# YuQiao0303/PointDreamer

Hardware: AMD Instinct MI355X
Metric: shapes/hour (30k-pt cloud, 8x256^2 views, DDNM) on MI355X (higher is better)
Workload: dtype f16 (f32 accumulate; f32 GroupNorm/softmax statistics, f32 geometry); 1 GPU; configs[2]: synthetic 30k-point sphere shape, 8x256^2 views, texture_gen_method='DDNM_inpaint' (100 DDNM steps, 552.8M-param guided-diffusion UNet, random-init weights), NBF [21], atlas 1024^2, complete_unseen_by='unproject', optimize_from=None, hidden-point removal on (device); 4 independent shapes per step, their views batched through the UNet together; parallelism=shapes-parallel x1, views_per_unet_batch=32

## Files before the change

include/pdhip.h:

```cpp
#ifndef PDHIP_H
#define PDHIP_H
#include <stdint.h>
#include <stddef.h>
#ifdef __cplusplus
extern "C" {
#endif

#define PDHIP_OK 0
#define PDHIP_E_ARG (-1)
#define PDHIP_E_HIP (-2)
#define PDHIP_E_STATE (-3)
#define PDHIP_E_NOMEM (-4)
#define PDHIP_E_UNKNOWN_NAME (-5)

int pdhip_version(void);
int pdhip_lab_build(void);
const char* pdhip_last_error(void);
int pdhip_debug_carve_log(int on);
int pdhip_debug_carve_log_read(uint64_t* triples, int capacity);

int pdhip_project_points(const float* cam_params, int V, const float* vertices, int Vn,
                         const float* points, int N, int rescale, double padding,
                         float* pos , float* vertice_uvs ,
                         float* uv_centers, float* uv_scales,
// ... 74 lines not shown
                              const uint8_t* hard_masks, int V, int S, int N, int res, int point_size, int edge_point_size,
                              double mask_ratio_thresh, float* sparse, float* mask0, float* mask2, float* scale_factors ,
                              float* mask_ratios, void* ws , void* stream);
int pdhip_texel_visibility_shapes(const float* cam_params, int V, int S, const float* gb_pos , const uint8_t* mask ,
                                  int A, const float* uv_centers, const float* uv_scales, double padding, const float* mesh_depths ,
                                  int R, float offset, uint8_t* visibility , void* stream);
int pdhip_nbf_shrink_shapes(const uint8_t* mask , const uint8_t* visibility , int V, int S, int A,
                            const int32_t* kernels, int K, uint8_t* out , uint8_t* ws , void* stream);
int pdhip_view_select_blend_shapes(const float* cam_params, int V, int S, const float* gb_pos, const uint8_t* mask, const int64_t* face_id,
                                   int A, const float* f_normals , int F, const float* base_dirs , const float* uv_centers,
                                   const float* uv_scales, double padding, const float* scale_factors, const uint8_t* shrinked ,
                                   int K, const uint8_t* visibility, int complete_unseen_by_projection, const float* inpainted ,
                                   int r, float* atlas , uint8_t* painted , int32_t* view_ids ,
                                   void* stream);

int pdhip_rescale_vertices(float* pos , int V, int Vn, const float* uv_centers, const float* uv_scales,
                           const float* factors , double padding, void* stream);
size_t pdhip_optimize_color_ws_bytes(int V, int res, int A);
int pdhip_optimize_color(float* atlas, int A, const float* uv_map, const int64_t* face_idxs, int V, int res,
                         const float* inpainted , int r, const uint8_t* shrinked, double lr, int iterations,
                         float* final_images, void* ws, void* stream);

int pdhip_resize_mask(const uint8_t* in , int B, int in_h, int in_w,
                      uint8_t* out , int out_h, int out_w, void* stream);

int pdhip_point_visibility(int cam_res, const float* point_uvs , const float* point_depths ,
                           const float* mesh_depths , int V, int N, float offset,
                           uint8_t* visibility , int64_t* point_pixels , void* stream);

size_t pdhip_hpr_ws_bytes(int V, int N);
int pdhip_hidden_point_removal(const float* points , int N, const double* eyes , int V, double radius,
                               const uint8_t* skip, uint8_t* visibility, void* ws, void* stream);
int pdhip_hpr_read_counters(const void* ws, int V, long long* out , void* stream);

int pdhip_point_pixels(const float* point_uvs , int V, int N, int res,
                       int64_t* point_pixels , void* stream);
int pdhip_point_visibility_pixels(int cam_res, const float* point_uvs, const float* point_depths, const float* mesh_depths,
                                  int V, int N, float offset, uint8_t* visibility , int res,
                                  int64_t* point_pixels , void* stream);

size_t pdhip_sparse_views_ws_bytes(int V, int N, int res);
int pdhip_sparse_views(const int64_t* point_pixels , const float* colors ,
                       const uint8_t* validation , const uint8_t* hard_masks ,
                       int V, int N, int res, int point_size, int edge_point_size, double mask_ratio_thresh,
                       float* sparse , float* mask0, float* mask2,
                       float* scale_factors , float* mask_ratios ,
                       void* ws, void* stream);

size_t pdhip_nearest_fill_ws_ints(int B, int H, int W);
int pdhip_nearest_fill(const float* img, float* out, int B, int C, int H, int W,
                       int64_t batch_stride, int64_t chan_stride, int64_t pix_stride,
                       const void* mask, int mask_is_f32, int64_t mask_batch_stride,
                       int32_t* ws, void* stream);

size_t pdhip_linear_fill_ws_bytes(int B, int H, int W);
int pdhip_linear_fill(const float* img, float* out, int B, int C, int H, int W, const void* mask, int mask_is_f32,
                      int64_t mask_batch_stride, void* ws, int32_t* tri, void* stream);
int pdhip_linear_fill_unresolved(const void* ws, int B, int H, int W, int* out, void* stream);
int pdhip_debug_set_linear_local(int on);

int pdhip_debug_set_unproject_generic(int on);

int pdhip_texel_visibility(const float* cam_params, int V, const float* gb_pos ,
                           const uint8_t* mask , int A, const float* uv_centers ,
                           const float* uv_scales , double padding,
                           const float* mesh_depths , int R, float offset,
                           uint8_t* visibility, void* stream);

int pdhip_nbf_shrink(const uint8_t* mask , const uint8_t* visibility , int V, int A,
                     const int32_t* kernels, int K, uint8_t* out, uint8_t* ws, void* stream);
int pdhip_pack_bits(const uint8_t* in , long long n, uint64_t* out , void* stream);
int pdhip_unpack_bits(const uint64_t* in , long long n, uint8_t* out , void* stream);
int pdhip_nbf_triptych(const uint8_t* mask, const uint8_t* visibility, int V, int A, int kernel, uint8_t* out, uint8_t* ws,
                       void* stream);

int pdhip_view_select_blend(const float* cam_params, int V, const float* gb_pos, const uint8_t* mask,
                            const int64_t* face_id , int A, const float* f_normals ,
                            const float* base_dirs , const float* uv_centers, const float* uv_scales,
                            double padding, const float* scale_factors ,
                            const uint8_t* shrinked, int K, const uint8_t* visibility,
                            int complete_unseen_by_projection,
                            const float* inpainted , int r,
                            float* atlas, uint8_t* painted, int32_t* view_ids, void* stream);

int pdhip_compact_texels(const float* gb_pos, const uint8_t* mask, int A, const int32_t* view_ids,
                         float* points, int64_t* coords, int64_t* point_view_ids, int32_t* count_dev,
                         int32_t* ws, void* stream);

typedef struct pdhip_unet pdhip_unet;

int pdhip_unet_create(int image_size, int model_channels, int num_res_blocks, const int* channel_mult, int n_mult,
                      const int* attention_ds, int n_att, int num_head_channels, int out_channels, int max_batch,
                      pdhip_unet** out);
void pdhip_unet_destroy(pdhip_unet* u);
long long pdhip_unet_arena_bytes(const pdhip_unet* u);
int pdhip_unet_route_table(int image_size, int model_channels, int num_res_blocks, const int* channel_mult, int n_mult, const int* attention_ds,
                           int n_att, int num_head_channels, int out_channels, int max_batch, int N, char* buf, int buf_len);
int pdhip_unet_num_tensors(const pdhip_unet* u);
int pdhip_unet_load_tensor(pdhip_unet* u, const char* name, const void* data, int is_f16, const int64_t* shape, int ndim,
                           void* stream);
int pdhip_unet_missing_tensors(const pdhip_unet* u, char* buf, int buf_len);
int pdhip_unet_forward(pdhip_unet* u, const float* x, const float* t, int N, float* out, void* stream);
int pdhip_unet_profile(pdhip_unet* u, int enable);
int pdhip_unet_profile_read(pdhip_unet* u, double* total_ms, double* total_flops, long long* launches);
int pdhip_unet_profile_read_attention(pdhip_unet* u, double* total_ms, double* total_flops, long long* launches);

int pdhip_ddnm_schedule(float* at, float* at_next, int* t, int* t_next, float* coefs);
int pdhip_ddnm_prepare(const float* masked_imgs , const float* masks , float* y, int N, int HW, void* stream);
int pdhip_ddnm_step(float* x, const float* et, int et_channels, const float* y, const float* mask, const float* eps,
                    uint64_t seed, int step, int N, int HW, void* stream);
int pdhip_ddnm_sample(pdhip_unet* u, const float* masked_imgs, const float* masks, int N, const float* x_T,
                      const float* eps_tape, uint64_t seed, int n_steps, float* out, void* stream);
int pdhip_ddnm_sample_keyed(pdhip_unet* u, const float* masked_imgs, const float* masks, int N, const float* x_T,
                            const float* eps_tape, uint64_t seed, uint64_t first_image_key, int n_steps, float* out, void* stream);

int pdhip_debug_set_conv_bk(int bk);
int pdhip_debug_set_conv_tile(int geometry);
int pdhip_debug_set_conv_stages(int stages);
int pdhip_debug_set_conv_splitk(void* ws, long long ws_floats, int splits);
int pdhip_debug_set_conv_halo_strips(int mode);
int pdhip_pack_conv_weight_f16(const float* w_oihw, int Cout, int Cin, int taps, void* w_packed , void* stream);
int pdhip_conv2d_nhwc_f16(const void* x, const void* w_packed , const float* bias, const void* residual,
                          void* y, int N, int H, int W, int Cin, int Cout, int Cout_pad, int taps, const void* zero_page,
                          void* stream);
int pdhip_groupnorm_nhwc_f16(const void* x, const float* gamma, const float* beta, const float* film , int N,
                             int H, int W, int C, int silu, int resample, void* y, float* stats_ws, float* ws,
                             long long ws_floats, void* stream);
int pdhip_gn_silu_conv3x3_nhwc_f16(const void* x, const float* gamma, const float* beta, const float* film ,
                                   long long film_stride, const void* w_packed, const float* bias, const void* residual, void* y,
                                   int N, int H, int W, int Cin, int Cout, int Cout_pad, const void* zero_page, float* ws,
                                   long long ws_floats, void* stream);
int pdhip_debug_conv3x3_apply(const void* x, const float* table , const void* w_packed, const float* bias, const void* residual,
                              void* y, int N, int H, int W, int Cin, int Cout, int Cout_pad, const void* zero_page, void* stream);
int pdhip_debug_set_fold_skip(int on);
int pdhip_debug_set_up_phase(int mode);
int pdhip_pack_conv_up2_phase_f16(const void* w_packed, int Cin, int Cout_pad, void* w_phase, void* stream);
int pdhip_conv3x3_up2_phase_nhwc_f16(const void* x, const void* w_phase, const float* bias, void* y, int N, int H, int W, int Cin, int Cout,
                                     int Cout_pad, const void* zero_page, float* gn_part, void* stream);
int pdhip_conv3x3_up2_halo_nhwc_f16(const void* x, const void* w_packed, const float* bias, void* y, int N, int H, int W, int Cin, int Cout,
                                    int Cout_pad, const void* zero_page, void* stream);
int pdhip_debug_set_fold_resample(int on);
int pdhip_debug_set_fold_finalize(int max_batch);
int pdhip_debug_set_fold_finalize_chunks(int chunks);
int pdhip_debug_set_conv_sk(int mode, int tile, int splits);
int pdhip_debug_set_conv_sk_stages(int stages);
int pdhip_debug_set_conv_sk_kgroups(int kg);
int pdhip_debug_set_attn(int nbuf, int vt_form, int qtiles);
int pdhip_debug_set_conv_sk_order(int order);
int pdhip_gn_silu_skip1x1_nhwc_f16(const void* xa, const void* xb, int Ca, int C, const float* stats, const float* gamma, const float* beta,
                                   const void* w_packed, const float* bias, void* h0, void* sk, int N, int H, int W, void* stream);
int pdhip_debug_set_gn_iters(int iters);
int pdhip_debug_set_gn_skip_variant(int v);
int pdhip_debug_set_fuse_skip(int mode, int min_tiles);
int pdhip_debug_set_fuse_gn(int on);
int pdhip_mark_unpainted_faces(const int64_t* face_id, const uint8_t* painted, int A, int F, uint8_t* flags , void* stream);
int pdhip_vertex_texel_fetch(const float* vert_uvs , int V, const float* atlas , const uint8_t* mask ,
                             int A, int32_t* texel , float* colors , float* count , void* stream);
int pdhip_neighbor_diffuse_round(const int32_t* rowptr , const int32_t* colidx, int V, const int32_t* invalid, int IV,
                                 float* colors, float* count, float* tmp , int* colored, void* stream);
int pdhip_scatter_vertex_colors(const int32_t* texel, const float* colors, int V, float* atlas, uint8_t* mask,
                                int32_t* owner_ws , int A, void* stream);
size_t pdhip_subdivide_with_uv_ws_bytes(int V, int U, int F, int K);
int pdhip_subdivide_with_uv(const float* vertices , int V, const int64_t* faces , int F, const float* uvs , int U,
                            const int64_t* face_uv_idx , const int64_t* face_index , int K,
                            float* out_vertices, int64_t* out_faces, float* out_uvs, int64_t* out_face_uv_idx,
                            int32_t* counts , int32_t* counts_host , void* ws, void* stream);
size_t pdhip_vertex_uv_table_ws_bytes(int V, int F);
int pdhip_vertex_uv_table(int V, const int64_t* faces , const int64_t* face_uv_idx , int F, const float* uvs ,
                          int U, float* vert_uvs , int32_t* counts , void* ws, void* stream);
size_t pdhip_neighbour_csr_ws_bytes(int V, int F);
int pdhip_neighbour_csr(int V, const int64_t* faces , int F, int32_t* rowptr , int32_t* colidx ,
                        int32_t* counts , int32_t* counts_host , void* ws, void* stream);
size_t pdhip_compact_zero_count_ws_bytes(int V);
int pdhip_compact_zero_count(const float* count , int V, int32_t* invalid , int32_t* counts ,
                             int32_t* counts_host , void* ws, void* stream);

long long pdhip_io_ply_count(const char* path);
int pdhip_io_read_ply_xyzrgb(const char* path, float* xyz , uint8_t* rgb , long long n);
int pdhip_io_write_obj_mtl(const char* obj_path, const char* mtl_path, const char* texture_stem, const double* points, long long P,
                           const double* tcoords, long long T, const int64_t* faces, const int64_t* facetex, long long F);
int pdhip_io_write_obj_plain(const char* obj_path, const float* points , long long P, const int64_t* faces , long long F);
int pdhip_io_write_png(const char* path, const uint8_t* hwc, int H, int W, int channels, int zlib_level);
int pdhip_chw_f32_to_hwc_u8(const float* img, int C, int H, int W, uint8_t* out, void* stream);

size_t pdhip_unet_head_ws_floats(int N, int H, int W, int C, int Cout);
int pdhip_unet_head_f32(const void* x, const float* gamma, const float* beta, const float* w_oihw, const float* bias,
                        int N, int H, int W, int C, int Cout, float* y_nchw, float* ws, long long ws_floats, void* stream);
int pdhip_conv_rr_f16(const void* x, const void* x2, int C, int Ca, int gn_mode, const float* gamma, const float* beta, const float* film,
                      long long film_stride, const float* partA, int chunksA, const float* partB, int chunksB, const void* xs, const void* xs2, int Cs,
                      int Cs1, int taps, const void* wf, const float* bias, const void* residual, int res_up, void* y, int N, int H, int W, int Cout,
                      float* ws, long long ws_floats, float* gn_part, int* gn_chunks, void* stream);
long long pdhip_conv_rr_weight_halfs(int Cin, int taps, int Cs, int Cout);
int pdhip_conv_rr_pack_f16(const void* w_packed, int Cin, int taps, int Cs, int Cout, void* wf, void* stream);
int pdhip_gn_octet_partials_f16(const void* x, int N, int HW, int C, int chunks, float* part, void* stream);
int pdhip_gn_apply_parts_f16(const void* x, const void* x2, int Ca, int C, const float* partA, int chunksA, const float* partB, int chunksB, const float* gamma,
                             const float* beta, const float* film, long long film_stride, int N, int H, int W, int silu, void* y, void* stream);
int pdhip_debug_conv_launch_nhwc_f16(const void* x, const void* x2, int Cin1, const void* w_packed, const float* bias, const void* residual, int res_up,
                                     const void* xs, const void* xs2, int Cs1, int Cs, void* y, int N, int H, int W, int Cin, int Cout, int Cout_pad, int taps,
                                     const void* zero_page, float* ws, long long ws_floats, float* gn_part, long long gn_part_floats, int* gn_chunks, int* kernel,
                                     void* stream);
int pdhip_gn_finalize_oct_f32(const float* partA, int Ca, int chunksA, const float* partB, int Cb, int chunksB, int N, int HW, float* stats, void* stream);
int pdhip_conv_ht_f16(const void* x, const void* w_packed, const float* bias, const void* residual, int res_up, void* y, int N, int H, int W, int Cin, int Cout,
                      int Cout_pad, const void* zero_page, float* splitk_ws, long long splitk_ws_floats, float* gn_part, int* gn_chunks, void* stream);
int pdhip_conv_ht_plan(int N, int H, int W, int Cin, int Cout, int Cout_pad, long long splitk_ws_floats, int* routed, int* slabs);
int pdhip_debug_set_conv_ht(int mode, int slabs);
int pdhip_debug_set_rr_gn(int max_width);
int pdhip_debug_set_conv_rr(int mode, int variant, int slabs);
int pdhip_attention_f16(const void* qkv , void* out , int N, int T, int C, int head_dim,
                        void* vt_ws , void* stream);
int pdhip_philox_normal(float* out, long long n, uint64_t seed, uint64_t stream_id, void* stream);
int pdhip_gemv_rows_f32(const float* W, const float* b, const float* x, float* y, int R, int K, int N, int silu_out, void* stream);
int pdhip_timestep_mlp_f32(const float* t, int N, int mc, const float* w0, const float* b0, const float* w2, const float* b2, float* emb_silu,
                           float* tmp, void* stream);
int pdhip_conv_in_f16(const float* x_nchw, const void* Wt, const float* bias, void* Y, int N, int H, int W, int Cout, int Cout_pad, void* im2col_ws,
                      const void* zero_page, void* stream);
int pdhip_gn_apply_f16(const void* x, const void* x2, int Ca, int C, const float* stats, const float* partA, int chunksA, const float* partB, int chunksB,
                       const float* gamma, const float* beta, const float* film, long long film_stride, int N, int H, int W, int silu, int resample, void* y,
                       void* y_raw, void* stream);
int pdhip_gn_table_f32(const float* stats, const float* gamma, const float* beta, const float* film, long long film_stride, int N, int C, float* table, void* stream);
int pdhip_resample2x_nhwc_f16(const void* x, int N, int H, int W, int C, int mode, void* y, void* stream);
int pdhip_concat_channels_f16(const void* a, int Ca, const void* b, int Cb, long long pixels, void* y, void* stream);
int pdhip_bench_copy16(const void* src, void* dst, long long bytes, int blocks, int unroll, void* stream);

size_t pdhip_nearest_points_workspace_bytes(int Q, int M);
int pdhip_nearest_points_stage_chunk(void);
int pdhip_nearest_points(const float* queries, int Q, const float* targets, int M, double* d2, int32_t* idx, int32_t* counts, void* ws, void* stream);
int pdhip_debug_set_nearest_path(int path);
size_t pdhip_cloud_metrics_workspace_bytes(int T);
int pdhip_cloud_metrics(const double* d2, const int32_t* idx, int Q, const float* normals_src, const float* normals_tgt, int M,
                        const double* thresholds, int T, double* sums, int64_t* within, void* ws, void* stream);

size_t pdhip_mesh_contains_workspace_bytes(int Vn, int F, int Q, int resolution);
int pdhip_mesh_contains(const float* vertices, int Vn, const int64_t* faces, int F, const float* points, int Q, int resolution, uint8_t* occ,
                        int32_t* counts, void* ws, void* stream);
int pdhip_debug_set_mesh_contains_slabs(int slabs);
int pdhip_occupancy_iou(const uint8_t* a, const uint8_t* b, int Q, int64_t* out, void* stream);

size_t pdhip_closest_on_mesh_workspace_bytes(int Vn, int F, int Q);
int pdhip_closest_on_mesh(const float* vertices, int Vn, const int64_t* faces, int F, const float* points, int Q, double* d2, int32_t* face,
                          double* closest, int32_t* counts, void* ws, void* stream);
int pdhip_debug_set_closest_on_mesh(int cells_per_axis, int path);

size_t pdhip_fps_workspace_bytes(int N, int M);
int pdhip_fps(const float* points, int N, int M, int start, int32_t* idx, double* min_d2, int32_t* counts, void* ws, void* stream);
int pdhip_debug_set_fps_cells(int cells_per_axis);
size_t pdhip_owner_mean_colors_workspace_bytes(int M);
int pdhip_owner_mean_colors(const int32_t* owner, const float* colors, int N, int M, const float* fallback, float* out, void* ws_or_null, void* stream);

size_t pdhip_knn_points_workspace_bytes(int Q, int M, int k);
int pdhip_knn_max_k(void);
size_t pdhip_knn_lds_bytes(int k);
int pdhip_knn_points(const float* queries, int Q, const float* targets, int M, int k, double* d2, int32_t* idx, int32_t* counts, void* ws, void* stream);
int pdhip_debug_set_knn(int cells_per_axis, int path);
size_t pdhip_sor_filter_workspace_bytes(int N);
int pdhip_sor_filter(const double* knn_d2, int N, int kk, double std_ratio, double* mean_d, double* stats, uint8_t* keep, int32_t* kept_idx,
                     int32_t* counts, void* ws, void* stream);

size_t pdhip_mesh_components_workspace_bytes(int Vn, int F);
int pdhip_mesh_components(const int64_t* faces, int F, const float* vertices_or_null, int Vn, int32_t* vertex_comp, int32_t* face_comp,
                          int32_t* comp_root, int32_t* comp_vertices, int32_t* comp_faces, float* comp_box_or_null, int comp_capacity,
                          int32_t* counts, void* ws, void* stream);
size_t pdhip_compact_mesh_workspace_bytes(int Vn, int F);
int pdhip_compact_mesh(const float* vertices, int Vn, const int64_t* faces, int F, const float* colors_or_null, const uint8_t* face_keep,
                       float* out_vertices, int64_t* out_faces, float* out_colors_or_null, int32_t* vertex_map_or_null, int32_t* counts, void* ws,
                       void* stream);

int pdhip_mesh_boundary_vertices(const int64_t* faces, int F, int Vn, const int32_t* rowptr, const int32_t* colidx, int32_t* pair_faces,
                                 uint8_t* boundary, int32_t* counts, void* stream);
int pdhip_smooth_mesh(const float* vertices, int Vn, const int32_t* rowptr, const int32_t* colidx, const uint8_t* held_or_null, int steps,
                      double lambda, double mu, double* state_a, double* state_b, float* out_vertices, int32_t* counts, void* stream);

int pdhip_weld_cells_axis(int Vn);
int pdhip_weld_vertices(const float* vertices, int Vn, double tol, int32_t* rep, int32_t* counts, uint64_t* keys_a, uint64_t* keys_b, int32_t* vals_a,
                        int32_t* vals_b, size_t sort_len, int32_t* hist, size_t hist_words, int32_t* cstart, size_t cstart_len, float* sorted_xyzi,
                        size_t sorted_len, int32_t* parent, size_t parent_len, int32_t* misc, size_t misc_len, void* stream);
int pdhip_clean_faces(const int64_t* faces, int F, const int32_t* rep, int Vn, int64_t* out_faces, uint8_t* keep, int32_t* counts, uint64_t* keys_a,
                      uint64_t* keys_b, int32_t* vals_a, int32_t* vals_b, size_t sort_len, int32_t* hist, size_t hist_words, int32_t* misc,
                      size_t misc_len, void* stream);

size_t pdhip_debug_prims_workspace_bytes(int n, int nc);
int pdhip_debug_radix_sort(const uint64_t* keys, const int32_t* vals, int n, int bits, uint64_t* keys_out, int32_t* vals_out, void* ws, void* stream);
int pdhip_debug_sort_by_cell(const uint64_t* keys, int n, int nc, uint64_t* keys_out, int32_t* idx_out, int32_t* cstart_out, void* ws, void* stream);
int pdhip_debug_scan(const void* in, void* out, int n, int elem_bytes, int mode, int inclusive, int nc, void* ws, void* stream);

#ifdef __cplusplus
}
#endif
#endif
```

pointdreamer_amd/csrc/nn_common.h:

```cpp
#pragma once
#include "common.h"
#include <hip/hip_fp16.h>

namespace pdnn {

typedef _Float16 half_t;
typedef __attribute__((ext_vector_type(8))) _Float16 half8;
typedef __attribute__((ext_vector_type(4))) _Float16 half4;
typedef __attribute__((ext_vector_type(4))) float float4_t;

struct Tuning {
    int force_bk = 0;
    int force_stages = 0;
    int force_wmw = 0;
    int force_splits = 0;
    int halo_strips = 0;
    int sk_mode = 1;
    int sk_tile = 0;
    int sk_splits = 0;
    int sk_stages = 0;
    int sk_kg = 0;
    int sk_order = 0;
    int rr_mode = 1;
    int rr_variant = 0;
    int rr_slabs = 0;
    int ht_mode = 1;
    int ht_slabs = 0;
    int fuse_gn = 0;
    int fold_resample = 1;
    int fold_skip = 1;
    int rr_gn = 0;
    int fold_finalize = 8, fold_finalize_chunks = 16;
    int fuse_skip = 1, fuse_skip_min_tiles = 1;
    int up_phase = 1;
    int attn_nbuf = 0;
    int attn_qtn = 0;
    int attn_vt = 0;
    int gn_iters = 0;
    int gs_variant = 1;
};
Tuning& tuning();

bool conv3x3_halo_eligible(int N, int H, int W, int Cin, int Cout_pad);
int conv3x3_halo_splits(int N, int H, int W, int Cin, int Cout, int Cout_pad, size_t splitk_ws_floats);
int conv3x3_halo_launch_splits(const Tuning& t, int N, int H, int W, int Cin, int Cout, int Cout_pad, size_t halo_ws_floats);
inline bool conv3x3_halo_rows(const Tuning& t, int H, int W) { return W == 256 && (t.halo_strips == 1 || H % 4 != 0); }
int conv3x3_halo(const half_t* X, const half_t* Wt, const float* bias, const half_t* residual, half_t* Y, int N, int H, int W,
                 int Cin, int Cout, int Cout_pad, const half_t* zero_page, hipStream_t s, float* gn_part, int splits, bool full_rows,
                 float* splitk_ws, size_t splitk_ws_floats, const float* apply_table = nullptr, int res_up = 0,
                 int in_up = 0);
int splitk_reduce(const float* partial, int splits, long long M, int Cout, const float* bias, const half_t* residual, half_t* Y,
                  float* gn_part, int hw, hipStream_t s);
int conv_igemm(const Tuning& t, const half_t* X, const half_t* Wt, const float* bias, const half_t* residual, half_t* Y, int N, int H,
               int W, int Cin, int Cout, int Cout_pad, int taps, const half_t* zero_page, hipStream_t s,
               float* splitk_ws = nullptr, size_t splitk_ws_floats = 0, float* gn_part = nullptr,
               const half_t* X2 = nullptr, int Cin1 = 0,
               const float* apply_table = nullptr,
               int res_up = 0,
               int in_up = 0);
bool conv_up2_phase_eligible(int N, int H, int W, int Cin, int Cout, int Cout_pad);
int conv_up2_phase_pack(const half_t* w9, int Cin, int Cout_pad, half_t* dst, hipStream_t s);
int conv_up2_phase(const half_t* X, const half_t* Wph, const float* bias, half_t* Y, int N, int H, int W, int Cin, int Cout, int Cout_pad,
                   const half_t* zero_page, hipStream_t s, float* gn_part, int geo);
struct SkPlan { int bm, bn, splits, tile_id;
                int kg, stages, m_fast; };
SkPlan conv_sk_plan(const Tuning& t, int N, int H, int W, int Cin, int Cout, int Cout_pad, int taps, bool two_source, size_t ws_floats, int k_extra = 0);
int conv_sk_skip(const SkPlan& pl, const half_t* X, const half_t* Wt, const float* bias, half_t* Y, int N, int H, int W, int Cin, int Cout,
                 int Cout_pad, const half_t* XS, const half_t* XS2, int Cs1, int Cs, const half_t* zero_page, hipStream_t s, float* ws,
                 size_t ws_floats, float* gn_part);
int fuse_skip_weights(const half_t* w3, int K9, const half_t* w1, int Cs, int Cout_pad, const float* b3, const float* b1, int Cout, half_t* dst,
                      float* bdst, hipStream_t s);
int conv_sk(const SkPlan& pl, const half_t* X, const half_t* Wt, const float* bias, const half_t* residual, half_t* Y, int N, int H, int W,
            int Cin, int Cout, int Cout_pad, int taps, const half_t* zero_page, hipStream_t s, float* ws, size_t ws_floats, float* gn_part,
            const half_t* X2, int Cin1, int res_up = 0);
#define PD_SK_TICKET_FLOATS 4096
int gn_finalize_oct(const float* partA, int Ca, int chunksA, const float* partB, int Cb, int chunksB, int N, int HW, float eps,
                    float* stats, hipStream_t s);

struct RrIn {
    const half_t* x; const half_t* x2; int C, Ca;
    int gn;
    const float* gamma; const float* beta; const float* film; long long film_stride;
    const float* partA; const float* partB; int chunksA, chunksB; float eps;
};
struct RrPlan { int variant, S0, U0, S1, U1, bands, ntiles; };
RrPlan conv_rr_plan(const Tuning& t, int N, int H, int W, int Cin, int Cout, int taps, int Cs , size_t ws_floats,
                    bool want_gn = false );
size_t conv_rr_weight_halfs(int Cin, int taps, int Cs, int Cout);
int conv_rr_pack(const half_t* w_packed, int Cin, int taps, int Cs, int Cout, half_t* dst, hipStream_t s);
int conv_rr(const RrPlan& pl, const RrIn& in, const RrIn* skip, int taps, const half_t* wf, const float* bias, const half_t* residual, int res_up,
            half_t* Y, int N, int H, int W, int Cout, float* ws, size_t ws_floats, float* gn_part , hipStream_t s);
#define PD_RR_MAX_PART_LOADS 8

bool conv_ht_routes(const Tuning& t, int N, int H, int W, int Cin, int Cout, int Cout_pad, size_t ws_floats);
int conv_ht_slabs(const Tuning& t, int N, int H, int W, int Cin, int Cout_pad, size_t ws_floats);
int conv_ht(const half_t* X, const half_t* Wt, const float* bias, const half_t* residual, half_t* Y, int N, int H, int W, int Cin, int Cout,
            int Cout_pad, const half_t* zero_page, hipStream_t s, float* gn_part , int res_up, int slabs, float* ws, size_t ws_floats);

enum ConvKernel { CONV_HALO, CONV_RR, CONV_HT, CONV_SK, CONV_IGEMM, CONV_UP_PHASE };
const char* conv_kernel_name(ConvKernel k);
struct ConvNeeds {
    bool two_source = false;
    bool in_up = false;
    bool apply = false;
    bool in_gn = false;
    bool want_gn = false;
    int skip_cs = 0;
    bool have_wf = false, have_wf_skip = false;
};
struct ConvPlan {
    int N = 0, H = 0, W = 0, Cin = 0, Cout = 0, Cout_pad = 0, taps = 0;
    ConvKernel kernel = CONV_IGEMM;
    SkPlan sk{0, 0, 0, 0}; RrPlan rr{0, 0, 0, 0, 0, 0, 0};
    int splits = 1;
    bool halo_rows = false;
    int slabs = 1;
    int bk = 0, geo = 0;
    int stages = 0;
    bool want_gn = false;
    int gn_chunks = 0;
    bool takes_res_up = false;
    bool takes_in_up = false, takes_apply = false, takes_in_gn = false, takes_skip = false;
    int skip_cs = 0;
};
ConvPlan conv_plan(const Tuning& t, int N, int H, int W, int Cin, int Cout, int Cout_pad, int taps, const ConvNeeds& needs, size_t ws_floats);
ConvPlan conv_up2_phase_plan(const Tuning& t, int N, int H, int W, int Cin, int Cout, int Cout_pad, bool want_gn);
struct ConvArgs {
    const half_t* X; const half_t* X2; int Cin1;
    const half_t* Wt;
    const float* bias; const half_t* residual; int res_up;
    const float* apply_table;
    const RrIn* rr_in;
    const half_t* XS; const half_t* XS2; int Cs1;
    half_t* Y; const half_t* zero_page; float* ws; size_t ws_floats;
    float* gn_part;
};
int conv_launch(const ConvPlan& p, const ConvArgs& a, hipStream_t s);

__device__ __forceinline__ float silu_f(float x) { return x * __builtin_amdgcn_rcpf(1.0f + __expf(-x)); }

__device__ __forceinline__ float gn_round_f16(float f) { asm("" : "+v"(f)); return (float)(half_t)f; }
template <bool OUT_F32, bool FILM>
__device__ __forceinline__ float gn_elem(float x, float ga, float gb, float t1, float sh, int silu) {
    float f = __builtin_fmaf(x, ga, gb);
    if (!OUT_F32) f = gn_round_f16(f);
    if (FILM) {
        f = gn_round_f16(f * t1);
        f = gn_round_f16(f + sh);
    }
    if (silu) { f = silu_f(f); if (!OUT_F32) f = gn_round_f16(f); }
    return f;
}


int gn_stats(const half_t* X, int N, int HW, int C, float eps, float* stats, float* ws, size_t ws_floats, hipStream_t s);
struct GnPartsArg { const float* partA; int Ca, chunksA; const float* partB; int Cb, chunksB; float eps; };
int gn_apply(const half_t* X, const float* stats, const float* gamma, const float* beta, const float* film,
             long long film_stride, int N, int H, int W, int C, int silu, int resample, void* Y, int out_f32, hipStream_t s,
             const half_t* XB = nullptr, int Ca = 0,
             half_t* Yraw = nullptr,
             const GnPartsArg* parts = nullptr,
             int iters_hook = 0);
int gn_table(const float* stats, const float* gamma, const float* beta, const float* film, long long film_stride, int N, int C,
             float* table, hipStream_t s);
bool gn_skip_eligible(int N, int HW, int Ca, int C, int Cout, int Cout_pad);
int gn_skip(const half_t* XA, const half_t* XB, int Ca, int C, const float* stats, const float* gamma, const float* beta, const half_t* Wt,
            const float* bias, half_t* H0, half_t* SK, int N, int HW, hipStream_t s, int variant );
int resample2x(const half_t* X, int N, int H, int W, int C, int mode, half_t* Y, hipStream_t s);
int concat_channels(const half_t* A, int Ca, const half_t* B, int Cb, long long pixels, half_t* Y, hipStream_t s);

int attention(const half_t* qkv, half_t* out, int N, int T, int C, int D, hipStream_t s, half_t* vt_ws, int nbuf, int qtn, int vt);

int conv_in_3x3(const ConvPlan& p, const float* x_nchw, const half_t* Wt , const float* bias, half_t* Y,
                int N, int H, int W, int Cout, int Cout_pad, half_t* im2col_ws , const half_t* zero_page, hipStream_t s, float* gn_part = nullptr);
int head_pack(const float* w, int NO, int C, half_t* wz, hipStream_t s);
int head_gn_silu_conv3x3(const half_t* X, const float* stats, const float* gamma, const float* beta, const half_t* wz,
                         const float* bias, float* y_nchw, int N, int H, int W, int C, int NO, hipStream_t s);
int timestep_mlp(const float* t, int N, int mc, const float* w0, const float* b0, const float* w2, const float* b2,
                 float* emb_silu , float* tmp, hipStream_t s);
int gemv_rows(const float* Wm , const float* b, const float* x , float* y , int R, int K, int N,
              hipStream_t s);

struct DdnmCoef { float sqrt_1m_at, sqrt_at, sqrt_at_next, sigma_t, c1, c2; };
int ddnm_update(float* x , const float* et , int Cet, const float* y,
                const float* mask , const float* eps , unsigned long long seed,
                unsigned long long step, DdnmCoef co, int N, int HW, hipStream_t s, unsigned long long quad0 = 0);
int ddnm_prepare(const float* masked_img, const float* mask, float* y, int N, int HW, hipStream_t s);
int ddnm_finish(const float* x, float* out, long long n, hipStream_t s);
int copy16(const void* src, void* dst, long long bytes, int blocks, int unroll, hipStream_t s);
int philox_normal(float* out, long long n, unsigned long long seed, unsigned long long stream_id, hipStream_t s,
                  unsigned long long quad0 = 0);

}
```

pointdreamer_amd/csrc/nn_head.hip:

```cpp
#include "nn_common.h"
using namespace pdhip;
namespace pdnn {

#define HD_TW 32
#define HD_TH 8
#define HD_TPW 4
#define HD_IW (HD_TW + 2)
#define HD_IH (HD_TH + 2)
#define HD_NPIX (HD_IW * HD_IH)
#define HD_NCH ((HD_NPIX + 15) / 16)
#define HD_ZS_OF(NO) ((NO) == 6 ? 60 : 28)

__device__ __host__ __forceinline__ int hd_swz(int n, int C) { return n & 15 & (C / 8 - 1); }

__global__ void k_head_pack(const float* __restrict__ w , int NO, int C, half_t* __restrict__ wz) {
    const int total = 64 * C;
    for (int i = blockIdx.x * blockDim.x + threadIdx.x; i < total; i += gridDim.x * blockDim.x) {
        const int n = i / C, c = i - n * C;
        float v = 0.f;
        if (n < 9 * NO) { const int tap = n / NO, o = n - tap * NO; v = w[(size_t)o * 9 * C + (size_t)tap * C + c]; }
        const half_t hi = (half_t)v;
        const half_t lo = (half_t)(v - (float)hi);
        const int dst = n * C + (((c >> 3) ^ hd_swz(n, C)) << 3) + (c & 7);
        wz[dst] = hi;
        wz[64 * C + dst] = lo;
    }
}

int head_pack(const float* w, int NO, int C, half_t* wz, hipStream_t s) {
    PD_REQUIRE((NO == 3 || NO == 6) && (C == 32 || C == 64 || C == 128 || C == 256), "head_pack: out channels 3|6, C in {32,64,128,256}");
    k_head_pack<<<cdiv(64 * C, 256), 256, 0, s>>>(w, NO, C, wz);
    PD_LAUNCH_CHECK();
    return PDHIP_OK;
}

__device__ __forceinline__ float hd_silu(float x) { return x * __builtin_amdgcn_rcpf(1.0f + __expf(-x)); }

template <int NO, int C>
__global__ __launch_bounds__(512) void k_head(const half_t* __restrict__ X, const float* __restrict__ stats,
                                              const float* __restrict__ gamma, const float* __restrict__ beta,
                                              const half_t* __restrict__ wz, const float* __restrict__ bias,
                                              float* __restrict__ y, int H, int W, int tpw) {
    constexpr int KK = C / 32;
    constexpr int NT = (9 * NO + 15) / 16;
    constexpr int NR = NT * 16;
    constexpr int HD_ZS = HD_ZS_OF(NO);
    extern __shared__ __attribute__((aligned(16))) char smem[];
    half_t* Bs = reinterpret_cast<half_t*>(smem);
    float* zs = reinterpret_cast<float*>(smem + (size_t)2 * NR * C * 2);
    float* gab = zs + HD_NCH * 16 * HD_ZS;
    const int tid = threadIdx.x, lane = tid & 63, wave = tid >> 6;
    const int n = blockIdx.z, x0 = blockIdx.x * HD_TW;

    for (int i = tid; i < 2 * NR * C / 8; i += 512) {
        const int pl = i / (NR * C / 8), r = i - pl * (NR * C / 8);
        reinterpret_cast<half8*>(Bs)[i] = reinterpret_cast<const half8*>(wz)[pl * (64 * C / 8) + r];
    }
    for (int c = tid; c < C; c += 512) {
        const int grp = c / (C / 32);
        const float mean = stats[((size_t)n * 32 + grp) * 2], rstd = stats[((size_t)n * 32 + grp) * 2 + 1];
        const float ga = rstd * gamma[c];
        gab[c] = ga;
        gab[C + c] = beta[c] - mean * ga;
    }
    __syncthreads();

    const int q4 = lane >> 4, r16 = lane & 15;
    for (int it = 0; it < tpw; ++it) {
    const int y0 = (blockIdx.y * tpw + it) * HD_TH;
    if (y0 >= H) break;
    auto src_of = [&](int chunk, bool* inimg) -> const half_t* {
        const int idx = chunk * 16 + r16;
        const int iy = idx / HD_IW, ix = idx - iy * HD_IW;
        const int gy = y0 - 1 + iy, gx = x0 - 1 + ix;
        *inimg = idx < HD_NPIX && gy >= 0 && gy < H && gx >= 0 && gx < W;
        return X + (((size_t)n * H + (*inimg ? gy : 0)) * W + (*inimg ? gx : 0)) * C + 8 * q4;
    };
    half8 vn[KK];
    bool in_n = false;
    if (wave < HD_NCH) {
        const half_t* sp = src_of(wave, &in_n);
#pragma unroll
        for (int kk = 0; kk < KK; ++kk) vn[kk] = *reinterpret_cast<const half8*>(sp + kk * 32);
    }
    for (int chunk = wave; chunk < HD_NCH; chunk += 8) {
        half8 v[KK];
        const bool inimg = in_n;
#pragma unroll
        for (int kk = 0; kk < KK; ++kk) v[kk] = vn[kk];
        if (chunk + 8 < HD_NCH) {
            const half_t* sp = src_of(chunk + 8, &in_n);
#pragma unroll
            for (int kk = 0; kk < KK; ++kk) vn[kk] = *reinterpret_cast<const half8*>(sp + kk * 32);
        }
        float4_t acc[NT];
#pragma unroll
        for (int t = 0; t < NT; ++t) acc[t] = (float4_t){0.f, 0.f, 0.f, 0.f};
#pragma unroll
        for (int kk = 0; kk < KK; ++kk) {
            const int c0 = kk * 32 + 8 * q4;
            const float4 g0 = *reinterpret_cast<const float4*>(gab + c0), g1 = *reinterpret_cast<const float4*>(gab + c0 + 4);
            const float4 b0 = *reinterpret_cast<const float4*>(gab + C + c0), b1 = *reinterpret_cast<const float4*>(gab + C + c0 + 4);
            const float ga[8] = {g0.x, g0.y, g0.z, g0.w, g1.x, g1.y, g1.z, g1.w};
            const float gb[8] = {b0.x, b0.y, b0.z, b0.w, b1.x, b1.y, b1.z, b1.w};
            half8 ah, al;
#pragma unroll
            for (int e = 0; e < 8; ++e) {
                float a = hd_silu((float)v[kk][e] * ga[e] + gb[e]);
                if (!inimg) a = 0.f;
                const half_t hi = (half_t)a;
                ah[e] = hi;
                al[e] = (half_t)(a - (float)hi);
            }
#pragma unroll
            for (int t = 0; t < NT; ++t) {
                const int nrow = t * 16 + r16;
                const int off = nrow * C + (((kk * 4 + q4) ^ hd_swz(nrow, C)) << 3);
                const half8 bh = *reinterpret_cast<const half8*>(Bs + off);
                const half8 bl = *reinterpret_cast<const half8*>(Bs + NR * C + off);
                acc[t] = __builtin_amdgcn_mfma_f32_16x16x32_f16(al, bh, acc[t], 0, 0, 0);
                acc[t] = __builtin_amdgcn_mfma_f32_16x16x32_f16(ah, bl, acc[t], 0, 0, 0);
                acc[t] = __builtin_amdgcn_mfma_f32_16x16x32_f16(ah, bh, acc[t], 0, 0, 0);
            }
        }
#pragma unroll
        for (int t = 0; t < NT; ++t) {
            const int col = t * 16 + r16;
            if (col < 9 * NO) {
#pragma unroll
                for (int r = 0; r < 4; ++r) zs[(chunk * 16 + q4 * 4 + r) * HD_ZS + col] = acc[t][r];
            }
        }
    }
    __syncthreads();

    for (int item = tid; item < HD_TW * HD_TH * NO; item += 512) {
        const int o = item / (HD_TW * HD_TH), q = item - o * (HD_TW * HD_TH);
        const int qy = q / HD_TW, qx = q - qy * HD_TW;
        const int gy = y0 + qy, gx = x0 + qx;
        if (gy >= H || gx >= W) continue;
        float a = bias[o];
#pragma unroll
        for (int tap = 0; tap < 9; ++tap) {
            const int iy = qy + tap / 3, ix = qx + tap % 3;
            a += zs[(iy * HD_IW + ix) * HD_ZS + tap * NO + o];
        }
        y[(((size_t)n * NO + o) * H + gy) * W + gx] = a;
    }
    __syncthreads();
    }
}

size_t head_smem_bytes(int C, int NO) {
    const int NR = ((9 * NO + 15) / 16) * 16;
    return (size_t)2 * NR * C * 2 + (size_t)HD_NCH * 16 * HD_ZS_OF(NO) * 4 + (size_t)2 * C * 4;
}

template <int NO, int C>
static int head_launch(const half_t* X, const float* stats, const float* gamma, const float* beta, const half_t* wz,
                       const float* bias, float* y, int N, int H, int W, hipStream_t s) {
    auto kern = k_head<NO, C>;
    const size_t smem = head_smem_bytes(C, NO);
    PD_HIP(hipFuncSetAttribute((const void*)kern, hipFuncAttributeMaxDynamicSharedMemorySize, (int)smem));
    int tpw = HD_TPW;
    while (tpw > 1 && (long long)cdiv(W, HD_TW) * cdiv(cdiv(H, HD_TH), tpw) * N < 512) tpw >>= 1;
    dim3 grid(cdiv(W, HD_TW), cdiv(cdiv(H, HD_TH), tpw), N);
    kern<<<grid, 512, smem, s>>>(X, stats, gamma, beta, wz, bias, y, H, W, tpw);
    PD_LAUNCH_CHECK();
    return PDHIP_OK;
}

int head_gn_silu_conv3x3(const half_t* X, const float* stats, const float* gamma, const float* beta, const half_t* wz,
                         const float* bias, float* y_nchw, int N, int H, int W, int C, int NO, hipStream_t s) {
    PD_REQUIRE(NO == 3 || NO == 6, "head: out channels must be 3 or 6");
#define HL(NO_, C_) head_launch<NO_, C_>(X, stats, gamma, beta, wz, bias, y_nchw, N, H, W, s)
    if (C == 256) return NO == 6 ? HL(6, 256) : HL(3, 256);
    if (C == 128) return NO == 6 ? HL(6, 128) : HL(3, 128);
    if (C == 64) return NO == 6 ? HL(6, 64) : HL(3, 64);
    if (C == 32) return NO == 6 ? HL(6, 32) : HL(3, 32);
#undef HL
    PD_REQUIRE(false, "head: final channel count must be 32, 64, 128 or 256 (got %d)", C);
    return PDHIP_OK;
}

}
```

pointdreamer_amd/csrc/nn_misc.hip:

```cpp
#include "nn_common.h"
using namespace pdhip;
namespace pdnn {

__global__ __launch_bounds__(256) void k_im2col_in(const float* __restrict__ x, half_t* __restrict__ A, int H, int W,
                                                   long long pixels) {
    for (long long p = blockIdx.x * (long long)blockDim.x + threadIdx.x; p < pixels; p += (long long)gridDim.x * blockDim.x) {
        const int xx = (int)(p % W), y = (int)((p / W) % H);
        const long long n = p / ((long long)W * H);
        half_t row[32];
#pragma unroll
        for (int k = 27; k < 32; ++k) row[k] = (half_t)0.f;
#pragma unroll
        for (int ky = 0; ky < 3; ++ky)
#pragma unroll
            for (int kx = 0; kx < 3; ++kx) {
                const int yy = y + ky - 1, xc = xx + kx - 1;
                const bool ok = yy >= 0 && yy < H && xc >= 0 && xc < W;
#pragma unroll
                for (int c = 0; c < 3; ++c)
                    row[(ky * 3 + kx) * 3 + c] = ok ? (half_t)x[(((size_t)n * 3 + c) * H + yy) * W + xc] : (half_t)0.f;
            }
        half8* dst = reinterpret_cast<half8*>(A + (size_t)p * 32);
#pragma unroll
        for (int q = 0; q < 4; ++q) {
            half8 v;
#pragma unroll
            for (int e = 0; e < 8; ++e) v[e] = row[q * 8 + e];
            dst[q] = v;
        }
    }
}

int conv_in_3x3(const ConvPlan& p, const float* x_nchw, const half_t* Wt, const float* bias, half_t* Y, int N, int H, int W, int Cout, int Cout_pad,
                half_t* im2col_ws, const half_t* zero_page, hipStream_t s, float* gn_part) {
    PD_REQUIRE(p.N == N && p.H == H && p.W == W && p.Cin == 32 && p.Cout == Cout && p.Cout_pad == Cout_pad && p.taps == 1, "conv_in_3x3: the plan is of another layer");
    const long long pixels = (long long)N * H * W;
    k_im2col_in<<<(int)std::min<long long>((pixels + 255) / 256, 8192), 256, 0, s>>>(x_nchw, im2col_ws, H, W, pixels);
    PD_LAUNCH_CHECK();
    const ConvArgs a{im2col_ws, nullptr, 32, Wt, bias, nullptr, 0, nullptr, nullptr, nullptr, nullptr, 0, Y, zero_page, nullptr, 0, gn_part};
    return conv_launch(p, a, s);
}

#define GEMV_ROWS 128
template <int KI>
__global__ __launch_bounds__(256) void k_gemv_rows(const float* __restrict__ Wm, const float* __restrict__ b,
                                                   const float* __restrict__ x, float* __restrict__ y, int R, int K, int N,
                                                   int silu_out) {
    extern __shared__ __attribute__((aligned(16))) float s_x[];
    const int lane = threadIdx.x & 63, wave = threadIdx.x >> 6;
    const int r0 = blockIdx.x * GEMV_ROWS + wave * (GEMV_ROWS / 4);
    for (int n0 = 0; n0 < N; n0 += 8) {
        const int nb = min(8, N - n0);
        __syncthreads();
        for (int j = 0; j < 8; ++j)
            for (int k = threadIdx.x; k < K; k += 256) s_x[j * K + k] = j < nb ? x[(size_t)(n0 + j) * K + k] : 0.f;
        __syncthreads();
        for (int rr = 0; rr < GEMV_ROWS / 4; rr += 4) {
            const int r = r0 + rr;
            if (r >= R) break;
            float acc[4][8];
#pragma unroll
            for (int q = 0; q < 4; ++q)
#pragma unroll
                for (int j = 0; j < 8; ++j) acc[q][j] = 0.f;
            if (KI > 0) {
                float4 w[4][KI > 0 ? KI : 1];
#pragma unroll
                for (int q = 0; q < 4; ++q)
#pragma unroll
                    for (int it = 0; it < KI; ++it)
                        w[q][it] = *reinterpret_cast<const float4*>(Wm + (size_t)min(r + q, R - 1) * K + it * 256 + lane * 4);
#pragma unroll
                for (int it = 0; it < KI; ++it)
#pragma unroll
                    for (int j = 0; j < 8; ++j) {
                        const float4 xv = *reinterpret_cast<const float4*>(s_x + j * K + it * 256 + lane * 4);
#pragma unroll
                        for (int q = 0; q < 4; ++q)
                            acc[q][j] += w[q][it].x * xv.x + w[q][it].y * xv.y + w[q][it].z * xv.z + w[q][it].w * xv.w;
                    }
            } else {
                for (int k = lane; k < K; k += 64) {
#pragma unroll
                    for (int q = 0; q < 4; ++q) {
                        const float w = Wm[(size_t)min(r + q, R - 1) * K + k];
#pragma unroll
                        for (int j = 0; j < 8; ++j) acc[q][j] += w * s_x[j * K + k];
                    }
                }
            }
#pragma unroll
            for (int q = 0; q < 4; ++q)
#pragma unroll
                for (int j = 0; j < 8; ++j) {
                    float a = acc[q][j];
#pragma unroll
                    for (int off = 32; off > 0; off >>= 1) a += __shfl_xor(a, off);
                    if (lane == 0 && j < nb && r + q < R) {
                        a += b[r + q];
                        if (silu_out) a = a / (1.0f + expf(-a));
                        y[(size_t)(n0 + j) * R + r + q] = a;
                    }
                }
        }
    }
}

static int gemv_launch(const float* Wm, const float* b, const float* x, float* y, int R, int K, int N, int silu_out, hipStream_t s) {
    PD_REQUIRE((size_t)8 * K * sizeof(float) <= 64 * 1024, "gemv_rows: K too large (%d)", K);
    const size_t smem = (size_t)8 * K * sizeof(float);
    const int grid = cdiv(R, GEMV_ROWS);
    if (K == 1024) k_gemv_rows<4><<<grid, 256, smem, s>>>(Wm, b, x, y, R, K, N, silu_out);
    else if (K == 512) k_gemv_rows<2><<<grid, 256, smem, s>>>(Wm, b, x, y, R, K, N, silu_out);
    else if (K == 256) k_gemv_rows<1><<<grid, 256, smem, s>>>(Wm, b, x, y, R, K, N, silu_out);
    else k_gemv_rows<0><<<grid, 256, smem, s>>>(Wm, b, x, y, R, K, N, silu_out);
    PD_LAUNCH_CHECK();
    return PDHIP_OK;
}

int gemv_rows(const float* Wm, const float* b, const float* x, float* y, int R, int K, int N, hipStream_t s) {
    return gemv_launch(Wm, b, x, y, R, K, N, 0, s);
}

__global__ void k_timestep_embedding(const float* __restrict__ t, int N, int mc, float* __restrict__ e) {
    const int half = mc / 2;
    for (int idx = blockIdx.x * blockDim.x + threadIdx.x; idx < N * half; idx += gridDim.x * blockDim.x) {
        const int n = idx / half, i = idx - n * half;
        const float freq = expf(-logf(10000.0f) * (float)i / (float)half);
        const float a = t[n] * freq;
        e[(size_t)n * mc + i] = cosf(a);
        e[(size_t)n * mc + half + i] = sinf(a);
    }
}

int timestep_mlp(const float* t, int N, int mc, const float* w0, const float* b0, const float* w2, const float* b2,
                 float* emb_silu, float* tmp, hipStream_t s) {
    float* temb = tmp;
    float* h1 = tmp + (size_t)N * mc;
    k_timestep_embedding<<<cdiv((long long)N * mc / 2, 256), 256, 0, s>>>(t, N, mc, temb);
    int rc = gemv_launch(w0, b0, temb, h1, 4 * mc, mc, N, 1, s);
    if (rc) return rc;
    return gemv_launch(w2, b2, h1, emb_silu, 4 * mc, 4 * mc, N, 1, s);
}

__device__ __forceinline__ void philox4x32_10(uint32_t c[4], uint32_t k0, uint32_t k1) {
#pragma unroll
    for (int r = 0; r < 10; ++r) {
        const uint64_t p0 = (uint64_t)0xD2511F53u * c[0], p1 = (uint64_t)0xCD9E8D57u * c[2];
        const uint32_t n0 = (uint32_t)(p1 >> 32) ^ c[1] ^ k0, n2 = (uint32_t)(p0 >> 32) ^ c[3] ^ k1;
        c[0] = n0; c[1] = (uint32_t)p1; c[2] = n2; c[3] = (uint32_t)p0;
        k0 += 0x9E3779B9u; k1 += 0xBB67AE85u;
    }
}
__device__ __forceinline__ void normal4(unsigned long long seed, unsigned long long stream_id, unsigned long long quad, float out[4]) {
    uint32_t c[4] = {(uint32_t)quad, (uint32_t)(quad >> 32), (uint32_t)stream_id, (uint32_t)(stream_id >> 32)};
    philox4x32_10(c, (uint32_t)seed, (uint32_t)(seed >> 32));
    const float u0 = ((float)c[0] + 0.5f) * 2.3283064365386963e-10f, u1 = ((float)c[1] + 0.5f) * 2.3283064365386963e-10f;
    const float u2 = ((float)c[2] + 0.5f) * 2.3283064365386963e-10f, u3 = ((float)c[3] + 0.5f) * 2.3283064365386963e-10f;
    const float r0 = sqrtf(-2.0f * logf(u0)), r1 = sqrtf(-2.0f * logf(u2));
    out[0] = r0 * cosf(6.283185307179586f * u1); out[1] = r0 * sinf(6.283185307179586f * u1);
    out[2] = r1 * cosf(6.283185307179586f * u3); out[3] = r1 * sinf(6.283185307179586f * u3);
}

__global__ void k_philox_normal(float* __restrict__ out, long long n, unsigned long long seed, unsigned long long stream_id,
                                unsigned long long quad0) {
    const long long quads = (n + 3) / 4;
    for (long long qd = blockIdx.x * (long long)blockDim.x + threadIdx.x; qd < quads; qd += (long long)gridDim.x * blockDim.x) {
        float z[4];
        normal4(seed, stream_id, quad0 + (unsigned long long)qd, z);
#pragma unroll
        for (int e = 0; e < 4; ++e)
            if (qd * 4 + e < n) out[qd * 4 + e] = z[e];
    }
}

int philox_normal(float* out, long long n, unsigned long long seed, unsigned long long stream_id, hipStream_t s,
                  unsigned long long quad0) {
    k_philox_normal<<<(int)std::min<long long>(((n + 3) / 4 + 255) / 256, 4096), 256, 0, s>>>(out, n, seed, stream_id, quad0);
    PD_LAUNCH_CHECK();
    return PDHIP_OK;
}

__global__ void k_ddnm_prepare(const float* __restrict__ img, const float* __restrict__ mask, float* __restrict__ y, int HW,
                               long long total) {
    for (long long i = blockIdx.x * (long long)blockDim.x + threadIdx.x; i < total; i += (long long)gridDim.x * blockDim.x) {
        const long long n = i / (3LL * HW);
        const int p = (int)(i % HW);
        y[i] = (2.0f * img[i] - 1.0f) * mask[n * HW + p];
    }
}
int ddnm_prepare(const float* masked_img, const float* mask, float* y, int N, int HW, hipStream_t s) {
    const long long total = (long long)N * 3 * HW;
    k_ddnm_prepare<<<(int)std::min<long long>((total + 255) / 256, 4096), 256, 0, s>>>(masked_img, mask, y, HW, total);
    PD_LAUNCH_CHECK();
    return PDHIP_OK;
}

__global__ void k_ddnm_update(float* __restrict__ x, const float* __restrict__ et, int Cet, const float* __restrict__ y,
                              const float* __restrict__ mask, const float* __restrict__ eps, unsigned long long seed,
                              unsigned long long step, DdnmCoef co, int HW, long long total, unsigned long long quad0) {
    for (long long q = blockIdx.x * (long long)blockDim.x + threadIdx.x; q * 4 < total; q += (long long)gridDim.x * blockDim.x) {
        const long long i = q * 4;
        const long long n = i / (3LL * HW);
        const int c = (int)((i / HW) % 3);
        const int p = (int)(i % HW);
        float z[4];
        if (eps) { const float4 e4 = *reinterpret_cast<const float4*>(eps + i); z[0] = e4.x; z[1] = e4.y; z[2] = e4.z; z[3] = e4.w; }
        else normal4(seed, step, quad0 + (unsigned long long)q, z);
        const float4 x4 = *reinterpret_cast<const float4*>(x + i);
        const float4 e4 = *reinterpret_cast<const float4*>(et + ((size_t)n * Cet + c) * HW + p);
        const float4 y4 = *reinterpret_cast<const float4*>(y + i);
        const float4 m4 = *reinterpret_cast<const float4*>(mask + n * HW + p);
        const float xv[4] = {x4.x, x4.y, x4.z, x4.w}, ev[4] = {e4.x, e4.y, e4.z, e4.w};
        const float yv[4] = {y4.x, y4.y, y4.z, y4.w}, mv[4] = {m4.x, m4.y, m4.z, m4.w};
        float o[4];
#pragma unroll
        for (int k = 0; k < 4; ++k) {
            const float x0 = (xv[k] - ev[k] * co.sqrt_1m_at) / co.sqrt_at;
            const float x0h = x0 - mv[k] * (mv[k] * x0 - yv[k]);
            o[k] = co.sqrt_at_next * x0h + co.sigma_t * (co.c1 * z[k] + co.c2 * ev[k]);
        }
        *reinterpret_cast<float4*>(x + i) = make_float4(o[0], o[1], o[2], o[3]);
    }
}
int ddnm_update(float* x, const float* et, int Cet, const float* y, const float* mask, const float* eps,
                unsigned long long seed, unsigned long long step, DdnmCoef co, int N, int HW, hipStream_t s,
                unsigned long long quad0) {
    PD_REQUIRE(HW % 4 == 0, "ddnm_update: H*W must be a multiple of 4");
    const long long total = (long long)N * 3 * HW;
    k_ddnm_update<<<(int)std::min<long long>((total / 4 + 255) / 256, 4096), 256, 0, s>>>(x, et, Cet, y, mask, eps, seed, step, co,
                                                                                       HW, total, quad0);
    PD_LAUNCH_CHECK();
    return PDHIP_OK;
}

__global__ void k_ddnm_finish(const float* __restrict__ x, float* __restrict__ out, long long n) {
    for (long long i = blockIdx.x * (long long)blockDim.x + threadIdx.x; i < n; i += (long long)gridDim.x * blockDim.x)
        out[i] = fminf(fmaxf((x[i] + 1.0f) / 2.0f, 0.0f), 1.0f);
}
int ddnm_finish(const float* x, float* out, long long n, hipStream_t s) {
    k_ddnm_finish<<<(int)std::min<long long>((n + 255) / 256, 4096), 256, 0, s>>>(x, out, n);
    PD_LAUNCH_CHECK();
    return PDHIP_OK;
}

typedef __attribute__((ext_vector_type(4))) float cp_f4;
template <int U, int MODE>
__global__ __launch_bounds__(256) void k_copy16(const cp_f4* __restrict__ src, cp_f4* __restrict__ dst, long long n16) {
    if (MODE == 2) {
        const long long per = (n16 + gridDim.x - 1) / gridDim.x, b0 = (long long)blockIdx.x * per, b1 = b0 + per < n16 ? b0 + per : n16;
        long long i = b0 + threadIdx.x;
        for (; i + (U - 1) * 256 < b1; i += U * 256) {
            cp_f4 v[U];
#pragma unroll
            for (int u = 0; u < U; ++u) v[u] = src[i + u * 256];
#pragma unroll
            for (int u = 0; u < U; ++u) dst[i + u * 256] = v[u];
        }
        for (; i < b1; i += 256) dst[i] = src[i];
        return;
    }
    const long long stride = (long long)gridDim.x * 256;
    long long i = (long long)blockIdx.x * 256 + threadIdx.x;
    for (; i + (U - 1) * stride < n16; i += U * stride) {
        cp_f4 v[U];
#pragma unroll
        for (int u = 0; u < U; ++u) v[u] = MODE == 1 ? __builtin_nontemporal_load(src + i + u * stride) : src[i + u * stride];
#pragma unroll
        for (int u = 0; u < U; ++u) { if (MODE == 1) __builtin_nontemporal_store(v[u], dst + i + u * stride); else dst[i + u * stride] = v[u]; }
    }
    for (; i < n16; i += stride) dst[i] = src[i];
}
int copy16(const void* src, void* dst, long long bytes, int blocks, int unroll, hipStream_t s) {
    PD_REQUIRE(src && dst && bytes > 0 && bytes % 16 == 0, "copy16: bytes must be a positive multiple of 16");
    const long long n16 = bytes / 16;
    if (blocks <= 0) blocks = 256 * 8;
    const int mode = unroll >> 4, u = unroll & 15;
#define PD_CP(U_, M_) k_copy16<U_, M_><<<blocks, 256, 0, s>>>((const cp_f4*)src, (cp_f4*)dst, n16)
#define PD_CPM(M_) (u == 8 ? PD_CP(8, M_) : u == 2 ? PD_CP(2, M_) : u == 1 ? PD_CP(1, M_) : PD_CP(4, M_))
    if (mode == 1) PD_CPM(1); else if (mode == 2) PD_CPM(2); else PD_CPM(0);
#undef PD_CPM
#undef PD_CP
    PD_LAUNCH_CHECK();
    return PDHIP_OK;
}

}

extern "C" int pdhip_gemv_rows_f32(const float* W, const float* b, const float* x, float* y, int R, int K, int N, int silu_out, void* stream) {
    PD_REQUIRE(W && b && x && y, "pdhip_gemv_rows_f32: null argument");
    PD_REQUIRE(R >= 1 && K >= 1 && N >= 1, "pdhip_gemv_rows_f32: R, K, N must be positive (R=%d K=%d N=%d)", R, K, N);
    return pdnn::gemv_launch(W, b, x, y, R, K, N, silu_out != 0, as_stream(stream));
}
extern "C" int pdhip_timestep_mlp_f32(const float* t, int N, int mc, const float* w0, const float* b0, const float* w2, const float* b2,
                                      float* emb_silu, float* tmp, void* stream) {
    PD_REQUIRE(t && w0 && b0 && w2 && b2 && emb_silu && tmp, "pdhip_timestep_mlp_f32: null argument");
    PD_REQUIRE(N >= 1 && mc >= 2 && mc % 2 == 0 && mc <= 512, "pdhip_timestep_mlp_f32: N must be positive and mc even, at most 512 (N=%d mc=%d)", N, mc);
    return pdnn::timestep_mlp(t, N, mc, w0, b0, w2, b2, emb_silu, tmp, as_stream(stream));
}
extern "C" int pdhip_conv_in_f16(const float* x_nchw, const void* Wt, const float* bias, void* Y, int N, int H, int W, int Cout, int Cout_pad,
                                 void* im2col_ws, const void* zero_page, void* stream) {
    PD_REQUIRE(x_nchw && Wt && bias && Y && im2col_ws && zero_page, "pdhip_conv_in_f16: null argument");
    PD_REQUIRE(N >= 1 && H >= 1 && W >= 1 && Cout >= 1, "pdhip_conv_in_f16: N, H, W, Cout must be positive");
    PD_REQUIRE(Cout % 8 == 0 && Cout_pad % 128 == 0 && Cout_pad >= Cout, "conv_igemm: need Cin %% 32 == 0, Cout %% 8 == 0, padded Cout %% 128 == 0 (Cin=%d Cout=%d pad=%d)", 32,
               Cout, Cout_pad);
    const pdnn::ConvPlan p = pdnn::conv_plan(pdnn::tuning(), N, H, W, 32, Cout, Cout_pad, 1, pdnn::ConvNeeds(), 0);
    return pdnn::conv_in_3x3(p, x_nchw, (const pdnn::half_t*)Wt, bias, (pdnn::half_t*)Y, N, H, W, Cout, Cout_pad, (pdnn::half_t*)im2col_ws, (const pdnn::half_t*)zero_page,
                             as_stream(stream));
}
```

pointdreamer_amd/csrc/nn_norm.hip:

```cpp
#include "nn_common.h"
using namespace pdhip;
namespace pdnn {

#define GN_PIX_PER_BLOCK 256

__global__ __launch_bounds__(256) void k_gn_partial(const half_t* __restrict__ X, int HW, int C, float* __restrict__ part) {
    extern __shared__ float s_acc[];
    const int n = blockIdx.y, chunk = blockIdx.x;
    const int opp = C >> 3;
    const int pps = max(1, 256 / opp);
    const int tid = threadIdx.x;
    const int sub = tid / opp, oct = tid - sub * opp;
    const int p0 = chunk * GN_PIX_PER_BLOCK;
    const int p1 = min(HW, p0 + GN_PIX_PER_BLOCK);
    float s[8], q[8];
#pragma unroll
    for (int e = 0; e < 8; ++e) { s[e] = 0.f; q[e] = 0.f; }
    if (sub < pps) {
        for (int oc = oct; oc < opp; oc += 256) {
            for (int p = p0 + sub; p < p1; p += pps) {
                const half8 v = *reinterpret_cast<const half8*>(X + ((size_t)n * HW + p) * C + oc * 8);
#pragma unroll
                for (int e = 0; e < 8; ++e) { const float f = (float)v[e]; s[e] += f; q[e] += f * f; }
            }
// ... 152 lines not shown
        __syncthreads();
        if (threadIdx.x < 32) {
            const int opg = cg >> 3, g = threadIdx.x;
            double ds = 0.0, dq = 0.0;
            for (int k = 0; k < opg; ++k)
                for (int sl = 0; sl < pps; ++sl) { ds += s_fin[(sl * opp + g * opg + k) * 2]; dq += s_fin[(sl * opp + g * opg + k) * 2 + 1]; }
            const double cnt = (double)H * W * cg;
            const double mean = ds / cnt;
            double var = dq / cnt - mean * mean;
            if (var < 0.0) var = 0.0;
            s_st[2 * g] = (float)mean; s_st[2 * g + 1] = (float)(1.0 / sqrt(var + (double)gp.eps));
        }
        __syncthreads();
    }
#ifdef PD_LAB_GN_REV
    const int n = gridDim.y - 1 - blockIdx.y, bx = gridDim.x - 1 - blockIdx.x;
#else
    const int n = blockIdx.y, bx = blockIdx.x;
#endif
    const int sub = threadIdx.x / opp;
    if (sub >= pps) return;
    const int p_begin = bx * (pps * iters), p_end = min(Ho * Wo, p_begin + pps * iters);
    for (int oc = threadIdx.x - sub * opp; oc < opp; oc += 256) {
        const int c0 = oc * 8;
        const bool second = XB != nullptr && c0 >= Ca;
        const half_t* const Xs = second ? XB + (c0 - Ca) : X + c0;
        const int cs = XB == nullptr ? C : (second ? C - Ca : Ca);
        float ga[8], gb[8], t1[8], sh[8];
#pragma unroll
        for (int e = 0; e < 8; ++e) {
            const int c = c0 + e, grp = c / cg;
            const float mean = FIN ? s_st[2 * grp] : stats[((size_t)n * 32 + grp) * 2], rstd = FIN ? s_st[2 * grp + 1] : stats[((size_t)n * 32 + grp) * 2 + 1];
            ga[e] = rstd * gamma[c];
            gb[e] = beta[c] - mean * ga[e];
            if (FILM) {
                t1[e] = (float)(half_t)(1.0f + (float)(half_t)film[(size_t)n * film_stride + c]);
                sh[e] = (float)(half_t)film[(size_t)n * film_stride + C + c];
            }
        }
        float raw[8];
#pragma unroll
        for (int e = 0; e < 8; ++e) raw[e] = 0.f;
        auto act = [&](int yi, int xi, float* o) {
            const half8 v = *reinterpret_cast<const half8*>(Xs + (((size_t)n * H + yi) * W + xi) * cs);
            if (RES == 1) {
#pragma unroll
                for (int e = 0; e < 8; ++e) raw[e] += (float)v[e];
            }
#pragma unroll
            for (int e = 0; e < 8; ++e) {
                o[e] = gn_elem<OUT_F32, FILM>((float)v[e], ga[e], gb[e], FILM ? t1[e] : 1.f, FILM ? sh[e] : 0.f, silu);
            }
        };
        auto finish = [&](const half8& v, float* r) {
#pragma unroll
            for (int e = 0; e < 8; ++e) {
                r[e] = gn_elem<OUT_F32, FILM>((float)v[e], ga[e], gb[e], FILM ? t1[e] : 1.f, FILM ? sh[e] : 0.f, silu);
            }
        };
        auto store = [&](int p, const float* r) {
            const size_t o = ((size_t)n * Ho * Wo + p) * C + c0;
            if (OUT_F32) {
                float* Y = reinterpret_cast<float*>(Yv);
                *reinterpret_cast<float4*>(Y + o) = make_float4(r[0], r[1], r[2], r[3]);
                *reinterpret_cast<float4*>(Y + o + 4) = make_float4(r[4], r[5], r[6], r[7]);
            } else {
                half8 hv;
#pragma unroll
                for (int e = 0; e < 8; ++e) hv[e] = (half_t)r[e];
#ifdef PD_LAB_GN_NT
                __builtin_nontemporal_store(hv, reinterpret_cast<half8*>(reinterpret_cast<half_t*>(Yv) + o));
#else
                *reinterpret_cast<half8*>(reinterpret_cast<half_t*>(Yv) + o) = hv;
#endif
            }
        };
        if (RES == 0) {
            int p = p_begin + sub;
#ifndef GNA_U
#define GNA_U 4
#endif
            for (; p + (GNA_U - 1) * pps < p_end; p += GNA_U * pps) {
                half8 v[GNA_U];
#pragma unroll
#ifdef PD_LAB_GN_NTL
                for (int u = 0; u < GNA_U; ++u) v[u] = __builtin_nontemporal_load(reinterpret_cast<const half8*>(Xs + ((size_t)n * H * W + p + u * pps) * cs));
#else
                for (int u = 0; u < GNA_U; ++u) v[u] = *reinterpret_cast<const half8*>(Xs + ((size_t)n * H * W + p + u * pps) * cs);
#endif
#pragma unroll
                for (int u = 0; u < GNA_U; ++u) { float r[8]; finish(v[u], r); store(p + u * pps, r); }
            }
            for (; p < p_end; p += pps) {
                const half8 v = *reinterpret_cast<const half8*>(Xs + ((size_t)n * H * W + p) * cs);
                float r[8]; finish(v, r); store(p, r);
            }
        } else {
            for (int p = p_begin + sub; p < p_end; p += pps) {
                float r[8];
                const int yo = p / Wo, xo = p - yo * Wo;
                if (RES == 1) {
                    float a[8], b[8], c[8], d[8];
                    act(2 * yo, 2 * xo, a); act(2 * yo, 2 * xo + 1, b); act(2 * yo + 1, 2 * xo, c); act(2 * yo + 1, 2 * xo + 1, d);
#pragma unroll
                    for (int e = 0; e < 8; ++e) r[e] = (a[e] + b[e] + c[e] + d[e]) * 0.25f;
                    if (Yraw != nullptr) {
                        half8 hv;
#pragma unroll
                        for (int e = 0; e < 8; ++e) { hv[e] = (half_t)(raw[e] * 0.25f); }
                        *reinterpret_cast<half8*>(Yraw + ((size_t)n * Ho * Wo + p) * C + c0) = hv;
                    }
#pragma unroll
                    for (int e = 0; e < 8; ++e) raw[e] = 0.f;
                } else {
                    act(yo >> 1, xo >> 1, r);
                }
                store(p, r);
            }
        }
    }
}

int gn_apply(const half_t* X, const float* stats, const float* gamma, const float* beta, const float* film,
             long long film_stride, int N, int H, int W, int C, int silu, int resample, void* Y, int out_f32, hipStream_t s,
             const half_t* XB, int Ca, half_t* Yraw, const GnPartsArg* parts, int iters_hook) {
    GnParts gp{nullptr, nullptr, 0, 0, 0, 0, 0.f};
    if (parts != nullptr) {
        PD_REQUIRE(stats == nullptr && parts->partA != nullptr && (C >> 3) <= 256 && ((C / 32) % 8) == 0 && parts->Ca + parts->Cb == C &&
                   parts->Ca % 8 == 0 && parts->Cb % 8 == 0 && (parts->Cb == 0 || parts->partB != nullptr),
                   "gn_apply: bad octet partials for the in-kernel statistics");
        gp = GnParts{parts->partA, parts->partB, parts->Ca, parts->Cb, parts->chunksA, parts->chunksB, parts->eps};
    }
    PD_REQUIRE(Yraw == nullptr || (resample == 1 && XB == nullptr), "gn_apply: the raw avg-pool output belongs to resample 1");
    PD_REQUIRE(XB == nullptr || (Ca > 0 && Ca < C && Ca % 8 == 0), "gn_apply: bad two-source split");
    PD_REQUIRE(C % 32 == 0 && resample >= 0 && resample <= 2, "gn_apply: bad arguments");
    PD_REQUIRE(resample != 1 || (H % 2 == 0 && W % 2 == 0), "gn_apply: avgpool needs even H, W");
    PD_REQUIRE(!out_f32 || (resample == 0 && film == nullptr), "gn_apply: f32 output only without resampling / FiLM");
    PD_REQUIRE(film == nullptr || resample == 0, "gn_apply: FiLM only without resampling");
    const int Ho = resample == 1 ? H / 2 : (resample == 2 ? H * 2 : H), Wo = resample == 1 ? W / 2 : (resample == 2 ? W * 2 : W);
    const int opp = C >> 3, pps = max(1, 256 / opp);
    int iters = iters_hook > 0 ? iters_hook : GNA_ITERS;
    const int tgt_blocks = parts != nullptr && N <= 8 ? 512 : 2048;
    while (iters > 1 && (long long)cdiv((long long)Ho * Wo, pps * iters) * N < tgt_blocks) iters >>= 1;
    dim3 grid(cdiv((long long)Ho * Wo, pps * iters), N);
#define GNA_ARGS X, stats, gamma, beta, film, film_stride, H, W, C, silu, Y, XB, Ca, iters, Yraw, gp
#define GNA_LAUNCH(R, O, F) do { if (parts) k_gn_apply<R, O, F, true><<<grid, 256, 0, s>>>(GNA_ARGS); else k_gn_apply<R, O, F, false><<<grid, 256, 0, s>>>(GNA_ARGS); } while (0)
    if (out_f32) GNA_LAUNCH(0, true, false);
    else if (film) GNA_LAUNCH(0, false, true);
    else if (resample == 0) GNA_LAUNCH(0, false, false);
    else if (resample == 1) GNA_LAUNCH(1, false, false);
    else GNA_LAUNCH(2, false, false);
#undef GNA_LAUNCH
#undef GNA_ARGS
    PD_LAUNCH_CHECK();
    return PDHIP_OK;
}

__global__ __launch_bounds__(256) void k_resample(const half_t* __restrict__ X, int H, int W, int C, int mode,
                                                  half_t* __restrict__ Y, long long total_oct) {
    const int opp = C >> 3;
    const int Ho = mode == 1 ? H / 2 : H * 2, Wo = mode == 1 ? W / 2 : W * 2;
    for (long long idx = blockIdx.x * (long long)blockDim.x + threadIdx.x; idx < total_oct; idx += (long long)gridDim.x * blockDim.x) {
        const int oc = (int)(idx % opp);
        const long long pix = idx / opp;
        const int xo = (int)(pix % Wo), yo = (int)((pix / Wo) % Ho), n = (int)(pix / ((long long)Wo * Ho));
        half8 out;
        if (mode == 1) {
            const half_t* p = X + (((size_t)n * H + 2 * yo) * W + 2 * xo) * C + oc * 8;
            const half8 a = *reinterpret_cast<const half8*>(p), b = *reinterpret_cast<const half8*>(p + C);
            const half8 c = *reinterpret_cast<const half8*>(p + (size_t)W * C), d = *reinterpret_cast<const half8*>(p + (size_t)W * C + C);
#pragma unroll
            for (int e = 0; e < 8; ++e) out[e] = (half_t)(((float)a[e] + (float)b[e] + (float)c[e] + (float)d[e]) * 0.25f);
        } else {
            out = *reinterpret_cast<const half8*>(X + (((size_t)n * H + (yo >> 1)) * W + (xo >> 1)) * C + oc * 8);
        }
        *reinterpret_cast<half8*>(Y + (((size_t)n * Ho + yo) * Wo + xo) * C + oc * 8) = out;
    }
}

int resample2x(const half_t* X, int N, int H, int W, int C, int mode, half_t* Y, hipStream_t s) {
    PD_REQUIRE((mode == 1 || mode == 2) && C % 8 == 0, "resample2x: bad arguments");
    const int Ho = mode == 1 ? H / 2 : H * 2, Wo = mode == 1 ? W / 2 : W * 2;
    const long long total = (long long)N * Ho * Wo * (C / 8);
    k_resample<<<(int)std::min<long long>((total + 255) / 256, 65536), 256, 0, s>>>(X, H, W, C, mode, Y, total);
    PD_LAUNCH_CHECK();
    return PDHIP_OK;
}

__global__ __launch_bounds__(256) void k_concat(const half_t* __restrict__ A, int Ca, const half_t* __restrict__ B, int Cb,
                                                long long pixels, half_t* __restrict__ Y) {
    const int oa = Ca >> 3, ob = Cb >> 3, ot = oa + ob;
    const long long total = pixels * ot;
    for (long long idx = blockIdx.x * (long long)blockDim.x + threadIdx.x; idx < total; idx += (long long)gridDim.x * blockDim.x) {
        const long long p = idx / ot;
        const int o = (int)(idx - p * ot);
        const half8 v = (o < oa) ? *reinterpret_cast<const half8*>(A + (size_t)p * Ca + o * 8)
                                 : *reinterpret_cast<const half8*>(B + (size_t)p * Cb + (o - oa) * 8);
        *reinterpret_cast<half8*>(Y + (size_t)p * (Ca + Cb) + o * 8) = v;
    }
}

int concat_channels(const half_t* A, int Ca, const half_t* B, int Cb, long long pixels, half_t* Y, hipStream_t s) {
    PD_REQUIRE(Ca % 8 == 0 && Cb % 8 == 0, "concat_channels: channels must be multiples of 8");
    const long long total = pixels * ((Ca + Cb) / 8);
    k_concat<<<(int)std::min<long long>((total + 255) / 256, 65536), 256, 0, s>>>(A, Ca, B, Cb, pixels, Y);
    PD_LAUNCH_CHECK();
    return PDHIP_OK;
}

constexpr int GS_BM = 128, GS_BN = 256, GS_CLD = GS_BN + 8;
constexpr int GS_SMEM = GS_BM * GS_CLD * 2;

template <int MI = 4>
__device__ __forceinline__ void gs_epilogue(const float4_t (&acc)[MI][8], char* smem, const float* __restrict__ bias, half_t* __restrict__ SK,
                                            long long m0, int tid) {
    const int lane = tid & 63, wave = tid >> 6, wm = wave & 1, wn = wave >> 1;
    half_t* const Cs = reinterpret_cast<half_t*>(smem);
#pragma unroll
    for (int j = 0; j < 8; ++j) {
        const int nl = wn * 128 + j * 16 + (lane >> 4) * 4;
        float4_t bv = (float4_t){0.f, 0.f, 0.f, 0.f};
        if (bias != nullptr) bv = *reinterpret_cast<const float4_t*>(bias + nl);
#pragma unroll
        for (int i = 0; i < MI; ++i) {
            const int ml = wm * (16 * MI) + i * 16 + (lane & 15);
            half4 h;
#pragma unroll
            for (int r = 0; r < 4; ++r) h[r] = (half_t)(acc[i][j][r] + bv[r]);
            *reinterpret_cast<half4*>(&Cs[ml * GS_CLD + nl]) = h;
        }
    }
    __syncthreads();
    const int col8 = (tid & 31) * 8;
#pragma unroll
    for (int p = 0; p < 4 * MI; ++p) {
        const int row = p * 8 + (tid >> 5);
        *reinterpret_cast<half8*>(SK + (size_t)(m0 + row) * GS_BN + col8) = *reinterpret_cast<const half8*>(&Cs[row * GS_CLD + col8]);
    }
}
template <int NB, int MI = 4>
__device__ __forceinline__ void gs_mfma_step(float4_t (&acc)[MI][8], const char* As, const char* Ws, int lane, int wm, int wn) {
#pragma unroll
    for (int kk = 0; kk < 2; ++kk) {
        const int fo = ((kk * 4 + (lane >> 4)) ^ (lane & 7)) << 4;
        half8 a[MI];
#pragma unroll
        for (int i = 0; i < MI; ++i) a[i] = *reinterpret_cast<const half8*>(As + (wm * (16 * MI) + i * 16 + (lane & 15)) * 128 + fo);
#pragma unroll
        for (int jh = 0; jh < 8 / NB; ++jh) {
            half8 b[NB];
#pragma unroll
            for (int j = 0; j < NB; ++j) b[j] = *reinterpret_cast<const half8*>(Ws + (wn * 128 + (jh * NB + j) * 16 + (lane & 15)) * 128 + fo);
#pragma unroll
            for (int i = 0; i < MI; ++i)
#pragma unroll
                for (int j = 0; j < NB; ++j) acc[i][jh * NB + j] = __builtin_amdgcn_mfma_f32_16x16x32_f16(b[j], a[i], acc[i][jh * NB + j], 0, 0, 0);
        }
    }
}

template <typename T> __device__ __forceinline__ T* gs_uniform(T* p) {
    const unsigned long long v = reinterpret_cast<unsigned long long>(p);
    const unsigned lo = __builtin_amdgcn_readfirstlane((unsigned)v), hi = __builtin_amdgcn_readfirstlane((unsigned)(v >> 32));
    return reinterpret_cast<T*>(((unsigned long long)hi << 32) | lo);
}

#ifndef GS1_NB
#define GS1_NB 2
#endif
constexpr int GS1_SMEM = GS_SMEM;
template <int BM>
__global__ __launch_bounds__(256, 2) void k_gn_skip_w1(const half_t* __restrict__ XA, const half_t* __restrict__ XB, int Ca, int C,
                                                       const float* __restrict__ stats, const float* __restrict__ gamma,
                                                       const float* __restrict__ beta, const half_t* __restrict__ Wt,
                                                       const float* __restrict__ bias, half_t* __restrict__ H0, half_t* __restrict__ SK,
                                                       int HW) {
    extern __shared__ __align__(16) char gs_smem[];
    char* const As = gs_smem;
    constexpr int MI = BM / 32, RJ = BM / 32;
    char* const Ws = gs_smem + BM * 128;
    float* const Gs = reinterpret_cast<float*>(gs_smem + BM * 128 + GS_BN * 128);
    const int tid = threadIdx.x, lane = tid & 63, wave = tid >> 6, wm = wave & 1, wn = wave >> 1;
    const long long m0 = (long long)blockIdx.x * BM;
    const int n = (int)(m0 / HW), cg = C / 32, Cb = C - Ca, KC = C / 64;
    const int slot = tid & 7, prow = tid >> 3;
    const int sw = (slot ^ (prow & 7)) << 4;
    half8 xa[2][RJ], wr[8];
    const unsigned offA = (unsigned)(prow * Ca + slot * 8) * 2u, offB = (unsigned)(prow * Cb + slot * 8) * 2u;
    const unsigned offC = (unsigned)(prow * C + slot * 8) * 2u;
    const char* const baseA = reinterpret_cast<const char*>(XA + (size_t)m0 * Ca);
    const char* const baseB = reinterpret_cast<const char*>(XB + (size_t)m0 * Cb);
    const char* const baseW = reinterpret_cast<const char*>(Wt);
    char* const baseH = reinterpret_cast<char*>(H0 + (size_t)m0 * C);
    auto issue_acts = [&](int kc, half8* dst) {
        const int cu = min(kc, KC - 1) * 64;
        const bool second = cu >= Ca;
        const char* const src = gs_uniform(second ? baseB + (size_t)(cu - Ca) * 2 : baseA + (size_t)cu * 2);
        const unsigned off = second ? offB : offA, rs = (unsigned)(second ? Cb : Ca) * 64u;
#pragma unroll
        for (int j = 0; j < RJ; ++j) dst[j] = *reinterpret_cast<const half8*>(src + (off + j * rs));
    };
    auto issue_w = [&](int kc) {
        const char* const src = gs_uniform(baseW + (size_t)(min(kc, KC - 1) * 64) * 2);
#pragma unroll
        for (int j = 0; j < 8; ++j) wr[j] = *reinterpret_cast<const half8*>(src + (offC + j * ((unsigned)C * 64u)));
    };
// ... 85 lines not shown
```

pointdreamer_amd/csrc/nn_unet.hip:

```cpp
#include "nn_common.h"
#include <map>
#include <string>
#include <vector>
#include <cmath>
#include <cstring>
using namespace pdhip;
using namespace pdnn;

namespace {

struct ConvW { half_t* w = nullptr; float* b = nullptr; int cin = 0, cout = 0, cout_pad = 0, taps = 0; bool have_w = false, have_b = false;
               half_t* wf = nullptr; half_t* wph = nullptr; bool has_wf = false, has_wph = false; };
struct NormW { float* g = nullptr; float* b = nullptr; int c = 0; bool have_g = false, have_b = false; };
struct ResB { std::string name; int cin, cout, mode; NormW n1, n2; ConvW c1, c2, skip; long long emb_off; bool has_skip; bool have_ew = false, have_eb = false;
              half_t* c2s_w = nullptr; float* c2s_b = nullptr; bool c2s_ready = false; half_t* c2s_wf = nullptr; int hw = 0; bool has_c2s = false, has_c2s_wf = false; };
struct AttB { std::string name; int c; NormW n; ConvW qkv, proj; };
struct Block { int kind; int idx; };

struct Act { half_t* p; int C, H, W; const float* gn_part = nullptr; int gn_chunks = 0; const float* gn_partB = nullptr; int Ca = 0; int gn_chunksB = 0;
             half_t* p2 = nullptr;
             int row = -1, rowB = -1; };

}
namespace pdnn {
Tuning& tuning() { static thread_local Tuning t; return t; }
}
static thread_local float* g_dbg_splitk_ws = nullptr;
static thread_local size_t g_dbg_splitk_floats = 0;
namespace {
struct Prof { std::vector<hipEvent_t> ev; std::vector<uint8_t> cls; size_t used = 0; double flops[2] = {0, 0}; bool on = false;
              int period = 1; long long forwards = 0; bool armed = false; };

}

struct pdhip_unet {
    int image_size, mc, nres, head, out_ch, max_batch, ted;
    std::vector<int> mult, att_ds;
    std::vector<ResB> res;
    std::vector<AttB> att;
    std::vector<std::vector<Block>> input, output;
    std::vector<Block> middle;
    int final_ch;
    half_t* w_in = nullptr; float* b_in = nullptr; bool have_win = false, have_bin = false;
    float *te_w0 = nullptr, *te_b0 = nullptr, *te_w2 = nullptr, *te_b2 = nullptr; bool have_te[4] = {false, false, false, false};
    float *emb_w = nullptr, *emb_b = nullptr; long long emb_rows = 0;
    NormW out_norm; float* out_w = nullptr; float* out_b = nullptr; bool have_ow = false, have_ob = false;
    half_t* zero_page = nullptr;
    char* arena = nullptr; size_t arena_bytes = 0, arena_off = 0; bool arena_overflow = false;
    float *stats = nullptr, *gn_ws = nullptr; size_t gn_ws_floats = 0;
    float* ap_table = nullptr;
    float *emb_silu = nullptr, *emb_tmp = nullptr, *emb_all = nullptr;
    float *steps_t = nullptr, *steps_silu = nullptr, *steps_tmp = nullptr, *steps_emb = nullptr; int steps_cached = 0;
    half_t* head_wz = nullptr;
    half_t* head_wz3 = nullptr;
    float *t_dev = nullptr;
    float* splitk_ws = nullptr; size_t splitk_floats = 0;
    float *sx = nullptr, *sy = nullptr, *set_ = nullptr, *smask = nullptr;
    Prof prof;
    std::vector<void*> owned;
};

namespace {

template <typename T>
int dalloc(pdhip_unet* u, T** p, size_t count) {
    void* q = nullptr;
    hipError_t e = hipMalloc(&q, std::max<size_t>(count * sizeof(T), 256));
    if (e != hipSuccess) { set_error("hipMalloc(%zu bytes) failed: %s", count * sizeof(T), hipGetErrorString(e)); return PDHIP_E_NOMEM; }
    u->owned.push_back(q);
    *p = reinterpret_cast<T*>(q);
    return PDHIP_OK;
}
#define PD_TRY(expr) do { int rc_ = (expr); if (rc_ != PDHIP_OK) return rc_; } while (0)

int alloc_conv(pdhip_unet* u, ConvW& c) {
    PD_TRY(dalloc(u, &c.w, (size_t)c.cout_pad * c.taps * c.cin));
    PD_HIP(hipMemset(c.w, 0, (size_t)c.cout_pad * c.taps * c.cin * sizeof(half_t)));
    PD_TRY(dalloc(u, &c.b, (size_t)c.cout));
    return PDHIP_OK;
}
int alloc_norm(pdhip_unet* u, NormW& n, int c) {
    n.c = c;
    PD_TRY(dalloc(u, &n.g, (size_t)c));
    PD_TRY(dalloc(u, &n.b, (size_t)c));
    return PDHIP_OK;
}

__global__ void k_pack_conv(const void* __restrict__ src, int src_f16, int Cout, int Cin, int taps, half_t* __restrict__ dst) {
    const long long total = (long long)Cout * Cin * taps;
    for (long long i = blockIdx.x * (long long)blockDim.x + threadIdx.x; i < total; i += (long long)gridDim.x * blockDim.x) {
        const int tap = (int)(i % taps);
        const int c = (int)((i / taps) % Cin);
        const int o = (int)(i / ((long long)taps * Cin));
        const float v = src_f16 ? (float)reinterpret_cast<const half_t*>(src)[i] : reinterpret_cast<const float*>(src)[i];
        dst[(size_t)o * taps * Cin + (size_t)tap * Cin + c] = (half_t)v;
    }
}
__global__ void k_pack_conv_in(const void* __restrict__ src, int src_f16, int Cout, half_t* __restrict__ dst) {
    const int total = Cout * 27;
    for (int i = blockIdx.x * blockDim.x + threadIdx.x; i < total; i += gridDim.x * blockDim.x) {
        const int tap = i % 9, c = (i / 9) % 3, o = i / 27;
        const float v = src_f16 ? (float)reinterpret_cast<const half_t*>(src)[i] : reinterpret_cast<const float*>(src)[i];
        dst[(size_t)o * 32 + tap * 3 + c] = (half_t)v;
    }
}
__global__ void k_pack_conv_f32(const void* __restrict__ src, int src_f16, int Cout, int Cin, int taps, float* __restrict__ dst) {
    const long long total = (long long)Cout * Cin * taps;
    for (long long i = blockIdx.x * (long long)blockDim.x + threadIdx.x; i < total; i += (long long)gridDim.x * blockDim.x) {
        const int tap = (int)(i % taps);
        const int c = (int)((i / taps) % Cin);
        const int o = (int)(i / ((long long)taps * Cin));
        const float v = src_f16 ? (float)reinterpret_cast<const half_t*>(src)[i] : reinterpret_cast<const float*>(src)[i];
        dst[(size_t)o * taps * Cin + (size_t)tap * Cin + c] = v;
    }
}
__global__ void k_copy_f32(const void* __restrict__ src, int src_f16, long long n, float* __restrict__ dst, int round_f16) {
    for (long long i = blockIdx.x * (long long)blockDim.x + threadIdx.x; i < n; i += (long long)gridDim.x * blockDim.x) {
        float v = src_f16 ? (float)reinterpret_cast<const half_t*>(src)[i] : reinterpret_cast<const float*>(src)[i];
        if (round_f16) v = (float)(half_t)v;
        dst[i] = v;
    }
}
int grid_for(long long n) { return (int)std::min<long long>((n + 255) / 256, 4096); }

half_t* arena_take(pdhip_unet* u, size_t halfs) {
    size_t bytes = (halfs * sizeof(half_t) + 255) & ~(size_t)255;
    if (u->arena == nullptr) { u->arena_off += bytes; return nullptr; }
    if (u->arena_off + bytes > u->arena_bytes) { u->arena_overflow = true; return reinterpret_cast<half_t*>(u->arena); }
    half_t* p = reinterpret_cast<half_t*>(u->arena + u->arena_off);
    u->arena_off += bytes;
    return p;
}

struct Act;
struct Table { std::vector<std::string> name, line; };
struct Ctx { pdhip_unet* u; int N; hipStream_t s; bool dry; const float* film_base; long long film_stride; Table* table;
             Tuning t;
             bool go() const { return !dry && table == nullptr; } };

int prof_begin(Ctx& c, double flops, int cls = 0) {
    Prof& p = c.u->prof;
    if (!p.on || !p.armed || !c.go()) return PDHIP_OK;
    if (p.used + 2 > p.ev.size()) {
        for (int i = 0; i < 256; ++i) { hipEvent_t e; PD_HIP(hipEventCreate(&e)); p.ev.push_back(e); p.cls.push_back(0); }
    }
    PD_HIP(hipEventRecord(p.ev[p.used], c.s));
    p.cls[p.used] = (uint8_t)cls;
    p.flops[cls] += flops;
    return PDHIP_OK;
}
int prof_end(Ctx& c) {
    Prof& p = c.u->prof;
    if (!p.on || !p.armed || !c.go()) return PDHIP_OK;
    PD_HIP(hipEventRecord(p.ev[p.used + 1], c.s));
    p.used += 2;
    return PDHIP_OK;
}

float* take_parts(Ctx& c, int H, int W, int cout) {
    return reinterpret_cast<float*>(arena_take(c.u, (size_t)c.N * ((H * W + 15) / 16) * (cout / 8) * 2 * 2));
}
void adopt_parts(Act* out, float* part, int chunks) {
    if (part != nullptr && chunks > 0) { out->gn_part = part; out->gn_chunks = chunks; out->Ca = out->C; }
}

struct ConvIn { const Act* x; const half_t* residual = nullptr; int res_up = 0; const float* apply_table = nullptr; const RrIn* rr_in = nullptr;
                const Act* skip_src = nullptr; const ResB* skip_w = nullptr;
                const Act* parts_of = nullptr; const char* note = nullptr; };

void table_row(Ctx& c, const std::string& name, const ConvPlan& p, const ConvIn& in, Act* out) {
    char detail[64];
    switch (p.kernel) {
    case CONV_HALO: case CONV_IGEMM: snprintf(detail, sizeof detail, "splits=%d", p.splits); break;
    case CONV_HT: snprintf(detail, sizeof detail, "slabs=%d", p.slabs); break;
    case CONV_RR: snprintf(detail, sizeof detail, "variant=%d,slabs=%d", p.rr.variant, p.rr.S0); break;
    case CONV_SK: snprintf(detail, sizeof detail, "tile=%dx%d,splits=%d", p.sk.bm, p.sk.bn, p.sk.splits); break;
    default: snprintf(detail, sizeof detail, "-"); break;
    }
    std::string folds;
    auto add = [&](const std::string& f) { folds += (folds.empty() ? "" : ",") + f; };
    if (in.note) add(in.note);
    if (in.x->p2) add("two_source");
    if (p.takes_apply) add("apply");
    if (p.takes_in_gn) add("in_gn");
    if (p.takes_in_up) add("in_up");
    if (in.res_up) add("res_up");
    if (p.takes_skip) add("skip");
    if (in.parts_of) {
        const Act& a = *in.parts_of;
        add("parts<-" + (a.gn_part && a.row >= 0 ? c.table->name[a.row] : std::string("?")) +
            (a.p2 ? "+" + (a.gn_partB && a.rowB >= 0 ? c.table->name[a.rowB] : std::string("?")) : std::string()));
    }
    char line[512];
    snprintf(line, sizeof line, "%s %dx%d %d->%d %s %s gn=%d %s", name.c_str(), p.H, p.W, p.Cin, p.Cout, conv_kernel_name(p.kernel), detail, p.gn_chunks,
             folds.empty() ? "-" : folds.c_str());
    out->row = (int)c.table->line.size();
    c.table->name.push_back(name);
    c.table->line.push_back(line);
}

int run_conv(Ctx& c, const std::string& name, const ConvPlan& p, const ConvW& w, const ConvIn& in, Act* out) {
    *out = Act{nullptr, p.Cout, p.H, p.W};
    out->p = arena_take(c.u, (size_t)c.N * p.H * p.W * p.Cout);
    float* part = p.want_gn ? take_parts(c, p.H, p.W, p.Cout) : nullptr;
    if (c.table) table_row(c, name, p, in, out);
    if (!c.dry) adopt_parts(out, part, p.gn_chunks);
    if (!c.go()) return PDHIP_OK;
    PD_REQUIRE(w.have_w && w.have_b, "unet: weights of %s not loaded", name.c_str());
    const ResB* fs = p.takes_skip ? in.skip_w : nullptr;
    PD_REQUIRE(fs == nullptr || (fs->skip.have_w && fs->skip.have_b && fs->c2s_ready), "unet: fused conv2 + skip weights of %s were not built at load time", name.c_str());
    const half_t* wt = fs ? (p.kernel == CONV_RR ? fs->c2s_wf : fs->c2s_w) : p.kernel == CONV_RR ? w.wf : p.kernel == CONV_UP_PHASE ? w.wph : w.w;
    const Act& x = *in.x;
    const Act* xs = p.takes_skip ? in.skip_src : nullptr;
    const ConvArgs a{x.p, x.p2, x.p2 ? x.Ca : 0, wt, fs ? fs->c2s_b : w.b, in.residual, in.res_up, in.apply_table, in.rr_in,
                     xs ? xs->p : nullptr, xs ? xs->p2 : nullptr, xs && xs->p2 ? xs->Ca : 0, out->p, c.u->zero_page, c.u->splitk_ws, c.u->splitk_floats, part};
    const bool booked = p.kernel == CONV_HALO && p.splits == 1;
    if (booked) PD_TRY(prof_begin(c, 2.0 * c.N * p.H * p.W * (double)p.Cout * 9.0 * p.Cin));
    PD_TRY(conv_launch(p, a, c.s));
    return booked ? prof_end(c) : PDHIP_OK;
}
ConvPlan plan_conv(const Ctx& c, const Act& x, const ConvW& w, bool want_gn) {
    ConvNeeds nd;
    nd.two_source = x.p2 != nullptr; nd.want_gn = want_gn; nd.have_wf = w.has_wf;
    return conv_plan(c.t, c.N, x.H, x.W, w.cin, w.cout, w.cout_pad, w.taps, nd, c.u->splitk_floats);
}

int run_gn_stats(Ctx& c, const Act& x) {
    if (x.gn_part != nullptr && ((x.C / 32) % 8) == 0)
        return gn_finalize_oct(x.gn_part, x.Ca, x.gn_chunks, x.gn_partB, x.C - x.Ca, x.gn_chunksB, c.N, x.H * x.W, 1e-5f, c.u->stats, c.s);
    PD_REQUIRE(x.p2 == nullptr, "unet: a virtual concat needs fused GroupNorm partials of both tensors");
    return gn_stats(x.p, c.N, x.H * x.W, x.C, 1e-5f, c.u->stats, c.u->gn_ws, c.u->gn_ws_floats, c.s);
}

int run_gn(Ctx& c, const Act& x, const NormW& n, const float* film, long long film_stride, int silu, int resample, Act* out,
           half_t* raw_pool = nullptr) {
    *out = Act{nullptr, x.C, 0, 0};
    out->H = resample == 1 ? x.H / 2 : (resample == 2 ? x.H * 2 : x.H);
    out->W = resample == 1 ? x.W / 2 : (resample == 2 ? x.W * 2 : x.W);
    out->p = arena_take(c.u, (size_t)c.N * out->H * out->W * x.C);
    if (!c.go()) return PDHIP_OK;
    PD_REQUIRE(n.have_g && n.have_b, "unet: norm weights not loaded");
#ifdef PD_LAB_SKIP_GN
    if (resample == 0 && x.p2 == nullptr && x.W <= 128 && silu) { out->p = x.p; return PDHIP_OK; }
#endif
    if (x.gn_part != nullptr && ((x.C / 32) % 8) == 0 && (x.C >> 3) <= 256 && c.t.fold_finalize > 0 &&
        (c.N <= c.t.fold_finalize || (x.gn_chunks <= c.t.fold_finalize_chunks && x.gn_chunksB <= c.t.fold_finalize_chunks))) {
        const GnPartsArg pa{x.gn_part, x.Ca, x.gn_chunks, x.gn_partB, x.C - x.Ca, x.gn_chunksB, 1e-5f};
        return gn_apply(x.p, nullptr, n.g, n.b, film, film_stride, c.N, x.H, x.W, x.C, silu, resample, out->p, 0, c.s, x.p2,
                        x.p2 ? x.Ca : 0, raw_pool, &pa, c.t.gn_iters);
    }
    PD_TRY(run_gn_stats(c, x));
    return gn_apply(x.p, c.u->stats, n.g, n.b, film, film_stride, c.N, x.H, x.W, x.C, silu, resample, out->p, 0, c.s, x.p2, x.p2 ? x.Ca : 0,
                    raw_pool, nullptr, c.t.gn_iters);
}

int run_gn_then_conv(Ctx& c, const std::string& name, const ConvPlan& p, const Act& x, const NormW& n, const float* film, long long film_stride,
                     int resample, half_t* raw_pool, const ConvW& w, ConvIn in, Act* out) {
    if (p.takes_apply) {
        if (c.go()) {
            PD_REQUIRE(n.have_g && n.have_b, "unet: norm weights not loaded");
            PD_TRY(run_gn_stats(c, x));
            PD_TRY(gn_table(c.u->stats, n.g, n.b, film, film_stride, c.N, x.C, c.u->ap_table, c.s));
            in.apply_table = c.u->ap_table;
        }
        in.x = &x;
        return run_conv(c, name, p, w, in, out);
    }
    if (p.takes_in_gn) {
        if (c.go()) PD_REQUIRE(n.have_g && n.have_b, "unet: norm weights not loaded");
        const RrIn rr_in{x.p, nullptr, x.C, x.C, 2, n.g, n.b, film, film_stride, x.gn_part, nullptr, x.gn_chunks, 0, 1e-5f};
        in.x = &x; in.rr_in = &rr_in; in.parts_of = &x;
        return run_conv(c, name, p, w, in, out);
    }
    Act h;
    PD_TRY(run_gn(c, x, n, film, film_stride, 1, resample, &h, raw_pool));
    in.x = &h;
    if (x.p2 != nullptr) in.parts_of = &x;
    return run_conv(c, name, p, w, in, out);
}

struct ResPlan {
    bool fuse_skip = false;
    bool fold_down = false;
    bool fold_up = false;
    bool skip_conv = false;
    ConvPlan c1, c2, skip;
};
bool wish_in_gn(const Tuning& t, const Act& x, const ConvW& w, int W) {
    if (t.rr_gn <= 0 || W > t.rr_gn || x.p2 != nullptr || x.gn_part == nullptr || x.gn_partB != nullptr || ((x.C / 32) % 8) != 0 || w.cin > 1024 ||
        x.C != w.cin) return false;
    const int pps = std::max(1, 256 / (x.C >> 3));
    return (x.gn_chunks + pps - 1) / pps <= PD_RR_MAX_PART_LOADS;
}
bool wish_up_phase(const Tuning& t, int N, const ResB& rb, int H, int W) {
    if (t.up_phase == 0 || rb.mode != 2 || !rb.c1.has_wph || (H * W) % 256 != 0 ||
        !conv_up2_phase_eligible(N, H, W, rb.c1.cin, rb.c1.cout, rb.c1.cout_pad)) return false;
    if (t.up_phase == 2) return true;
    const long long tiles = (long long)N * H * W / 256 * 4 * (rb.c1.cout_pad / (rb.c1.cout_pad % 256 == 0 ? 256 : 128));
    return tiles >= 128;
}
ResPlan plan_res(const Tuning& t, int N, size_t ws_floats, bool conservative, const Act& x, const ResB& rb) {
    ResPlan r;
    const int Ho = rb.mode == 1 ? x.H / 2 : (rb.mode == 2 ? x.H * 2 : x.H), Wo = rb.mode == 1 ? x.W / 2 : (rb.mode == 2 ? x.W * 2 : x.W);
    const bool lean = !conservative;
    const bool fold = t.fold_resample != 0 && lean && x.p2 == nullptr && !rb.has_skip;
    r.fold_down = fold && rb.mode == 1;
    r.fuse_skip = rb.has_skip && rb.mode == 0 && t.fuse_skip != 0 && rb.skip.taps == 1 && x.C == rb.skip.cin &&
                  gn_skip_eligible(N, x.H * x.W, x.p2 ? x.Ca : x.C, x.C, rb.skip.cout, rb.skip.cout_pad) &&
                  (t.fuse_skip == 2 || (long long)N * x.H * x.W / 128 >= t.fuse_skip_min_tiles) &&
                  (conservative || (x.gn_part != nullptr && ((x.C / 32) % 8) == 0));
    ConvNeeds n1;
    n1.want_gn = true; n1.have_wf = rb.c1.has_wf;
    if (lean && !r.fuse_skip && rb.mode == 0 && x.p2 == nullptr) { n1.apply = t.fuse_gn != 0; n1.in_gn = wish_in_gn(t, x, rb.c1, x.W); }
    n1.in_up = fold && rb.mode == 2;
    if (lean && x.p2 == nullptr && !rb.has_skip && wish_up_phase(t, N, rb, x.H, x.W))
        r.c1 = conv_up2_phase_plan(t, N, Ho, Wo, rb.c1.cin, rb.c1.cout, rb.c1.cout_pad, true);
    else
        r.c1 = conv_plan(t, N, Ho, Wo, rb.c1.cin, rb.c1.cout, rb.c1.cout_pad, 9, n1, ws_floats);
    Act h1{nullptr, rb.cout, Ho, Wo};
    if (r.c1.gn_chunks > 0) { h1.gn_part = x.gn_part ? x.gn_part : reinterpret_cast<const float*>(&r); h1.gn_chunks = r.c1.gn_chunks; h1.Ca = rb.cout; }
    ConvNeeds n2;
    n2.want_gn = true; n2.have_wf = rb.c2.has_wf;
    if (lean) { n2.apply = t.fuse_gn != 0; n2.in_gn = wish_in_gn(t, h1, rb.c2, Wo); }
    if (lean && rb.has_skip && !r.fuse_skip && t.fold_skip != 0 && rb.mode == 0 && rb.has_c2s && rb.skip.taps == 1 &&
        (x.p2 == nullptr || (x.Ca % 64 == 0 && (x.C - x.Ca) % 64 == 0))) {
        n2.skip_cs = rb.skip.cin;
        n2.have_wf_skip = rb.has_c2s_wf && (x.p2 == nullptr || (x.Ca % 128 == 0 && (x.C - x.Ca) % 128 == 0));
    }
    r.c2 = conv_plan(t, N, Ho, Wo, rb.c2.cin, rb.c2.cout, rb.c2.cout_pad, 9, n2, ws_floats);
    r.fold_up = fold && rb.mode == 2 && r.c2.takes_res_up;
    r.skip_conv = rb.has_skip && !r.fuse_skip && !r.c2.takes_skip;
    if (r.skip_conv) {
        ConvNeeds ns;
        ns.two_source = x.p2 != nullptr;
        r.skip = conv_plan(t, N, Ho, Wo, rb.skip.cin, rb.skip.cout, rb.skip.cout_pad, rb.skip.taps, ns, ws_floats);
    }
    return r;
}

int run_res(Ctx& c, const Act& x, ResB& rb, Act* out) {
    const ResPlan r = plan_res(c.t, c.N, c.u->splitk_floats, c.dry, x, rb);
    Act h1, xr = x, sk;
    const float* film = c.go() ? c.film_base + rb.emb_off : nullptr;
    if (c.go()) PD_REQUIRE(rb.have_ew && rb.have_eb, "unet: emb_layers of %s not loaded", rb.name.c_str());
    if (rb.mode != 0) {
        xr.H = r.c2.H; xr.W = r.c2.W;
        xr.p = arena_take(c.u, (size_t)c.N * xr.H * xr.W * x.C);
    }
    const std::string n1 = rb.name + ".in_layers.2";
    if (r.fuse_skip) {
        Act h0{nullptr, x.C, x.H, x.W};
        h0.p = arena_take(c.u, (size_t)c.N * x.H * x.W * x.C);
        sk = Act{nullptr, rb.skip.cout, x.H, x.W};
        sk.p = arena_take(c.u, (size_t)c.N * x.H * x.W * rb.skip.cout);
        if (c.go()) {
            PD_REQUIRE(rb.n1.have_g && rb.n1.have_b && rb.skip.have_w && rb.skip.have_b, "unet: norm / skip weights of %s not loaded", rb.name.c_str());
            PD_TRY(run_gn_stats(c, x));
            PD_TRY(gn_skip(x.p, x.p2, x.p2 ? x.Ca : x.C, x.C, c.u->stats, rb.n1.g, rb.n1.b, rb.skip.w, rb.skip.b, h0.p, sk.p, c.N, x.H * x.W, c.s, c.t.gs_variant));
        }
        ConvIn in{&h0};
        in.parts_of = &x; in.note = "gn_skip";
        PD_TRY(run_conv(c, n1, r.c1, rb.c1, in, &h1));
    } else {
        const bool half_res = r.c1.kernel == CONV_UP_PHASE || r.c1.takes_in_up;
        PD_TRY(run_gn_then_conv(c, n1, r.c1, x, rb.n1, nullptr, 0, half_res ? 0 : rb.mode, r.fold_down ? xr.p : nullptr, rb.c1, ConvIn{nullptr}, &h1));
    }
    if (rb.mode != 0 && c.go() && !r.fold_down && !r.fold_up) PD_TRY(resample2x(x.p, c.N, x.H, x.W, x.C, rb.mode, xr.p, c.s));
    if (!r.fuse_skip) sk = r.fold_up ? x : xr;
    if (r.skip_conv) PD_TRY(run_conv(c, rb.name + ".skip_connection", r.skip, rb.skip, ConvIn{&xr}, &sk));
    ConvIn in2{nullptr, r.c2.takes_skip ? nullptr : sk.p, r.fold_up ? 1 : 0};
    in2.skip_src = &x; in2.skip_w = &rb;
    return run_gn_then_conv(c, rb.name + ".out_layers.3", r.c2, h1, rb.n2, film, c.film_stride, 0, nullptr, rb.c2, in2, out);
}

int run_att(Ctx& c, const Act& x, AttB& ab, Act* out) {
    Act xn, qkv, a;
    PD_TRY(run_gn(c, x, ab.n, nullptr, 0, 0, 0, &xn));
    PD_TRY(run_conv(c, ab.name + ".qkv", plan_conv(c, xn, ab.qkv, false), ab.qkv, ConvIn{&xn}, &qkv));
    a = x;
    a.p = arena_take(c.u, (size_t)c.N * x.H * x.W * x.C);
    half_t* vt = arena_take(c.u, (size_t)c.N * x.H * x.W * x.C);
    if (c.go()) {
        const double T = (double)x.H * x.W;
        PD_TRY(prof_begin(c, 4.0 * c.N * T * T * x.C, 1));
        PD_TRY(attention(qkv.p, a.p, c.N, x.H * x.W, x.C, c.u->head, c.s, vt, c.t.attn_nbuf, c.t.attn_qtn, c.t.attn_vt));
        PD_TRY(prof_end(c));
    }
    return run_conv(c, ab.name + ".proj_out", plan_conv(c, a, ab.proj, true), ab.proj, ConvIn{&a, x.p}, out);
}

int run_blocks(Ctx& c, std::vector<Block>& blocks, Act* h, const float* x_nchw) {
    for (Block& b : blocks) {
        Act o;
        if (b.kind == 0) {
            o.C = c.u->mult[0] * c.u->mc; o.H = o.W = c.u->image_size;
            const int cpad = ((o.C + 127) / 128) * 128;
            ConvNeeds nd;
            nd.want_gn = true;
            const ConvPlan p = conv_plan(c.t, c.N, o.H, o.W, 32, o.C, cpad, 1, nd, 0);
            o.p = arena_take(c.u, (size_t)c.N * o.H * o.W * o.C);
            half_t* col = arena_take(c.u, (size_t)c.N * o.H * o.W * 32);
            float* part = reinterpret_cast<float*>(arena_take(c.u, (size_t)c.N * ((o.H * o.W + 127) / 128) * (o.C / 8) * 2 * 2));
            if (c.table) { Act in{nullptr, 32, o.H, o.W}; table_row(c, "input_blocks.0.0", p, ConvIn{&in}, &o); }
            if (!c.dry) adopt_parts(&o, part, p.gn_chunks);
            if (c.go()) {
                PD_REQUIRE(c.u->have_win && c.u->have_bin, "unet: input conv not loaded");
                PD_TRY(conv_in_3x3(p, x_nchw, c.u->w_in, c.u->b_in, o.p, c.N, o.H, o.W, o.C, cpad, col, c.u->zero_page, c.s, part));
            }
        } else if (b.kind == 1) {
            PD_TRY(run_res(c, *h, c.u->res[b.idx], &o));
        } else {
            PD_TRY(run_att(c, *h, c.u->att[b.idx], &o));
        }
        *h = o;
    }
    return PDHIP_OK;
}

int forward_impl(const Tuning& tun, pdhip_unet* u, const float* x, const float* t, int N, float* out, hipStream_t s, bool dry,
                 const float* shared_emb = nullptr, int head_ch = 0, Table* table = nullptr) {
    Ctx c{u, N, s, dry, shared_emb ? shared_emb : u->emb_all, shared_emb ? 0 : u->emb_rows, table, tun};
    u->arena_off = 0;
    u->arena_overflow = false;
    if (c.go() && u->prof.on) u->prof.armed = (u->prof.forwards++ % u->prof.period) == 0;
    if (c.go() && shared_emb == nullptr) {
        PD_REQUIRE(u->have_te[0] && u->have_te[1] && u->have_te[2] && u->have_te[3], "unet: time_embed not loaded");
        PD_TRY(timestep_mlp(t, N, u->mc, u->te_w0, u->te_b0, u->te_w2, u->te_b2, u->emb_silu, u->emb_tmp, s));
        PD_TRY(gemv_rows(u->emb_w, u->emb_b, u->emb_silu, u->emb_all, (int)u->emb_rows, u->ted, N, s));
    }
    std::vector<Act> hs;
    Act h{nullptr, 0, 0, 0};
    for (auto& blk : u->input) {
        PD_TRY(run_blocks(c, blk, &h, x));
        hs.push_back(h);
    }
    PD_TRY(run_blocks(c, u->middle, &h, x));
    for (auto& blk : u->output) {
        Act sk = hs.back(); hs.pop_back();
        Act cat{nullptr, h.C + sk.C, h.H, h.W};
        const bool part_ok = h.gn_part && sk.gn_part && !h.gn_partB && !sk.gn_partB && !h.p2 && !sk.p2;
        if (part_ok) {
            cat.gn_part = h.gn_part; cat.gn_partB = sk.gn_part; cat.Ca = h.C; cat.gn_chunks = h.gn_chunks; cat.gn_chunksB = sk.gn_chunks;
            cat.row = h.row; cat.rowB = sk.row;
        }
        const Block& first = blk.front();
        const bool virt = part_ok && h.C % 64 == 0 && sk.C % 64 == 0 && ((cat.C / 32) % 8) == 0 && first.kind == 1 &&
                          u->res[first.idx].mode == 0 && u->res[first.idx].has_skip;
        if (virt) {
            cat.p = h.p; cat.p2 = sk.p;
        } else {
            cat.p = arena_take(u, (size_t)N * h.H * h.W * (h.C + sk.C));
            if (c.go()) PD_TRY(concat_channels(h.p, h.C, sk.p, sk.C, (long long)N * h.H * h.W, cat.p, s));
        }
        h = cat;
        PD_TRY(run_blocks(c, blk, &h, x));
    }
    if (c.go()) {
        PD_REQUIRE(!u->arena_overflow, "unet: activation arena too small for this routing (sized at create())");
        PD_REQUIRE(u->out_norm.have_g && u->out_norm.have_b && u->have_ow && u->have_ob, "unet: output head not loaded");
        PD_TRY(run_gn_stats(c, h));
        const bool eps_only = head_ch == 3 && u->out_ch == 6;
        PD_TRY(head_gn_silu_conv3x3(h.p, u->stats, u->out_norm.g, u->out_norm.b, eps_only ? u->head_wz3 : u->head_wz, u->out_b, out, N,
                                    h.H, h.W, h.C, eps_only ? 3 : u->out_ch, s));
    }
    return PDHIP_OK;
}

const size_t kSplitkFloats = (size_t)16 * 384 * 128 * 128;
void shape_conv(ConvW& c, int cin, int cout, int taps) { c.cin = cin; c.cout = cout; c.taps = taps; c.cout_pad = ((cout + 127) / 128) * 128; }
int build_graph(pdhip_unet* u, int image_size, int model_channels, int num_res_blocks, const int* channel_mult, int n_mult,
                const int* attention_ds, int n_att, int num_head_channels, int out_channels, int max_batch) {
    PD_REQUIRE(channel_mult && n_mult > 0 && (n_att == 0 || attention_ds), "pdhip_unet_create: null argument");
    PD_REQUIRE(model_channels % 32 == 0 && image_size % (1 << (n_mult - 1)) == 0 && max_batch >= 1 && max_batch <= 64,
               "pdhip_unet_create: model_channels %% 32, image_size %% 2^(levels-1), 1 <= max_batch <= 64 required");
    PD_REQUIRE(num_head_channels == 32 || num_head_channels == 64, "pdhip_unet_create: num_head_channels must be 32 or 64");
    PD_REQUIRE(out_channels == 3 || out_channels == 6, "pdhip_unet_create: out_channels must be 3 or 6");
    u->image_size = image_size; u->mc = model_channels; u->nres = num_res_blocks; u->head = num_head_channels;
    u->out_ch = out_channels; u->max_batch = max_batch; u->ted = model_channels * 4;
    u->splitk_floats = kSplitkFloats;
    u->mult.assign(channel_mult, channel_mult + n_mult);
    u->att_ds.assign(attention_ds, attention_ds + n_att);
    auto is_att = [&](int ds) { for (int a : u->att_ds) if (a == ds) return true; return false; };
    long long emb_rows = 0;
    auto add_res = [&](const std::string& name, int cin, int cout, int mode, int hw) -> int {
        ResB rb; rb.name = name; rb.cin = cin; rb.cout = cout; rb.mode = mode; rb.has_skip = cin != cout; rb.hw = hw;
        rb.emb_off = emb_rows; emb_rows += 2 * cout;
        shape_conv(rb.c1, cin, cout, 9); shape_conv(rb.c2, cout, cout, 9);
        if (rb.has_skip) shape_conv(rb.skip, cin, cout, 1);
        rb.has_c2s = rb.has_skip && mode == 0 && cin % 64 == 0 && cout % 64 == 0;
        rb.c1.has_wph = mode == 2 && ((hw / 2) * (hw / 2)) % 256 == 0 && conv_up2_phase_eligible(1, hw / 2, hw / 2, cin, cout, rb.c1.cout_pad);
        rb.c1.has_wf = rb.c2.has_wf = hw <= 64 && cin % 128 == 0 && cout % 128 == 0;
        rb.has_c2s_wf = rb.c2.has_wf && rb.has_c2s;
        u->res.push_back(rb);
        return (int)u->res.size() - 1;
    };
    auto add_att = [&](const std::string& name, int c) -> int {
        AttB ab; ab.name = name; ab.c = c;
        shape_conv(ab.qkv, c, 3 * c, 1); shape_conv(ab.proj, c, c, 1);
        u->att.push_back(ab);
        return (int)u->att.size() - 1;
    };
    int ch = u->mult[0] * u->mc;
    std::vector<int> chans{ch};
    u->input.push_back({Block{0, 0}});
    int ds = 1, n = 1;
    for (int level = 0; level < n_mult; ++level) {
        for (int r = 0; r < num_res_blocks; ++r) {
            std::vector<Block> layers;
            const int o = u->mult[level] * u->mc;
            layers.push_back(Block{1, add_res("input_blocks." + std::to_string(n) + ".0", ch, o, 0, image_size / ds)});
            ch = o;
            if (is_att(ds)) layers.push_back(Block{2, add_att("input_blocks." + std::to_string(n) + ".1", ch)});
            u->input.push_back(layers);
            chans.push_back(ch);
            ++n;
        }
        if (level != n_mult - 1) {
            u->input.push_back({Block{1, add_res("input_blocks." + std::to_string(n) + ".0", ch, ch, 1, image_size / (ds * 2))}});
            chans.push_back(ch);
            ds *= 2;
            ++n;
        }
    }
    u->middle.push_back(Block{1, add_res("middle_block.0", ch, ch, 0, image_size / ds)});
    u->middle.push_back(Block{2, add_att("middle_block.1", ch)});
    u->middle.push_back(Block{1, add_res("middle_block.2", ch, ch, 0, image_size / ds)});
    n = 0;
    for (int level = n_mult - 1; level >= 0; --level) {
        for (int i = 0; i < num_res_blocks + 1; ++i) {
            const int ich = chans.back(); chans.pop_back();
            const int o = u->mc * u->mult[level];
            std::vector<Block> layers;
            const std::string base = "output_blocks." + std::to_string(n) + ".";
            layers.push_back(Block{1, add_res(base + "0", ch + ich, o, 0, image_size / ds)});
            ch = o;
            int k = 1;
            if (is_att(ds)) { layers.push_back(Block{2, add_att(base + std::to_string(k), ch)}); ++k; }
            if (level && i == num_res_blocks) {
                layers.push_back(Block{1, add_res(base + std::to_string(k), ch, ch, 2, image_size / (ds / 2))});
                ds /= 2;
            }
            u->output.push_back(layers);
            ++n;
        }
    }
    u->final_ch = ch;
    u->emb_rows = emb_rows;
    return PDHIP_OK;
}

}

extern "C" int pdhip_unet_create(int image_size, int model_channels, int num_res_blocks, const int* channel_mult, int n_mult,
                                 const int* attention_ds, int n_att, int num_head_channels, int out_channels, int max_batch,
                                 pdhip_unet** out) {
    PD_REQUIRE(out, "pdhip_unet_create: null argument");
    pdhip_unet* u = new pdhip_unet();
    *out = nullptr;
    auto fail = [&](int rc) { for (void* p : u->owned) (void)hipFree(p); delete u; return rc; };
    int rc = build_graph(u, image_size, model_channels, num_res_blocks, channel_mult, n_mult, attention_ds, n_att, num_head_channels, out_channels, max_batch);
    if (rc) return fail(rc);
    const long long emb_rows = u->emb_rows;
    auto chk = [&](int r) { if (rc == PDHIP_OK) rc = r; };
    for (ResB& rb : u->res) {
        chk(alloc_norm(u, rb.n1, rb.cin)); chk(alloc_norm(u, rb.n2, rb.cout));
        chk(alloc_conv(u, rb.c1)); chk(alloc_conv(u, rb.c2));
        if (rb.has_skip) chk(alloc_conv(u, rb.skip));
        if (rb.has_c2s) {
            chk(dalloc(u, &rb.c2s_w, (size_t)rb.c2.cout_pad * (9 * (size_t)rb.cout + rb.cin)));
            chk(dalloc(u, &rb.c2s_b, (size_t)rb.cout));
        }
        if (rb.c1.has_wph) chk(dalloc(u, &rb.c1.wph, (size_t)16 * rb.c1.cout_pad * rb.cin));
        if (rb.c1.has_wf) chk(dalloc(u, &rb.c1.wf, conv_rr_weight_halfs(rb.cin, 9, 0, rb.cout)));
        if (rb.c2.has_wf) chk(dalloc(u, &rb.c2.wf, conv_rr_weight_halfs(rb.cout, 9, 0, rb.cout)));
        if (rb.has_c2s_wf) chk(dalloc(u, &rb.c2s_wf, conv_rr_weight_halfs(rb.cout, 9, rb.cin, rb.cout)));
        if (rc) return fail(rc);
    }
    for (AttB& ab : u->att) {
        chk(alloc_norm(u, ab.n, ab.c)); chk(alloc_conv(u, ab.qkv)); chk(alloc_conv(u, ab.proj));
        if (rc) return fail(rc);
    }
    const int c0 = u->mult[0] * u->mc;
    chk(dalloc(u, &u->w_in, (size_t)(((c0 + 127) / 128) * 128) * 32)); chk(dalloc(u, &u->b_in, (size_t)c0));
    if (rc == PDHIP_OK && hipMemset(u->w_in, 0, (size_t)(((c0 + 127) / 128) * 128) * 32 * sizeof(half_t)) != hipSuccess) rc = PDHIP_E_HIP;
    chk(dalloc(u, &u->te_w0, (size_t)u->ted * u->mc)); chk(dalloc(u, &u->te_b0, (size_t)u->ted));
    chk(dalloc(u, &u->te_w2, (size_t)u->ted * u->ted)); chk(dalloc(u, &u->te_b2, (size_t)u->ted));
    chk(dalloc(u, &u->emb_w, (size_t)emb_rows * u->ted)); chk(dalloc(u, &u->emb_b, (size_t)emb_rows));
    chk(alloc_norm(u, u->out_norm, u->final_ch));
    chk(dalloc(u, &u->out_w, (size_t)out_channels * 9 * u->final_ch)); chk(dalloc(u, &u->out_b, (size_t)out_channels));
    chk(dalloc(u, &u->zero_page, (size_t)128));
    if (rc) return fail(rc);
    if (hipMemset(u->zero_page, 0, 256) != hipSuccess) { set_error("hipMemset failed"); return fail(PDHIP_E_HIP); }
    const size_t S2 = (size_t)image_size * image_size;
    chk(forward_impl(tuning(), u, nullptr, nullptr, max_batch, nullptr, nullptr, true));
    u->arena_bytes = u->arena_off + 4096;
    {
        void* q = nullptr;
        hipError_t e = hipMalloc(&q, u->arena_bytes);
        if (e != hipSuccess) { set_error("pdhip_unet_create: activation arena of %zu bytes: %s", u->arena_bytes, hipGetErrorString(e)); return fail(PDHIP_E_NOMEM); }
        u->owned.push_back(q);
        u->arena = reinterpret_cast<char*>(q);
    }
    u->gn_ws_floats = (size_t)max_batch * ((S2 + 255) / 256) * 64;
    chk(dalloc(u, &u->stats, (size_t)max_batch * 64)); chk(dalloc(u, &u->gn_ws, u->gn_ws_floats));
    { int cmax = 0; for (const ResB& rb : u->res) cmax = std::max(cmax, std::max(rb.cin, rb.cout)); chk(dalloc(u, &u->ap_table, (size_t)max_batch * cmax * 2)); }
    chk(dalloc(u, &u->emb_silu, (size_t)max_batch * u->ted)); chk(dalloc(u, &u->emb_tmp, (size_t)max_batch * (u->mc + u->ted)));
    chk(dalloc(u, &u->emb_all, (size_t)max_batch * emb_rows));
    chk(dalloc(u, &u->steps_t, 128)); chk(dalloc(u, &u->steps_silu, (size_t)100 * u->ted));
    chk(dalloc(u, &u->steps_tmp, (size_t)100 * (u->mc + u->ted))); chk(dalloc(u, &u->steps_emb, (size_t)100 * emb_rows));
    { float* wz = nullptr; chk(dalloc(u, &wz, (size_t)64 * u->final_ch)); u->head_wz = reinterpret_cast<half_t*>(wz); }
    { float* wz = nullptr; chk(dalloc(u, &wz, (size_t)64 * u->final_ch)); u->head_wz3 = reinterpret_cast<half_t*>(wz); }
    chk(dalloc(u, &u->t_dev, (size_t)max_batch));
    chk(dalloc(u, &u->splitk_ws, u->splitk_floats));
    if (rc == PDHIP_OK && hipMemset(u->splitk_ws, 0, PD_SK_TICKET_FLOATS * sizeof(float)) != hipSuccess) rc = PDHIP_E_HIP;
    chk(dalloc(u, &u->sx, (size_t)max_batch * 3 * S2)); chk(dalloc(u, &u->sy, (size_t)max_batch * 3 * S2));
    chk(dalloc(u, &u->set_, (size_t)max_batch * out_channels * S2)); chk(dalloc(u, &u->smask, (size_t)max_batch * S2));
// ... 128 lines not shown
        if (rest == "in_layers.0.bias") return load_vec(rb.n1.b, rb.cin, &rb.n1.have_b, 0);
        if (rest == "in_layers.2.weight") return load_conv_w(rb.c1);
        if (rest == "in_layers.2.bias") return load_vec(rb.c1.b, rb.cout, &rb.c1.have_b, 1);
        if (rest == "emb_layers.1.weight") return load_vec(u->emb_w + rb.emb_off * u->ted, (long long)2 * rb.cout * u->ted, &rb.have_ew, 0);
        if (rest == "emb_layers.1.bias") return load_vec(u->emb_b + rb.emb_off, 2 * rb.cout, &rb.have_eb, 0);
        if (rest == "out_layers.0.weight") return load_vec(rb.n2.g, rb.cout, &rb.n2.have_g, 0);
        if (rest == "out_layers.0.bias") return load_vec(rb.n2.b, rb.cout, &rb.n2.have_b, 0);
        auto refuse = [&](int rc) -> int {
            if (rc != PDHIP_OK || !rb.has_c2s) return rc;
            rb.c2s_ready = false;
            if (rb.c2.have_w && rb.c2.have_b && rb.skip.have_w && rb.skip.have_b && rb.skip.taps == 1) {
                PD_TRY(fuse_skip_weights(rb.c2.w, 9 * rb.c2.cin, rb.skip.w, rb.skip.cin, rb.c2.cout_pad, rb.c2.b, rb.skip.b, rb.cout, rb.c2s_w, rb.c2s_b, s));
                if (rb.has_c2s_wf) PD_TRY(conv_rr_pack(rb.c2s_w, rb.c2.cin, 9, rb.skip.cin, rb.cout, rb.c2s_wf, s));
                rb.c2s_ready = true;
            }
            return PDHIP_OK;
        };
        if (rest == "out_layers.3.weight") return refuse(load_conv_w(rb.c2));
        if (rest == "out_layers.3.bias") return refuse(load_vec(rb.c2.b, rb.cout, &rb.c2.have_b, 1));
        if (rb.has_skip && rest == "skip_connection.weight") return refuse(load_conv_w(rb.skip));
        if (rb.has_skip && rest == "skip_connection.bias") return refuse(load_vec(rb.skip.b, rb.cout, &rb.skip.have_b, 1));
    }
    for (AttB& ab : u->att) {
        if (!starts(ab.name + ".")) continue;
        const std::string rest = name.substr(ab.name.size() + 1);
        if (rest == "norm.weight") return load_vec(ab.n.g, ab.c, &ab.n.have_g, 0);
        if (rest == "norm.bias") return load_vec(ab.n.b, ab.c, &ab.n.have_b, 0);
        if (rest == "qkv.weight") return load_conv_w(ab.qkv);
        if (rest == "qkv.bias") return load_vec(ab.qkv.b, 3 * ab.c, &ab.qkv.have_b, 1);
        if (rest == "proj_out.weight") return load_conv_w(ab.proj);
        if (rest == "proj_out.bias") return load_vec(ab.proj.b, ab.c, &ab.proj.have_b, 1);
    }
    (void)ends;
    set_error("pdhip_unet_load_tensor: unknown tensor name '%s'", name_c);
    return PDHIP_E_UNKNOWN_NAME;
}

extern "C" int pdhip_unet_forward(pdhip_unet* u, const float* x, const float* t, int N, float* out, void* stream) {
    PD_REQUIRE(u && x && t && out, "pdhip_unet_forward: null argument");
    PD_REQUIRE(N >= 1 && N <= u->max_batch, "pdhip_unet_forward: batch %d outside [1, %d]", N, u->max_batch);
    return forward_impl(tuning(), u, x, t, N, out, as_stream(stream), false);
}

extern "C" int pdhip_unet_profile(pdhip_unet* u, int enable) {
    PD_REQUIRE(u, "pdhip_unet_profile: null handle");
    u->prof.on = enable != 0;
    u->prof.period = enable > 1 ? enable : 1;
    u->prof.forwards = 0;
    u->prof.armed = false;
    u->prof.used = 0;
    u->prof.flops[0] = u->prof.flops[1] = 0;
    return PDHIP_OK;
}
static int prof_read(pdhip_unet* u, int cls, double* total_ms, double* total_flops, long long* launches) {
    double ms = 0;
    long long n = 0;
    for (size_t i = 0; i + 1 < u->prof.used; i += 2) {
        if (u->prof.cls[i] != cls) continue;
        PD_HIP(hipEventSynchronize(u->prof.ev[i + 1]));
        float e = 0;
        PD_HIP(hipEventElapsedTime(&e, u->prof.ev[i], u->prof.ev[i + 1]));
        ms += e; ++n;
    }
    *total_ms = ms; *total_flops = u->prof.flops[cls]; *launches = n;
    return PDHIP_OK;
}
extern "C" int pdhip_unet_profile_read(pdhip_unet* u, double* total_ms, double* total_flops, long long* launches) {
    PD_REQUIRE(u && total_ms && total_flops && launches, "pdhip_unet_profile_read: null argument");
    return prof_read(u, 0, total_ms, total_flops, launches);
}
extern "C" int pdhip_unet_profile_read_attention(pdhip_unet* u, double* total_ms, double* total_flops, long long* launches) {
    PD_REQUIRE(u && total_ms && total_flops && launches, "pdhip_unet_profile_read_attention: null argument");
    return prof_read(u, 1, total_ms, total_flops, launches);
}

namespace {
struct Sched { std::vector<int> t; std::vector<DdnmCoef> co; std::vector<float> ab; };
Sched make_schedule() {
    Sched s;
    s.ab.resize(1001);
    double acc = 1.0;
    s.ab[0] = 1.0f;
    const double b0 = 1e-4, b1 = 0.02, step = (b1 - b0) / 999.0;
    for (int i = 0; i < 1000; ++i) {
        const double beta = (i == 999) ? b1 : b0 + (double)i * step;
        acc = acc * (double)(1.0f - (float)beta);
        s.ab[i + 1] = (float)acc;
    }
    const double eta = 0.85;
    for (int k = 99; k >= 0; --k) {
        const int t = k * 10, tn = (k - 1) * 10 < 0 ? -1 : (k - 1) * 10;
        const float at = s.ab[t + 1], an = s.ab[tn + 1];
        DdnmCoef c;
        c.sqrt_1m_at = sqrtf(1.0f - at); c.sqrt_at = sqrtf(at); c.sqrt_at_next = sqrtf(an);
        c.sigma_t = sqrtf(1.0f - an * an);
        c.c1 = sqrtf(1.0f - an) * (float)eta;
        c.c2 = sqrtf(1.0f - an) * (float)std::sqrt(1.0 - eta * eta);
        s.t.push_back(t); s.co.push_back(c);
    }
    return s;
}
__global__ void k_fill(float* p, float v, int n) { int i = blockIdx.x * blockDim.x + threadIdx.x; if (i < n) p[i] = v; }
}

extern "C" int pdhip_ddnm_schedule(float* at, float* at_next, int* t, int* t_next, float* coefs ) {
    Sched s = make_schedule();
    for (int k = 0; k < 100; ++k) {
        const int tt = s.t[k], tn = tt - 10 < 0 ? -1 : tt - 10;
        if (at) at[k] = s.ab[tt + 1];
        if (at_next) at_next[k] = s.ab[tn + 1];
        if (t) t[k] = tt;
        if (t_next) t_next[k] = tn;
        if (coefs) memcpy(coefs + 6 * k, &s.co[k], sizeof(DdnmCoef));
    }
    return PDHIP_OK;
}

extern "C" int pdhip_ddnm_step(float* x, const float* et, int et_channels, const float* y, const float* mask, const float* eps,
                               uint64_t seed, int step, int N, int HW, void* stream) {
    PD_REQUIRE(x && et && y && mask && step >= 0 && step < 100 && (et_channels == 3 || et_channels == 6), "pdhip_ddnm_step: bad arguments");
    static const Sched sched = make_schedule();
    return ddnm_update(x, et, et_channels, y, mask, eps, seed, (unsigned long long)step + 1, sched.co[step], N, HW, as_stream(stream));
}

extern "C" int pdhip_ddnm_prepare(const float* masked_imgs, const float* masks, float* y, int N, int HW, void* stream) {
    PD_REQUIRE(masked_imgs && masks && y, "pdhip_ddnm_prepare: null argument");
    return ddnm_prepare(masked_imgs, masks, y, N, HW, as_stream(stream));
}

extern "C" int pdhip_ddnm_sample_keyed(pdhip_unet* u, const float* masked_imgs, const float* masks, int N, const float* x_T,
                                       const float* eps_tape, uint64_t seed, uint64_t first_image_key, int n_steps, float* out,
                                       void* stream) {
    PD_REQUIRE(u && masked_imgs && masks && out, "pdhip_ddnm_sample: null argument");
    PD_REQUIRE(N >= 1 && N <= u->max_batch && n_steps >= 1 && n_steps <= 100, "pdhip_ddnm_sample: bad N / n_steps");
    static const Sched sched = make_schedule();
    hipStream_t s = as_stream(stream);
    const int HW = u->image_size * u->image_size;
    const long long n3 = (long long)N * 3 * HW;
    PD_TRY(ddnm_prepare(masked_imgs, masks, u->sy, N, HW, s));
    const unsigned long long quad0 = (unsigned long long)first_image_key * (unsigned long long)(3LL * HW / 4);
    if (x_T) PD_HIP(hipMemcpyAsync(u->sx, x_T, n3 * sizeof(float), hipMemcpyDeviceToDevice, s));
    else PD_TRY(philox_normal(u->sx, n3, seed, 0, s, quad0));
    if (u->steps_cached != n_steps) {
        PD_REQUIRE(u->have_te[0] && u->have_te[1] && u->have_te[2] && u->have_te[3], "unet: time_embed not loaded");
        float th[100];
        for (int k = 0; k < n_steps; ++k) th[k] = (float)sched.t[k];
        PD_HIP(hipMemcpyAsync(u->steps_t, th, n_steps * sizeof(float), hipMemcpyHostToDevice, s));
        PD_HIP(hipStreamSynchronize(s));
        PD_TRY(timestep_mlp(u->steps_t, n_steps, u->mc, u->te_w0, u->te_b0, u->te_w2, u->te_b2, u->steps_silu, u->steps_tmp, s));
        PD_TRY(gemv_rows(u->emb_w, u->emb_b, u->steps_silu, u->steps_emb, (int)u->emb_rows, u->ted, n_steps, s));
        u->steps_cached = n_steps;
    }
    const Tuning tun = tuning();
    for (int k = 0; k < n_steps; ++k) {
        PD_TRY(forward_impl(tun, u, u->sx, nullptr, N, u->set_, s, false, u->steps_emb + (size_t)k * u->emb_rows, 3));
        PD_TRY(ddnm_update(u->sx, u->set_, 3, u->sy, masks, eps_tape ? eps_tape + (size_t)k * n3 : nullptr, seed,
                           (unsigned long long)k + 1, sched.co[k], N, HW, s, quad0));
    }
    return ddnm_finish(u->sx, out, n3, s);
}
extern "C" int pdhip_ddnm_sample(pdhip_unet* u, const float* masked_imgs, const float* masks, int N, const float* x_T,
                                 const float* eps_tape, uint64_t seed, int n_steps, float* out, void* stream) {
    return pdhip_ddnm_sample_keyed(u, masked_imgs, masks, N, x_T, eps_tape, seed, 0, n_steps, out, stream);
}

static int swap_hook(int& field, int v) { const int old = field; field = v; return old; }
extern "C" int pdhip_debug_set_conv_tile(int wmw) { return swap_hook(tuning().force_wmw, wmw); }
extern "C" int pdhip_debug_set_conv_stages(int st) { return swap_hook(tuning().force_stages, st); }
extern "C" int pdhip_debug_set_conv_bk(int bk) { return swap_hook(tuning().force_bk, bk); }
extern "C" int pdhip_debug_set_conv_halo_strips(int mode) { return swap_hook(tuning().halo_strips, mode); }
extern "C" int pdhip_debug_set_conv_splitk(void* ws, long long ws_floats, int splits) {
    g_dbg_splitk_ws = (float*)ws; g_dbg_splitk_floats = ws ? (size_t)ws_floats : 0;
    if (ws != nullptr && ws_floats >= PD_SK_TICKET_FLOATS) (void)hipMemset(ws, 0, PD_SK_TICKET_FLOATS * sizeof(float));
    return swap_hook(tuning().force_splits, splits);
}
extern "C" int pdhip_debug_set_conv_sk(int mode, int tile, int splits) { tuning().sk_tile = tile; tuning().sk_splits = splits; return swap_hook(tuning().sk_mode, mode); }
extern "C" int pdhip_debug_set_conv_sk_stages(int stages) { return swap_hook(tuning().sk_stages, stages); }
extern "C" int pdhip_debug_set_conv_sk_kgroups(int kg) { return swap_hook(tuning().sk_kg, kg); }
extern "C" int pdhip_debug_set_conv_sk_order(int order) { return swap_hook(tuning().sk_order, order); }
extern "C" int pdhip_debug_set_conv_rr(int mode, int variant, int slabs) { tuning().rr_variant = variant; tuning().rr_slabs = slabs; return swap_hook(tuning().rr_mode, mode); }
extern "C" int pdhip_debug_set_conv_ht(int mode, int slabs) { tuning().ht_slabs = slabs; return swap_hook(tuning().ht_mode, mode); }
extern "C" int pdhip_debug_set_fuse_gn(int on) { return swap_hook(tuning().fuse_gn, on); }
extern "C" int pdhip_debug_set_fold_resample(int on) { return swap_hook(tuning().fold_resample, on); }
extern "C" int pdhip_debug_set_fold_skip(int on) { return swap_hook(tuning().fold_skip, on); }
extern "C" int pdhip_debug_set_rr_gn(int max_width) { return swap_hook(tuning().rr_gn, max_width); }
extern "C" int pdhip_debug_set_fold_finalize(int max_batch) { return swap_hook(tuning().fold_finalize, max_batch); }
extern "C" int pdhip_debug_set_fold_finalize_chunks(int chunks) { return swap_hook(tuning().fold_finalize_chunks, chunks); }
extern "C" int pdhip_debug_set_fuse_skip(int mode, int min_tiles) { if (min_tiles > 0) tuning().fuse_skip_min_tiles = min_tiles; return swap_hook(tuning().fuse_skip, mode); }
extern "C" int pdhip_debug_set_up_phase(int mode) { return swap_hook(tuning().up_phase, mode); }
extern "C" int pdhip_debug_set_attn(int nbuf, int vt_form, int qtiles) {
    Tuning& t = tuning();
    const int old = t.attn_nbuf | (t.attn_vt << 8) | (t.attn_qtn << 16);
    t.attn_nbuf = nbuf; t.attn_vt = vt_form; t.attn_qtn = qtiles;
    return old;
}
extern "C" int pdhip_debug_set_gn_iters(int iters) { return swap_hook(tuning().gn_iters, iters); }
extern "C" int pdhip_debug_set_gn_skip_variant(int v) { return swap_hook(tuning().gs_variant, v); }

extern "C" int pdhip_conv2d_nhwc_f16(const void* x, const void* w_packed, const float* bias, const void* residual, void* y,
                                     int N, int H, int W, int Cin, int Cout, int Cout_pad, int taps, const void* zero_page,
                                     void* stream) {
    PD_REQUIRE(x && w_packed && y && zero_page, "pdhip_conv2d_nhwc_f16: null argument");
    return conv_igemm(tuning(), (const half_t*)x, (const half_t*)w_packed, bias, (const half_t*)residual, (half_t*)y, N, H, W, Cin, Cout,
                      Cout_pad, taps, (const half_t*)zero_page, as_stream(stream), g_dbg_splitk_ws, g_dbg_splitk_floats);
}
extern "C" int pdhip_debug_conv_launch_nhwc_f16(const void* x, const void* x2, int Cin1, const void* w_packed, const float* bias, const void* residual,
                                                int res_up, const void* xs, const void* xs2, int Cs1, int Cs, void* y, int N, int H, int W, int Cin, int Cout,
                                                int Cout_pad, int taps, const void* zero_page, float* ws, long long ws_floats, float* gn_part,
                                                long long gn_part_floats, int* gn_chunks, int* kernel, void* stream) {
    const char* const fn = "pdhip_debug_conv_launch_nhwc_f16";
    PD_REQUIRE(x && w_packed && y && zero_page, "%s: null argument", fn);
    PD_REQUIRE(N > 0 && H > 0 && W > 0 && (taps == 1 || taps == 9), "%s: bad shape (N=%d H=%d W=%d taps=%d)", fn, N, H, W, taps);
    PD_REQUIRE(Cin % 32 == 0 && Cout % 8 == 0 && Cout_pad % 128 == 0 && Cout_pad >= Cout && Cin > 0 && Cout > 0,
               "%s: need Cin %% 32 == 0, Cout %% 8 == 0, padded Cout %% 128 == 0 (Cin=%d Cout=%d pad=%d)", fn, Cin, Cout, Cout_pad);
    PD_REQUIRE(x2 == nullptr || (taps == 1 && Cin1 > 0 && Cin1 < Cin && Cin1 % 64 == 0 && (Cin - Cin1) % 64 == 0),
               "%s: a two-source input needs a 1x1 conv and channel counts that are multiples of 64", fn);
    if (xs == nullptr) Cs = 0;
    PD_REQUIRE(xs == nullptr || (taps == 9 && Cs > 0 && Cs % 64 == 0 && (xs2 == nullptr || (Cs1 > 0 && Cs1 < Cs && Cs1 % 64 == 0))),
               "%s: a skip source needs a 3x3 conv and channel counts that are multiples of 64", fn);
    PD_REQUIRE(xs != nullptr || xs2 == nullptr, "%s: xs2 without xs", fn);
    PD_REQUIRE(xs == nullptr || residual == nullptr, "%s: the appended skip 1x1 takes the residual's place", fn);
    PD_REQUIRE(res_up == 0 || residual != nullptr, "%s: res_up without a residual", fn);
    const size_t wsf = ws != nullptr && ws_floats > 0 ? (size_t)ws_floats : 0;
    pdnn::ConvNeeds nd;
    nd.two_source = x2 != nullptr; nd.want_gn = gn_part != nullptr; nd.skip_cs = Cs;
    const pdnn::ConvPlan p = conv_plan(tuning(), N, H, W, Cin, Cout, Cout_pad, taps, nd, wsf);
    if (kernel) *kernel = (int)p.kernel;
    if (gn_chunks) *gn_chunks = p.gn_chunks;
    PD_REQUIRE(res_up == 0 || p.takes_res_up, "%s: the planned kernel (%s) does not read its residual at half resolution", fn, conv_kernel_name(p.kernel));
    PD_REQUIRE(Cs == 0 || p.takes_skip, "%s: the planned kernel (%s) does not append the skip 1x1", fn, conv_kernel_name(p.kernel));
    PD_REQUIRE(x2 == nullptr || p.kernel == pdnn::CONV_SK || p.kernel == pdnn::CONV_IGEMM, "%s: the planned kernel (%s) reads one source", fn,
               conv_kernel_name(p.kernel));
    PD_REQUIRE(gn_part == nullptr || gn_part_floats >= (long long)N * p.gn_chunks * (Cout / 8) * 2,
               "%s: gn_part holds %lld floats, the launch writes %lld", fn, gn_part_floats, (long long)N * p.gn_chunks * (Cout / 8) * 2);
    const pdnn::ConvArgs a{(const half_t*)x, (const half_t*)x2, x2 ? Cin1 : 0, (const half_t*)w_packed, bias, (const half_t*)residual, res_up, nullptr, nullptr,
                           (const half_t*)xs, (const half_t*)xs2, Cs1, (half_t*)y, (const half_t*)zero_page, wsf ? ws : nullptr, wsf, gn_part};
    return conv_launch(p, a, as_stream(stream));
}
extern "C" int pdhip_gn_finalize_oct_f32(const float* partA, int Ca, int chunksA, const float* partB, int Cb, int chunksB, int N, int HW, float* stats,
                                         void* stream) {
    PD_REQUIRE(partA && stats && N > 0 && HW > 0 && Ca > 0 && chunksA > 0, "pdhip_gn_finalize_oct_f32: bad arguments");
    PD_REQUIRE(partB ? (Cb > 0 && chunksB > 0) : Cb == 0, "pdhip_gn_finalize_oct_f32: partB and Cb / chunksB disagree");
    return gn_finalize_oct(partA, Ca, chunksA, partB, Cb, partB ? chunksB : 0, N, HW, 1e-5f, stats, as_stream(stream));
}
extern "C" int pdhip_pack_conv_up2_phase_f16(const void* w_packed, int Cin, int Cout_pad, void* w_phase, void* stream) {
    PD_REQUIRE(w_packed && w_phase && Cin > 0 && Cout_pad > 0, "pdhip_pack_conv_up2_phase_f16: bad arguments");
    return conv_up2_phase_pack((const half_t*)w_packed, Cin, Cout_pad, (half_t*)w_phase, as_stream(stream));
}
extern "C" int pdhip_conv3x3_up2_phase_nhwc_f16(const void* x, const void* w_phase, const float* bias, void* y, int N, int H, int W, int Cin, int Cout,
                                                int Cout_pad, const void* zero_page, float* gn_part, void* stream) {
    PD_REQUIRE(x && w_phase && y && zero_page, "pdhip_conv3x3_up2_phase_nhwc_f16: null argument");
    const pdnn::ConvPlan p = conv_up2_phase_plan(tuning(), N, 2 * H, 2 * W, Cin, Cout, Cout_pad, gn_part != nullptr);
    return conv_up2_phase((const half_t*)x, (const half_t*)w_phase, bias, (half_t*)y, N, H, W, Cin, Cout, Cout_pad, (const half_t*)zero_page,
                          as_stream(stream), p.gn_chunks > 0 ? gn_part : nullptr, p.geo);
}
extern "C" int pdhip_conv3x3_up2_halo_nhwc_f16(const void* x, const void* w_packed, const float* bias, void* y, int N, int H, int W, int Cin, int Cout,
                                               int Cout_pad, const void* zero_page, void* stream) {
    PD_REQUIRE(x && w_packed && y && zero_page, "pdhip_conv3x3_up2_halo_nhwc_f16: null argument");
    pdnn::ConvNeeds nd;
    nd.in_up = true;
    PD_REQUIRE(conv_plan(tuning(), N, 2 * H, 2 * W, Cin, Cout, Cout_pad, 9, nd, 0).takes_in_up,
               "pdhip_conv3x3_up2_halo_nhwc_f16: not a layer the halo-resident kernel takes unsplit");
    return conv_igemm(tuning(), (const half_t*)x, (const half_t*)w_packed, bias, nullptr, (half_t*)y, N, 2 * H, 2 * W, Cin, Cout, Cout_pad, 9,
                      (const half_t*)zero_page, as_stream(stream), nullptr, 0, nullptr, nullptr, 0, nullptr, 0, 1);
}
extern "C" int pdhip_gn_silu_skip1x1_nhwc_f16(const void* xa, const void* xb, int Ca, int C, const float* stats, const float* gamma,
                                              const float* beta, const void* w_packed, const float* bias, void* h0, void* sk, int N, int H,
                                              int W, void* stream) {
    PD_REQUIRE(xa && stats && gamma && beta && w_packed && h0 && sk, "pdhip_gn_silu_skip1x1_nhwc_f16: null argument");
    return gn_skip((const half_t*)xa, (const half_t*)xb, Ca, C, stats, gamma, beta, (const half_t*)w_packed, bias, (half_t*)h0, (half_t*)sk,
                   N, H * W, as_stream(stream), tuning().gs_variant);
}
extern "C" int pdhip_gn_silu_conv3x3_nhwc_f16(const void* x, const float* gamma, const float* beta, const float* film,
                                              long long film_stride, const void* w_packed, const float* bias, const void* residual,
                                              void* y, int N, int H, int W, int Cin, int Cout, int Cout_pad, const void* zero_page,
                                              float* ws, long long ws_floats, void* stream) {
    PD_REQUIRE(x && gamma && beta && w_packed && y && zero_page && ws, "pdhip_gn_silu_conv3x3_nhwc_f16: null argument");
    const size_t gws = (size_t)N * 64 * ((H * W + 255) / 256);
    PD_REQUIRE((size_t)ws_floats >= (size_t)N * 64 + gws + (size_t)N * Cin * 2, "pdhip_gn_silu_conv3x3_nhwc_f16: workspace too small");
    hipStream_t s = as_stream(stream);
    float* stats = ws;
    float* table = ws + (size_t)N * 64 + gws;
    PD_TRY(gn_stats((const half_t*)x, N, H * W, Cin, 1e-5f, stats, ws + (size_t)N * 64, gws, s));
    PD_TRY(gn_table(stats, gamma, beta, film, film_stride, N, Cin, table, s));
    float* hws = g_dbg_splitk_ws != nullptr && g_dbg_splitk_floats > PD_SK_TICKET_FLOATS ? g_dbg_splitk_ws + PD_SK_TICKET_FLOATS : nullptr;
    const size_t hws_floats = hws ? g_dbg_splitk_floats - PD_SK_TICKET_FLOATS : 0;
    PD_REQUIRE(conv3x3_halo_eligible(N, H, W, Cin, Cout_pad) && N > 0 && Cout > 0 && Cout_pad > 0, "conv3x3_halo: unsupported geometry (N=%d H=%d W=%d Cin=%d)", N, H, W, Cin);
    return conv3x3_halo((const half_t*)x, (const half_t*)w_packed, bias, (const half_t*)residual, (half_t*)y, N, H, W, Cin, Cout,
                        Cout_pad, (const half_t*)zero_page, s, nullptr, conv3x3_halo_launch_splits(tuning(), N, H, W, Cin, Cout, Cout_pad, hws_floats),
                        conv3x3_halo_rows(tuning(), H, W), hws, hws_floats, table);
}
extern "C" int pdhip_debug_conv3x3_apply(const void* x, const float* table, const void* w_packed, const float* bias, const void* residual,
                                         void* y, int N, int H, int W, int Cin, int Cout, int Cout_pad, const void* zero_page, void* stream) {
    PD_REQUIRE(x && table && w_packed && y && zero_page, "pdhip_debug_conv3x3_apply: null argument");
    return conv3x3_halo((const half_t*)x, (const half_t*)w_packed, bias, (const half_t*)residual, (half_t*)y, N, H, W, Cin, Cout,
                        Cout_pad, (const half_t*)zero_page, as_stream(stream), nullptr, 1, conv3x3_halo_rows(tuning(), H, W), nullptr, 0, table);
}
extern "C" int pdhip_pack_conv_weight_f16(const float* w_oihw, int Cout, int Cin, int taps, void* w_packed, void* stream) {
    PD_REQUIRE(w_oihw && w_packed, "pdhip_pack_conv_weight_f16: null argument");
    k_pack_conv<<<grid_for((long long)Cout * Cin * taps), 256, 0, as_stream(stream)>>>(w_oihw, 0, Cout, Cin, taps, (half_t*)w_packed);
    PD_LAUNCH_CHECK();
    return PDHIP_OK;
}
extern "C" int pdhip_groupnorm_nhwc_f16(const void* x, const float* gamma, const float* beta, const float* film, int N, int H,
                                        int W, int C, int silu, int resample, void* y, float* stats_ws ,
                                        float* ws, long long ws_floats, void* stream) {
    PD_REQUIRE(x && gamma && beta && y && stats_ws && ws, "pdhip_groupnorm_nhwc_f16: null argument");
    PD_TRY(gn_stats((const half_t*)x, N, H * W, C, 1e-5f, stats_ws, ws, (size_t)ws_floats, as_stream(stream)));
    return gn_apply((const half_t*)x, stats_ws, gamma, beta, film, 2LL * C, N, H, W, C, silu, resample, y, 0, as_stream(stream), nullptr, 0, nullptr, nullptr,
                    tuning().gn_iters);
}
extern "C" size_t pdhip_unet_head_ws_floats(int N, int H, int W, int C, int Cout) {
    return (size_t)N * 64 + (size_t)N * 64 * ((H * W + 255) / 256) + (size_t)Cout * 9 * C + (size_t)64 * C;
}
extern "C" int pdhip_unet_head_f32(const void* x, const float* gamma, const float* beta, const float* w_oihw, const float* bias,
                                   int N, int H, int W, int C, int Cout, float* y_nchw, float* ws, long long ws_floats, void* stream) {
    PD_REQUIRE(x && gamma && beta && w_oihw && bias && y_nchw && ws, "pdhip_unet_head_f32: null argument");
    PD_REQUIRE((size_t)ws_floats >= pdhip_unet_head_ws_floats(N, H, W, C, Cout), "pdhip_unet_head_f32: workspace too small");
    hipStream_t s = as_stream(stream);
    float* stats = ws;
    float* gws = stats + (size_t)N * 64;
    const size_t gws_floats = (size_t)N * 64 * ((H * W + 255) / 256);
    float* wp = gws + gws_floats;
    half_t* wz = reinterpret_cast<half_t*>(wp + (size_t)Cout * 9 * C);
    PD_TRY(gn_stats((const half_t*)x, N, H * W, C, 1e-5f, stats, gws, gws_floats, s));
    k_pack_conv_f32<<<grid_for((long long)Cout * 9 * C), 256, 0, s>>>(w_oihw, 0, Cout, C, 9, wp);
    PD_LAUNCH_CHECK();
    PD_TRY(head_pack(wp, Cout, C, wz, s));
    return head_gn_silu_conv3x3((const half_t*)x, stats, gamma, beta, wz, bias, y_nchw, N, H, W, C, Cout, s);
}
extern "C" int pdhip_attention_f16(const void* qkv, void* out, int N, int T, int C, int head_dim, void* vt_ws, void* stream) {
    PD_REQUIRE(qkv && out, "pdhip_attention_f16: null argument");
    const Tuning& t = tuning();
    return attention((const half_t*)qkv, (half_t*)out, N, T, C, head_dim, as_stream(stream), (half_t*)vt_ws, t.attn_nbuf, t.attn_qtn, t.attn_vt);
}
extern "C" int pdhip_philox_normal(float* out, long long n, uint64_t seed, uint64_t stream_id, void* stream) {
    PD_REQUIRE(out && n > 0, "pdhip_philox_normal: bad arguments");
    return philox_normal(out, n, seed, stream_id, as_stream(stream));
}
extern "C" int pdhip_bench_copy16(const void* src, void* dst, long long bytes, int blocks, int unroll, void* stream) {
    return copy16(src, dst, bytes, blocks, unroll, as_stream(stream));
}
extern "C" int pdhip_gn_apply_f16(const void* x, const void* x2, int Ca, int C, const float* stats, const float* partA, int chunksA,
                                  const float* partB, int chunksB, const float* gamma, const float* beta, const float* film,
                                  long long film_stride, int N, int H, int W, int silu, int resample, void* y, void* y_raw, void* stream) {
    PD_REQUIRE(x && gamma && beta && y, "pdhip_gn_apply_f16: null argument");
    PD_REQUIRE(N > 0 && H > 0 && W > 0 && C > 0, "pdhip_gn_apply_f16: empty tensor");
    PD_REQUIRE((stats != nullptr) != (partA != nullptr), "pdhip_gn_apply_f16: the statistics come finished (stats) or as octet partials (partA), not both");
    PD_REQUIRE(stats == nullptr || (partB == nullptr && chunksA == 0 && chunksB == 0), "pdhip_gn_apply_f16: partials next to finished statistics");
    PD_REQUIRE(partA == nullptr || (chunksA >= 1 && (x2 == nullptr ? (partB == nullptr && chunksB == 0) : (partB != nullptr && chunksB >= 1))),
               "pdhip_gn_apply_f16: one set of octet partials (and a chunk count >= 1) per source tensor");
    PD_REQUIRE(film == nullptr || film_stride >= 2LL * C, "pdhip_gn_apply_f16: film rows hold scale[C] | shift[C]");
    if (partA != nullptr) {
        const GnPartsArg pa{partA, x2 ? Ca : C, chunksA, partB, x2 ? C - Ca : 0, chunksB, 1e-5f};
        return gn_apply((const half_t*)x, nullptr, gamma, beta, film, film_stride, N, H, W, C, silu, resample, y, 0, as_stream(stream),
                        (const half_t*)x2, x2 ? Ca : 0, (half_t*)y_raw, &pa, tuning().gn_iters);
    }
    return gn_apply((const half_t*)x, stats, gamma, beta, film, film_stride, N, H, W, C, silu, resample, y, 0, as_stream(stream),
                    (const half_t*)x2, x2 ? Ca : 0, (half_t*)y_raw, nullptr, tuning().gn_iters);
}
extern "C" int pdhip_gn_table_f32(const float* stats, const float* gamma, const float* beta, const float* film, long long film_stride, int N, int C,
                                  float* table, void* stream) {
    PD_REQUIRE(stats && gamma && beta && table && N > 0 && C > 0, "pdhip_gn_table_f32: bad arguments");
    PD_REQUIRE(film == nullptr || film_stride >= 2LL * C, "pdhip_gn_table_f32: film rows hold scale[C] | shift[C]");
    return gn_table(stats, gamma, beta, film, film_stride, N, C, table, as_stream(stream));
}
extern "C" int pdhip_resample2x_nhwc_f16(const void* x, int N, int H, int W, int C, int mode, void* y, void* stream) {
    PD_REQUIRE(x && y && N > 0 && H > 0 && W > 0 && C > 0, "pdhip_resample2x_nhwc_f16: bad arguments");
    PD_REQUIRE(mode != 1 || (H % 2 == 0 && W % 2 == 0), "pdhip_resample2x_nhwc_f16: avgpool needs even H, W");
    return resample2x((const half_t*)x, N, H, W, C, mode, (half_t*)y, as_stream(stream));
}
extern "C" int pdhip_concat_channels_f16(const void* a, int Ca, const void* b, int Cb, long long pixels, void* y, void* stream) {
    PD_REQUIRE(a && b && y && Ca > 0 && Cb > 0 && pixels > 0, "pdhip_concat_channels_f16: bad arguments");
    return concat_channels((const half_t*)a, Ca, (const half_t*)b, Cb, pixels, (half_t*)y, as_stream(stream));
}
```

pointdreamer_amd/ddnm_inpainting.py:

```python
import ctypes as C
import math
import os

import torch

from . import _lib
from ._lib import ptr, stream, check

_reg = _lib.register
vp, i32, i64, f32, f64, u64 = C.c_void_p, C.c_int, C.c_int64, C.c_float, C.c_double, C.c_uint64
_reg('pdhip_unet_create', C.c_int, [i32, i32, i32, C.POINTER(C.c_int), i32, C.POINTER(C.c_int), i32, i32, i32, i32,
                                    C.POINTER(vp)])
_reg('pdhip_unet_destroy', None, [vp])
_reg('pdhip_unet_arena_bytes', C.c_longlong, [vp])
_reg('pdhip_unet_num_tensors', C.c_int, [vp])
_reg('pdhip_unet_load_tensor', C.c_int, [vp, C.c_char_p, vp, i32, C.POINTER(C.c_int64), i32, vp])
_reg('pdhip_unet_missing_tensors', C.c_int, [vp, C.c_char_p, i32])
_reg('pdhip_unet_forward', C.c_int, [vp, vp, vp, i32, vp, vp])
_reg('pdhip_unet_profile', C.c_int, [vp, i32])
_reg('pdhip_unet_profile_read', C.c_int, [vp, C.POINTER(C.c_double), C.POINTER(C.c_double), C.POINTER(C.c_longlong)])
_reg('pdhip_unet_profile_read_attention', C.c_int, [vp, C.POINTER(C.c_double), C.POINTER(C.c_double), C.POINTER(C.c_longlong)])
_reg('pdhip_ddnm_schedule', C.c_int, [vp, vp, vp, vp, vp])
_reg('pdhip_ddnm_prepare', C.c_int, [vp, vp, vp, i32, i32, vp])
_reg('pdhip_ddnm_step', C.c_int, [vp, vp, i32, vp, vp, vp, u64, i32, i32, i32, vp])
_reg('pdhip_ddnm_sample', C.c_int, [vp, vp, vp, i32, vp, vp, u64, i32, vp, vp])
_reg('pdhip_ddnm_sample_keyed', C.c_int, [vp, vp, vp, i32, vp, vp, u64, u64, i32, vp, vp])
_reg('pdhip_debug_set_conv_bk', C.c_int, [i32])
_reg('pdhip_debug_set_conv_stages', C.c_int, [i32])
_reg('pdhip_debug_set_conv_tile', C.c_int, [i32])
_reg('pdhip_debug_set_conv_halo_strips', C.c_int, [i32])
_reg('pdhip_debug_set_conv_splitk', C.c_int, [vp, C.c_longlong, i32])
_reg('pdhip_pack_conv_weight_f16', C.c_int, [vp, i32, i32, i32, vp, vp])
_reg('pdhip_unet_head_ws_floats', C.c_size_t, [i32, i32, i32, i32, i32])
_reg('pdhip_unet_head_f32', C.c_int, [vp, vp, vp, vp, vp, i32, i32, i32, i32, i32, vp, vp, C.c_longlong, vp])
_reg('pdhip_conv2d_nhwc_f16', C.c_int, [vp, vp, vp, vp, vp, i32, i32, i32, i32, i32, i32, i32, vp, vp])
_reg('pdhip_groupnorm_nhwc_f16', C.c_int, [vp, vp, vp, vp, i32, i32, i32, i32, i32, i32, vp, vp, vp, C.c_longlong, vp])
_reg('pdhip_gn_silu_conv3x3_nhwc_f16', C.c_int, [vp, vp, vp, vp, C.c_longlong, vp, vp, vp, vp, i32, i32, i32, i32, i32, i32, vp, vp, C.c_longlong, vp])
_reg('pdhip_debug_set_fuse_gn', C.c_int, [i32])
_reg('pdhip_gn_silu_skip1x1_nhwc_f16', C.c_int, [vp, vp, i32, i32, vp, vp, vp, vp, vp, vp, vp, i32, i32, i32, vp])
_reg('pdhip_debug_set_fuse_skip', C.c_int, [i32, i32])
_reg('pdhip_debug_set_gn_skip_variant', C.c_int, [i32])
_reg('pdhip_debug_set_fold_resample', C.c_int, [i32])
_reg('pdhip_debug_set_fold_finalize', C.c_int, [i32])
_reg('pdhip_debug_set_fold_finalize_chunks', C.c_int, [i32])
_reg('pdhip_debug_set_fold_skip', C.c_int, [i32])
_reg('pdhip_debug_set_up_phase', C.c_int, [i32])
_reg('pdhip_pack_conv_up2_phase_f16', C.c_int, [vp, i32, i32, vp, vp])
_reg('pdhip_conv3x3_up2_phase_nhwc_f16', C.c_int, [vp, vp, vp, vp, i32, i32, i32, i32, i32, i32, vp, vp, vp])
_reg('pdhip_conv3x3_up2_halo_nhwc_f16', C.c_int, [vp, vp, vp, vp, i32, i32, i32, i32, i32, i32, vp, vp])
_reg('pdhip_debug_set_conv_sk', C.c_int, [i32, i32, i32])
_reg('pdhip_debug_set_conv_sk_stages', C.c_int, [i32])
_reg('pdhip_debug_set_conv_sk_kgroups', C.c_int, [i32])
_reg('pdhip_debug_set_conv_sk_order', C.c_int, [i32])
_reg('pdhip_debug_set_attn', C.c_int, [i32, i32, i32])
_reg('pdhip_debug_set_conv_rr', C.c_int, [i32, i32, i32])
_reg('pdhip_debug_set_rr_gn', C.c_int, [i32])
_reg('pdhip_debug_set_conv_ht', C.c_int, [i32, i32])
_reg('pdhip_conv_ht_plan', C.c_int, [i32, i32, i32, i32, i32, i32, C.c_longlong, C.POINTER(C.c_int), C.POINTER(C.c_int)])
_reg('pdhip_unet_route_table', C.c_int, [i32, i32, i32, C.POINTER(C.c_int), i32, C.POINTER(C.c_int), i32, i32, i32, i32, i32, C.c_char_p, i32])
_reg('pdhip_conv_ht_f16', C.c_int, [vp, vp, vp, vp, i32, vp, i32, i32, i32, i32, i32, i32, vp, vp, C.c_longlong, vp, C.POINTER(C.c_int), vp])
_reg('pdhip_conv_rr_weight_halfs', C.c_longlong, [i32, i32, i32, i32])
_reg('pdhip_conv_rr_pack_f16', C.c_int, [vp, i32, i32, i32, i32, vp, vp])
_reg('pdhip_gn_octet_partials_f16', C.c_int, [vp, i32, i32, i32, i32, vp, vp])
_reg('pdhip_gn_apply_parts_f16', C.c_int, [vp, vp, i32, i32, vp, i32, vp, i32, vp, vp, vp, C.c_longlong, i32, i32, i32, i32, vp, vp])
_reg('pdhip_conv_rr_f16', C.c_int, [vp, vp, i32, i32, i32, vp, vp, vp, C.c_longlong, vp, i32, vp, i32, vp, vp, i32, i32, i32, vp, vp, vp, i32, vp,
                                   i32, i32, i32, i32, vp, C.c_longlong, vp, C.POINTER(C.c_int), vp])
_reg('pdhip_debug_conv_launch_nhwc_f16', C.c_int, [vp, vp, i32, vp, vp, vp, i32, vp, vp, i32, i32, vp, i32, i32, i32, i32, i32, i32, i32, vp, vp, C.c_longlong,
                                                  vp, C.c_longlong, C.POINTER(C.c_int), C.POINTER(C.c_int), vp])
_reg('pdhip_gn_finalize_oct_f32', C.c_int, [vp, i32, i32, vp, i32, i32, i32, i32, vp, vp])
_reg('pdhip_debug_conv3x3_apply', C.c_int, [vp, vp, vp, vp, vp, vp, i32, i32, i32, i32, i32, i32, vp, vp])
_reg('pdhip_attention_f16', C.c_int, [vp, vp, i32, i32, i32, i32, vp, vp])
_reg('pdhip_philox_normal', C.c_int, [vp, C.c_longlong, u64, u64, vp])
_reg('pdhip_gemv_rows_f32', C.c_int, [vp, vp, vp, vp, i32, i32, i32, i32, vp])
_reg('pdhip_timestep_mlp_f32', C.c_int, [vp, i32, i32, vp, vp, vp, vp, vp, vp, vp])
_reg('pdhip_conv_in_f16', C.c_int, [vp, vp, vp, vp, i32, i32, i32, i32, i32, vp, vp, vp])
_reg('pdhip_debug_set_gn_iters', C.c_int, [i32])
_reg('pdhip_gn_apply_f16', C.c_int, [vp, vp, i32, i32, vp, vp, i32, vp, i32, vp, vp, vp, C.c_longlong, i32, i32, i32, i32, i32, vp, vp, vp])
_reg('pdhip_gn_table_f32', C.c_int, [vp, vp, vp, vp, C.c_longlong, i32, i32, vp, vp])
_reg('pdhip_resample2x_nhwc_f16', C.c_int, [vp, i32, i32, i32, i32, i32, vp, vp])
_reg('pdhip_concat_channels_f16', C.c_int, [vp, i32, vp, i32, C.c_longlong, vp, vp])
_reg('pdhip_bench_copy16', C.c_int, [vp, vp, C.c_longlong, i32, i32, vp])

IMAGENET_256 = dict(image_size=256, num_channels=256, num_res_blocks=2, attention_resolutions="32,16,8",
                    num_head_channels=64, learn_sigma=True, use_scale_shift_norm=True, resblock_updown=True,
                    use_fp16=True, channel_mult="")
DEFAULT_CKPT = 'models/DDNM/256x256_diffusion_uncond.pt'


def default_channel_mult(image_size):
    return {512: (0.5, 1, 1, 2, 2, 4, 4), 256: (1, 1, 2, 2, 4, 4), 128: (1, 1, 2, 3, 4), 64: (1, 2, 3, 4)}[image_size]


def unet_route_table(N, image_size=256, num_channels=256, num_res_blocks=2, attention_resolutions="32,16,8", num_head_channels=64,
                     learn_sigma=True, channel_mult="", max_batch=64, **unused):
    L = _lib.lib()
    cm = tuple(int(c) for c in channel_mult.split(",")) if channel_mult else default_channel_mult(image_size)
    ads = tuple(image_size // int(r) for r in attention_resolutions.split(","))
    args = (image_size, num_channels, num_res_blocks, (C.c_int * len(cm))(*cm), len(cm), (C.c_int * len(ads))(*ads), len(ads), num_head_channels,
            6 if learn_sigma else 3, max_batch, N)
    n = L.pdhip_unet_route_table(*args, None, 0)
    check(min(n, 0), 'pdhip_unet_route_table')
    buf = C.create_string_buffer(n + 1)
    check(min(L.pdhip_unet_route_table(*args, buf, n + 1), 0), 'pdhip_unet_route_table')
    return buf.value.decode().splitlines()


class UNetModel:

    def __init__(self, image_size=256, num_channels=256, num_res_blocks=2, attention_resolutions="32,16,8",
                 num_head_channels=64, learn_sigma=True, channel_mult="", max_batch=8, device='cuda', **unused):
        if not unused.get('use_scale_shift_norm', True) or not unused.get('resblock_updown', True):
            raise NotImplementedError("only the scale-shift-norm / resblock-updown variant (imagenet_256.yml) is built")
        L = _lib.lib()
        cm = tuple(int(c) for c in channel_mult.split(",")) if channel_mult else default_channel_mult(image_size)
        if any(int(c) != c for c in cm):
            raise NotImplementedError("fractional channel multipliers (image_size 512) are not built")
        ads = tuple(image_size // int(r) for r in attention_resolutions.split(","))
        self.image_size, self.out_channels, self.max_batch = image_size, 6 if learn_sigma else 3, max_batch
        self.device = _lib.resolve_device(device)
        cm_arr = (C.c_int * len(cm))(*[int(c) for c in cm])
        ad_arr = (C.c_int * len(ads))(*ads)
        h = vp()
        with torch.cuda.device(self.device):
            check(L.pdhip_unet_create(image_size, num_channels, num_res_blocks, cm_arr, len(cm), ad_arr, len(ads),
                                      num_head_channels, self.out_channels, max_batch, C.byref(h)), 'pdhip_unet_create')
        self._h = h
        self._L = L

    def __del__(self):
        h, self._h = getattr(self, '_h', None), None
        if h:
            self._L.pdhip_unet_destroy(h)

    @property
    def arena_bytes(self):
        return int(self._L.pdhip_unet_arena_bytes(self._h))

    def load_state_dict(self, state_dict, strict=True):
        L = self._L
        n = 0
        with torch.cuda.device(self.device):
            for name, t in state_dict.items():
                if t.dtype not in (torch.float32, torch.float16):
                    t = t.float()
                t = t.to(self.device).contiguous()
                shape = (C.c_int64 * t.dim())(*t.shape)
                rc = L.pdhip_unet_load_tensor(self._h, name.encode(), ptr(t), 1 if t.dtype == torch.float16 else 0, shape,
                                              t.dim(), stream())
                if rc == -5 and not strict:
                    continue
                check(rc, f'pdhip_unet_load_tensor({name})')
                n += 1
            torch.cuda.synchronize(self.device)
        buf = C.create_string_buffer(4096)
        missing = L.pdhip_unet_missing_tensors(self._h, buf, 4096)
        if strict and missing:
            raise _lib.PdhipError(f"load_state_dict: {missing} tensors missing, e.g. {buf.value.decode().split()[:4]}")
        return n

    def forward(self, x, timesteps):
        x = x.float().contiguous()
        t = timesteps.float().to(x.device).contiguous()
        N = x.shape[0]
        if x.device != self.device:
            raise _lib.PdhipError(f"UNetModel lives on {self.device}, input is on {x.device}")
        out = torch.empty((N, self.out_channels, self.image_size, self.image_size), device=x.device)
        with torch.cuda.device(self.device):
            check(self._L.pdhip_unet_forward(self._h, ptr(x), ptr(t), N, ptr(out), stream()), 'pdhip_unet_forward')
        return out

    __call__ = forward

    def profile(self, enable):
        check(self._L.pdhip_unet_profile(self._h, int(enable)), 'pdhip_unet_profile')

    def profile_read(self, attention=False):
        ms, fl, n = C.c_double(), C.c_double(), C.c_longlong()
        fn = self._L.pdhip_unet_profile_read_attention if attention else self._L.pdhip_unet_profile_read
        check(fn(self._h, C.byref(ms), C.byref(fl), C.byref(n)), 'pdhip_unet_profile_read')
        return ms.value, fl.value, n.value


def ddnm_schedule():
    import numpy as np
    L = _lib.lib()
    at = np.zeros(100, np.float32)
    an = np.zeros(100, np.float32)
    t = np.zeros(100, np.int32)
    tn = np.zeros(100, np.int32)
    co = np.zeros((100, 6), np.float32)
    check(L.pdhip_ddnm_schedule(at.ctypes.data, an.ctypes.data, t.ctypes.data, tn.ctypes.data, co.ctypes.data),
          'pdhip_ddnm_schedule')
    return at, an, t, tn, co


def random_state_dict(model_kwargs, seed=0, device='cpu'):
    image_size = model_kwargs.get('image_size', 256)
    mc = model_kwargs.get('num_channels', 256)
    nres = model_kwargs.get('num_res_blocks', 2)
    cm = model_kwargs.get('channel_mult') or ""
    cm = tuple(int(c) for c in cm.split(",")) if cm else default_channel_mult(image_size)
    ads = tuple(image_size // int(r) for r in model_kwargs.get('attention_resolutions', "32,16,8").split(","))
    out_ch = 6 if model_kwargs.get('learn_sigma', True) else 3
    ted = mc * 4
    g = torch.Generator(device='cpu').manual_seed(seed)
    sd = {}

    def lin(name, o, i):
        sd[name + '.weight'] = torch.randn((o, i), generator=g) / math.sqrt(i)
        sd[name + '.bias'] = torch.randn((o,), generator=g) * 0.05

    def conv(name, o, i, k, one_d=False):
        shape = (o, i, k) if one_d else (o, i, k, k)
        sd[name + '.weight'] = torch.randn(shape, generator=g) / math.sqrt(i * k * (1 if one_d else k))
        sd[name + '.bias'] = torch.randn((o,), generator=g) * 0.05

    def norm(name, c):
        sd[name + '.weight'] = 1.0 + torch.randn((c,), generator=g) * 0.05
        sd[name + '.bias'] = torch.randn((c,), generator=g) * 0.05

    def res(name, cin, cout):
        norm(name + '.in_layers.0', cin); conv(name + '.in_layers.2', cout, cin, 3)
        lin(name + '.emb_layers.1', 2 * cout, ted)
        norm(name + '.out_layers.0', cout); conv(name + '.out_layers.3', cout, cout, 3)
        if cin != cout:
            conv(name + '.skip_connection', cout, cin, 1)

    def att(name, c):
        norm(name + '.norm', c); conv(name + '.qkv', 3 * c, c, 1, True); conv(name + '.proj_out', c, c, 1, True)
    lin('time_embed.0', ted, mc); lin('time_embed.2', ted, ted)
    ch = int(cm[0] * mc)
    conv('input_blocks.0.0', ch, 3, 3)
    chans = [ch]
    ds, n = 1, 1
# ... 69 lines not shown
```

Baseline: 2204 shapes/hour.

## Carry head conv halo rows across tiles and add fused DDNM update and conv_in GN paths

Measured after the change: 2207 shapes/hour, median of 6. Within noise of the previous version (+0.1%).

```diff
diff --git a/include/pdhip.h b/include/pdhip.h
--- a/include/pdhip.h
+++ b/include/pdhip.h
@@ -250,6 +250,12 @@
 int pdhip_debug_set_gn_iters(int iters);
 int pdhip_debug_set_gn_skip_variant(int v);
 int pdhip_debug_set_fuse_skip(int mode, int min_tiles);
+int pdhip_debug_set_ends(int bits);
+int pdhip_gn_apply_conv_in_f16(const void* col, const void* Wt, const float* bias, const float* stats, const float* gamma, const float* beta,
+                               int N, int H, int W, int C, int silu, void* y, void* stream);
+int pdhip_unet_head_ddnm_f32(const void* x, const float* gamma, const float* beta, const float* w_oihw, const float* bias, int N, int H, int W, int C,
+                             float* ws, long long ws_floats, float* xs, const float* y, const float* mask, const float* eps, uint64_t seed, int step,
+                             void* stream);
 int pdhip_debug_set_fuse_gn(int on);
 int pdhip_mark_unpainted_faces(const int64_t* face_id, const uint8_t* painted, int A, int F, uint8_t* flags , void* stream);
 int pdhip_vertex_texel_fetch(const float* vert_uvs , int V, const float* atlas , const uint8_t* mask ,
diff --git a/pointdreamer_amd/csrc/nn_common.h b/pointdreamer_amd/csrc/nn_common.h
--- a/pointdreamer_amd/csrc/nn_common.h
+++ b/pointdreamer_amd/csrc/nn_common.h
@@ -38,7 +38,9 @@
     int attn_vt = 0;
     int gn_iters = 0;
     int gs_variant = 1;
-};
+    int ends = 4;
+};
+enum { ENDS_CONV_IN_GN = 1, ENDS_CONV_IN_SKIP = 2, ENDS_HEAD_CARRY = 4, ENDS_HEAD_UPDATE = 8 };
 Tuning& tuning();
 
 bool conv3x3_halo_eligible(int N, int H, int W, int Cin, int Cout_pad);
@@ -161,6 +163,8 @@
              half_t* Yraw = nullptr,
              const GnPartsArg* parts = nullptr,
              int iters_hook = 0);
+int gn_apply_conv_in(const half_t* col, const half_t* Wt, const float* bias, const float* stats, const float* gamma, const float* beta, int N,
+                     int H, int W, int C, int silu, half_t* Y, hipStream_t s);
 int gn_table(const float* stats, const float* gamma, const float* beta, const float* film, long long film_stride, int N, int C,
              float* table, hipStream_t s);
 bool gn_skip_eligible(int N, int HW, int Ca, int C, int Cout, int Cout_pad);
@@ -174,14 +178,16 @@
 int conv_in_3x3(const ConvPlan& p, const float* x_nchw, const half_t* Wt , const float* bias, half_t* Y,
                 int N, int H, int W, int Cout, int Cout_pad, half_t* im2col_ws , const half_t* zero_page, hipStream_t s, float* gn_part = nullptr);
 int head_pack(const float* w, int NO, int C, half_t* wz, hipStream_t s);
+struct DdnmCoef { float sqrt_1m_at, sqrt_at, sqrt_at_next, sigma_t, c1, c2; };
+struct HeadUpdate { float* x; const float* y; const float* mask; const float* eps; unsigned long long seed, step, quad0; DdnmCoef co; };
 int head_gn_silu_conv3x3(const half_t* X, const float* stats, const float* gamma, const float* beta, const half_t* wz,
-                         const float* bias, float* y_nchw, int N, int H, int W, int C, int NO, hipStream_t s);
+                         const float* bias, float* y_nchw, int N, int H, int W, int C, int NO, hipStream_t s, int ends = 0,
+                         const HeadUpdate* upd = nullptr);
 int timestep_mlp(const float* t, int N, int mc, const float* w0, const float* b0, const float* w2, const float* b2,
                  float* emb_silu , float* tmp, hipStream_t s);
 int gemv_rows(const float* Wm , const float* b, const float* x , float* y , int R, int K, int N,
               hipStream_t s);
 
-struct DdnmCoef { float sqrt_1m_at, sqrt_at, sqrt_at_next, sigma_t, c1, c2; };
 int ddnm_update(float* x , const float* et , int Cet, const float* y,
                 const float* mask , const float* eps , unsigned long long seed,
                 unsigned long long step, DdnmCoef co, int N, int HW, hipStream_t s, unsigned long long quad0 = 0);
@@ -191,4 +197,44 @@
 int philox_normal(float* out, long long n, unsigned long long seed, unsigned long long stream_id, hipStream_t s,
                   unsigned long long quad0 = 0);
 
-}
+__device__ __forceinline__ void philox4x32_10(uint32_t c[4], uint32_t k0, uint32_t k1) {
+#pragma unroll
+    for (int r = 0; r < 10; ++r) {
+        const uint64_t p0 = (uint64_t)0xD2511F53u * c[0], p1 = (uint64_t)0xCD9E8D57u * c[2];
+        const uint32_t n0 = (uint32_t)(p1 >> 32) ^ c[1] ^ k0, n2 = (uint32_t)(p0 >> 32) ^ c[3] ^ k1;
+        c[0] = n0; c[1] = (uint32_t)p1; c[2] = n2; c[3] = (uint32_t)p0;
+        k0 += 0x9E3779B9u; k1 += 0xBB67AE85u;
+    }
+}
+__device__ __forceinline__ void normal4(unsigned long long seed, unsigned long long stream_id, unsigned long long quad, float out[4]) {
+    uint32_t c[4] = {(uint32_t)quad, (uint32_t)(quad >> 32), (uint32_t)stream_id, (uint32_t)(stream_id >> 32)};
+    philox4x32_10(c, (uint32_t)seed, (uint32_t)(seed >> 32));
+    const float u0 = ((float)c[0] + 0.5f) * 2.3283064365386963e-10f, u1 = ((float)c[1] + 0.5f) * 2.3283064365386963e-10f;
+    const float u2 = ((float)c[2] + 0.5f) * 2.3283064365386963e-10f, u3 = ((float)c[3] + 0.5f) * 2.3283064365386963e-10f;
+    const float r0 = sqrtf(-2.0f * logf(u0)), r1 = sqrtf(-2.0f * logf(u2));
+    out[0] = r0 * cosf(6.283185307179586f * u1); out[1] = r0 * sinf(6.283185307179586f * u1);
+    out[2] = r1 * cosf(6.283185307179586f * u3); out[3] = r1 * sinf(6.283185307179586f * u3);
+}
+
+__device__ __forceinline__ void ddnm_update_quad(float* __restrict__ x, const float ev[4], const float* __restrict__ y, const float* __restrict__ mask,
+                                                 const float* __restrict__ eps, unsigned long long seed, unsigned long long step,
+                                                 unsigned long long quad, const DdnmCoef& co) {
+    float z[4];
+    if (eps) { const float4 e4 = *reinterpret_cast<const float4*>(eps); z[0] = e4.x; z[1] = e4.y; z[2] = e4.z; z[3] = e4.w; }
+    else normal4(seed, step, quad, z);
+    const float4 x4 = *reinterpret_cast<const float4*>(x);
+    const float4 y4 = *reinterpret_cast<const float4*>(y);
+    const float4 m4 = *reinterpret_cast<const float4*>(mask);
+    const float xv[4] = {x4.x, x4.y, x4.z, x4.w};
+    const float yv[4] = {y4.x, y4.y, y4.z, y4.w}, mv[4] = {m4.x, m4.y, m4.z, m4.w};
+    float o[4];
+#pragma unroll
+    for (int k = 0; k < 4; ++k) {
+        const float x0 = (xv[k] - ev[k] * co.sqrt_1m_at) / co.sqrt_at;
+        const float x0h = x0 - mv[k] * (mv[k] * x0 - yv[k]);
+        o[k] = co.sqrt_at_next * x0h + co.sigma_t * (co.c1 * z[k] + co.c2 * ev[k]);
+    }
+    *reinterpret_cast<float4*>(x) = make_float4(o[0], o[1], o[2], o[3]);
+}
+
+}
diff --git a/pointdreamer_amd/csrc/nn_head.hip b/pointdreamer_amd/csrc/nn_head.hip
--- a/pointdreamer_amd/csrc/nn_head.hip
+++ b/pointdreamer_amd/csrc/nn_head.hip
@@ -9,6 +9,7 @@
 #define HD_IH (HD_TH + 2)
 #define HD_NPIX (HD_IW * HD_IH)
 #define HD_NCH ((HD_NPIX + 15) / 16)
+#define HD_CARRY_PIX 64
 #define HD_ZS_OF(NO) ((NO) == 6 ? 60 : 28)
 
 __device__ __host__ __forceinline__ int hd_swz(int n, int C) { return n & 15 & (C / 8 - 1); }
@@ -36,11 +37,11 @@
 
 __device__ __forceinline__ float hd_silu(float x) { return x * __builtin_amdgcn_rcpf(1.0f + __expf(-x)); }
 
-template <int NO, int C>
+template <int NO, int C, bool UPD>
 __global__ __launch_bounds__(512) void k_head(const half_t* __restrict__ X, const float* __restrict__ stats,
                                               const float* __restrict__ gamma, const float* __restrict__ beta,
                                               const half_t* __restrict__ wz, const float* __restrict__ bias,
-                                              float* __restrict__ y, int H, int W, int tpw) {
+                                              float* __restrict__ y, int H, int W, int tpw, int carry, HeadUpdate u) {
     constexpr int KK = C / 32;
     constexpr int NT = (9 * NO + 15) / 16;
     constexpr int NR = NT * 16;
@@ -66,6 +67,8 @@
     __syncthreads();
 
     const int q4 = lane >> 4, r16 = lane & 15;
+    constexpr int HD_CJ = (HD_CARRY_PIX * 9 * NO + 511) / 512;
+    bool carried = false;
     for (int it = 0; it < tpw; ++it) {
     const int y0 = (blockIdx.y * tpw + it) * HD_TH;
     if (y0 >= H) break;
@@ -78,12 +81,13 @@
     };
     half8 vn[KK];
     bool in_n = false;
-    if (wave < HD_NCH) {
-        const half_t* sp = src_of(wave, &in_n);
+    const int chunk0 = wave + (carried ? HD_CARRY_PIX / 16 : 0);
+    if (chunk0 < HD_NCH) {
+        const half_t* sp = src_of(chunk0, &in_n);
 #pragma unroll
         for (int kk = 0; kk < KK; ++kk) vn[kk] = *reinterpret_cast<const half8*>(sp + kk * 32);
     }
-    for (int chunk = wave; chunk < HD_NCH; chunk += 8) {
+    for (int chunk = chunk0; chunk < HD_NCH; chunk += 8) {
         half8 v[KK];
         const bool inimg = in_n;
 #pragma unroll
@@ -134,6 +138,27 @@
     }
     __syncthreads();
 
+    if (UPD) {
+        for (int item = tid; item < HD_TW / 4 * HD_TH * NO; item += 512) {
+            const int o = item / (HD_TW / 4 * HD_TH), q = item - o * (HD_TW / 4 * HD_TH);
+            const int qy = q / (HD_TW / 4), qx = (q - qy * (HD_TW / 4)) * 4;
+            const int gy = y0 + qy, gx = x0 + qx;
+            if (gy >= H || gx >= W) continue;
+            float a[4];
+#pragma unroll
+            for (int k = 0; k < 4; ++k) {
+                a[k] = bias[o];
+#pragma unroll
+                for (int tap = 0; tap < 9; ++tap) {
+                    const int iy = qy + tap / 3, ix = qx + k + tap % 3;
+                    a[k] += zs[(iy * HD_IW + ix) * HD_ZS + tap * NO + o];
+                }
+            }
+            const size_t i = (((size_t)n * NO + o) * H + gy) * W + gx;
+            ddnm_update_quad(u.x + i, a, u.y + i, u.mask + ((size_t)n * H + gy) * W + gx, u.eps ? u.eps + i : nullptr, u.seed, u.step,
+                             u.quad0 + (unsigned long long)(i >> 2), u.co);
+        }
+    } else {
     for (int item = tid; item < HD_TW * HD_TH * NO; item += 512) {
         const int o = item / (HD_TW * HD_TH), q = item - o * (HD_TW * HD_TH);
         const int qy = q / HD_TW, qx = q - qy * HD_TW;
@@ -147,7 +172,24 @@
         }
         y[(((size_t)n * NO + o) * H + gy) * W + gx] = a;
     }
+    }
+    carried = carry != 0 && it + 1 < tpw && y0 + HD_TH < H;
+    float cv[HD_CJ];
+    if (carried) {
+#pragma unroll
+        for (int j = 0; j < HD_CJ; ++j) {
+            const int e = tid + j * 512, pix = e / (9 * NO), col = e - pix * (9 * NO);
+            if (e < HD_CARRY_PIX * 9 * NO) cv[j] = zs[(HD_TH * HD_IW + pix) * HD_ZS + col];
+        }
+    }
     __syncthreads();
+    if (carried) {
+#pragma unroll
+        for (int j = 0; j < HD_CJ; ++j) {
+            const int e = tid + j * 512, pix = e / (9 * NO), col = e - pix * (9 * NO);
+            if (e < HD_CARRY_PIX * 9 * NO) zs[pix * HD_ZS + col] = cv[j];
+        }
+    }
     }
 }
 
@@ -156,24 +198,38 @@
     return (size_t)2 * NR * C * 2 + (size_t)HD_NCH * 16 * HD_ZS_OF(NO) * 4 + (size_t)2 * C * 4;
 }
 
-template <int NO, int C>
+template <int NO, int C, bool UPD>
 static int head_launch(const half_t* X, const float* stats, const float* gamma, const float* beta, const half_t* wz,
-                       const float* bias, float* y, int N, int H, int W, hipStream_t s) {
-    auto kern = k_head<NO, C>;
+                       const float* bias, float* y, int N, int H, int W, hipStream_t s, int ends, const HeadUpdate& u) {
+    auto kern = k_head<NO, C, UPD>;
     const size_t smem = head_smem_bytes(C, NO);
     PD_HIP(hipFuncSetAttribute((const void*)kern, hipFuncAttributeMaxDynamicSharedMemorySize, (int)smem));
     int tpw = HD_TPW;
     while (tpw > 1 && (long long)cdiv(W, HD_TW) * cdiv(cdiv(H, HD_TH), tpw) * N < 512) tpw >>= 1;
+    if ((ends >> 8) > 0) tpw = std::min(ends >> 8, 8);
     dim3 grid(cdiv(W, HD_TW), cdiv(cdiv(H, HD_TH), tpw), N);
-    kern<<<grid, 512, smem, s>>>(X, stats, gamma, beta, wz, bias, y, H, W, tpw);
+    kern<<<grid, 512, smem, s>>>(X, stats, gamma, beta, wz, bias, y, H, W, tpw, (ends & ENDS_HEAD_CARRY) != 0, u);
     PD_LAUNCH_CHECK();
     return PDHIP_OK;
 }
 
 int head_gn_silu_conv3x3(const half_t* X, const float* stats, const float* gamma, const float* beta, const half_t* wz,
-                         const float* bias, float* y_nchw, int N, int H, int W, int C, int NO, hipStream_t s) {
+                         const float* bias, float* y_nchw, int N, int H, int W, int C, int NO, hipStream_t s, int ends,
+                         const HeadUpdate* upd) {
     PD_REQUIRE(NO == 3 || NO == 6, "head: out channels must be 3 or 6");
-#define HL(NO_, C_) head_launch<NO_, C_>(X, stats, gamma, beta, wz, bias, y_nchw, N, H, W, s)
+    if (upd != nullptr) {
+        PD_REQUIRE(NO == 3 && W % 4 == 0 && upd->x && upd->y && upd->mask, "head: the fused DDNM update takes 3 output channels and W %% 4 == 0 (NO=%d W=%d)", NO, W);
+#define HU(C_) head_launch<3, C_, true>(X, stats, gamma, beta, wz, bias, nullptr, N, H, W, s, ends, *upd)
+        if (C == 256) return HU(256);
+        if (C == 128) return HU(128);
+        if (C == 64) return HU(64);
+        if (C == 32) return HU(32);
+#undef HU
+        PD_REQUIRE(false, "head: final channel count must be 32, 64, 128 or 256 (got %d)", C);
+    }
+    PD_REQUIRE(y_nchw != nullptr, "head: null output");
+    const HeadUpdate none{};
+#define HL(NO_, C_) head_launch<NO_, C_, false>(X, stats, gamma, beta, wz, bias, y_nchw, N, H, W, s, ends, none)
     if (C == 256) return NO == 6 ? HL(6, 256) : HL(3, 256);
     if (C == 128) return NO == 6 ? HL(6, 128) : HL(3, 128);
     if (C == 64) return NO == 6 ? HL(6, 64) : HL(3, 64);
diff --git a/pointdreamer_amd/csrc/nn_misc.hip b/pointdreamer_amd/csrc/nn_misc.hip
--- a/pointdreamer_amd/csrc/nn_misc.hip
+++ b/pointdreamer_amd/csrc/nn_misc.hip
@@ -143,25 +143,6 @@
     return gemv_launch(w2, b2, h1, emb_silu, 4 * mc, 4 * mc, N, 1, s);
 }
 
-__device__ __forceinline__ void philox4x32_10(uint32_t c[4], uint32_t k0, uint32_t k1) {
-#pragma unroll
-    for (int r = 0; r < 10; ++r) {
-        const uint64_t p0 = (uint64_t)0xD2511F53u * c[0], p1 = (uint64_t)0xCD9E8D57u * c[2];
-        const uint32_t n0 = (uint32_t)(p1 >> 32) ^ c[1] ^ k0, n2 = (uint32_t)(p0 >> 32) ^ c[3] ^ k1;
-        c[0] = n0; c[1] = (uint32_t)p1; c[2] = n2; c[3] = (uint32_t)p0;
-        k0 += 0x9E3779B9u; k1 += 0xBB67AE85u;
-    }
-}
-__device__ __forceinline__ void normal4(unsigned long long seed, unsigned long long stream_id, unsigned long long quad, float out[4]) {
-    uint32_t c[4] = {(uint32_t)quad, (uint32_t)(quad >> 32), (uint32_t)stream_id, (uint32_t)(stream_id >> 32)};
-    philox4x32_10(c, (uint32_t)seed, (uint32_t)(seed >> 32));
-    const float u0 = ((float)c[0] + 0.5f) * 2.3283064365386963e-10f, u1 = ((float)c[1] + 0.5f) * 2.3283064365386963e-10f;
-    const float u2 = ((float)c[2] + 0.5f) * 2.3283064365386963e-10f, u3 = ((float)c[3] + 0.5f) * 2.3283064365386963e-10f;
-    const float r0 = sqrtf(-2.0f * logf(u0)), r1 = sqrtf(-2.0f * logf(u2));
-    out[0] = r0 * cosf(6.283185307179586f * u1); out[1] = r0 * sinf(6.283185307179586f * u1);
-    out[2] = r1 * cosf(6.283185307179586f * u3); out[3] = r1 * sinf(6.283185307179586f * u3);
-}
-
 __global__ void k_philox_normal(float* __restrict__ out, long long n, unsigned long long seed, unsigned long long stream_id,
                                 unsigned long long quad0) {
     const long long quads = (n + 3) / 4;
@@ -204,23 +185,9 @@
         const long long n = i / (3LL * HW);
         const int c = (int)((i / HW) % 3);
         const int p = (int)(i % HW);
-        float z[4];
-        if (eps) { const float4 e4 = *reinterpret_cast<const float4*>(eps + i); z[0] = e4.x; z[1] = e4.y; z[2] = e4.z; z[3] = e4.w; }
-        else normal4(seed, step, quad0 + (unsigned long long)q, z);
-        const float4 x4 = *reinterpret_cast<const float4*>(x + i);
         const float4 e4 = *reinterpret_cast<const float4*>(et + ((size_t)n * Cet + c) * HW + p);
-        const float4 y4 = *reinterpret_cast<const float4*>(y + i);
-        const float4 m4 = *reinterpret_cast<const float4*>(mask + n * HW + p);
-        const float xv[4] = {x4.x, x4.y, x4.z, x4.w}, ev[4] = {e4.x, e4.y, e4.z, e4.w};
-        const float yv[4] = {y4.x, y4.y, y4.z, y4.w}, mv[4] = {m4.x, m4.y, m4.z, m4.w};
-        float o[4];
-#pragma unroll
-        for (int k = 0; k < 4; ++k) {
-            const float x0 = (xv[k] - ev[k] * co.sqrt_1m_at) / co.sqrt_at;
-            const float x0h = x0 - mv[k] * (mv[k] * x0 - yv[k]);
-            o[k] = co.sqrt_at_next * x0h + co.sigma_t * (co.c1 * z[k] + co.c2 * ev[k]);
-        }
-        *reinterpret_cast<float4*>(x + i) = make_float4(o[0], o[1], o[2], o[3]);
+        const float ev[4] = {e4.x, e4.y, e4.z, e4.w};
+        ddnm_update_quad(x + i, ev, y + i, mask + n * HW + p, eps ? eps + i : nullptr, seed, step, quad0 + (unsigned long long)q, co);
     }
 }
 int ddnm_update(float* x, const float* et, int Cet, const float* y, const float* mask, const float* eps,
diff --git a/pointdreamer_amd/csrc/nn_norm.hip b/pointdreamer_amd/csrc/nn_norm.hip
--- a/pointdreamer_amd/csrc/nn_norm.hip
+++ b/pointdreamer_amd/csrc/nn_norm.hip
@@ -328,6 +328,87 @@
     else GNA_LAUNCH(2, false, false);
 #undef GNA_LAUNCH
 #undef GNA_ARGS
+    PD_LAUNCH_CHECK();
+    return PDHIP_OK;
+}
+
+#define GCI_GROUPS 32
+__global__ __launch_bounds__(256) void k_gn_apply_conv_in(const half_t* __restrict__ col, const half_t* __restrict__ Wt, const float* __restrict__ bias,
+                                                          const float* __restrict__ stats, const float* __restrict__ gamma,
+                                                          const float* __restrict__ beta, int HW, int C, int silu, half_t* __restrict__ Y, int gpw) {
+    __shared__ half8 s_t[4][16][8];
+    const int lane = threadIdx.x & 63, wave = threadIdx.x >> 6;
+    const int r16 = lane & 15, q4 = lane >> 4;
+    const int slices = C >> 6, pw = 4 / slices;
+    const int slice = wave % slices, psub = wave / slices;
+    const int n = blockIdx.y, cg = C / 32;
+    const int cb = slice * 64;
+    half8 wa[4];
+#pragma unroll
+    for (int t = 0; t < 4; ++t) {
+        const int ch = cb + 32 * (t >> 1) + 8 * (r16 >> 2) + 4 * (t & 1) + (r16 & 3);
+        wa[t] = *reinterpret_cast<const half8*>(Wt + (size_t)ch * 32 + 8 * q4);
+    }
+    float bv[2][8], ga[2][8], gb[2][8];
+#pragma unroll
+    for (int t = 0; t < 2; ++t)
+#pragma unroll
+        for (int e = 0; e < 8; ++e) {
+            const int c = cb + 32 * t + 8 * q4 + e, grp = c / cg;
+            const float mean = stats[((size_t)n * 32 + grp) * 2], rstd = stats[((size_t)n * 32 + grp) * 2 + 1];
+            bv[t][e] = bias[c];
+            ga[t][e] = rstd * gamma[c];
+            gb[t][e] = beta[c] - mean * ga[t][e];
+        }
+    const int groups = (HW + 15) >> 4;
+    const int g_begin = blockIdx.x * (pw * gpw) + psub, g_end = min(groups, (int)(blockIdx.x + 1) * (pw * gpw));
+    const half_t* const cn = col + (size_t)n * HW * 32;
+    half_t* const Yn = Y + (size_t)n * HW * C + cb;
+    auto load = [&](int g) -> half8 {
+        const int p = g * 16 + r16;
+        return p < HW ? *reinterpret_cast<const half8*>(cn + (size_t)p * 32 + 8 * q4) : (half8){0, 0, 0, 0, 0, 0, 0, 0};
+    };
+    const int spx = lane >> 3, sseg = lane & 7;
+    half8 bn = g_begin < g_end ? load(g_begin) : (half8){0, 0, 0, 0, 0, 0, 0, 0};
+    for (int g = g_begin; g < g_end; g += pw) {
+        const half8 b = bn;
+        if (g + pw < g_end) bn = load(g + pw);
+#pragma unroll
+        for (int t = 0; t < 2; ++t) {
+            const float4_t z = (float4_t){0.f, 0.f, 0.f, 0.f};
+            const float4_t a0 = __builtin_amdgcn_mfma_f32_16x16x32_f16(wa[2 * t], b, z, 0, 0, 0);
+            const float4_t a1 = __builtin_amdgcn_mfma_f32_16x16x32_f16(wa[2 * t + 1], b, z, 0, 0, 0);
+            half8 hv;
+#pragma unroll
+            for (int e = 0; e < 8; ++e) {
+                const half_t x = (half_t)((e < 4 ? a0[e & 3] : a1[e & 3]) + bv[t][e]);
+                hv[e] = (half_t)gn_elem<false, false>((float)x, ga[t][e], gb[t][e], 1.f, 0.f, silu);
+            }
+            s_t[wave][r16][(4 * t + q4) ^ (r16 & 7)] = hv;
+        }
+        __builtin_amdgcn_fence(__ATOMIC_RELEASE, "wavefront");
+        __builtin_amdgcn_wave_barrier();
+        __builtin_amdgcn_fence(__ATOMIC_ACQUIRE, "wavefront");
+#pragma unroll
+        for (int k = 0; k < 2; ++k) {
+            const int px = 8 * k + spx, p = g * 16 + px;
+            const half8 v = s_t[wave][px][sseg ^ (px & 7)];
+            if (p < HW) *reinterpret_cast<half8*>(Yn + (size_t)p * C + 8 * sseg) = v;
+        }
+        __builtin_amdgcn_fence(__ATOMIC_RELEASE, "wavefront");
+        __builtin_amdgcn_wave_barrier();
+        __builtin_amdgcn_fence(__ATOMIC_ACQUIRE, "wavefront");
+    }
+}
+
+int gn_apply_conv_in(const half_t* col, const half_t* Wt, const float* bias, const float* stats, const float* gamma, const float* beta, int N,
+                     int H, int W, int C, int silu, half_t* Y, hipStream_t s) {
+    PD_REQUIRE(col && Wt && bias && stats && gamma && beta && Y, "gn_apply_conv_in: null argument");
+    PD_REQUIRE((C == 64 || C == 128 || C == 256) && N > 0 && H > 0 && W > 0, "gn_apply_conv_in: C must be 64, 128 or 256 (got %d)", C);
+    const int groups = (H * W + 15) / 16, pw = 256 / C;
+    int gpw = GCI_GROUPS;
+    while (gpw > 1 && (long long)cdiv(groups, pw * gpw) * N < 2048) gpw >>= 1;
+    k_gn_apply_conv_in<<<dim3(cdiv(groups, pw * gpw), N), 256, 0, s>>>(col, Wt, bias, stats, gamma, beta, H * W, C, silu, Y, gpw);
     PD_LAUNCH_CHECK();
     return PDHIP_OK;
 }
diff --git a/pointdreamer_amd/csrc/nn_unet.hip b/pointdreamer_amd/csrc/nn_unet.hip
--- a/pointdreamer_amd/csrc/nn_unet.hip
+++ b/pointdreamer_amd/csrc/nn_unet.hip
@@ -19,7 +19,8 @@
 
 struct Act { half_t* p; int C, H, W; const float* gn_part = nullptr; int gn_chunks = 0; const float* gn_partB = nullptr; int Ca = 0; int gn_chunksB = 0;
              half_t* p2 = nullptr;
-             int row = -1, rowB = -1; };
+             int row = -1, rowB = -1;
+             const half_t* col = nullptr; };
 
 }
 namespace pdnn {
@@ -250,6 +251,8 @@
                         x.p2 ? x.Ca : 0, raw_pool, &pa, c.t.gn_iters);
     }
     PD_TRY(run_gn_stats(c, x));
+    if ((c.t.ends & ENDS_CONV_IN_GN) != 0 && x.col != nullptr && x.p2 == nullptr && film == nullptr && resample == 0 && (x.C == 64 || x.C == 128 || x.C == 256))
+        return gn_apply_conv_in(x.col, c.u->w_in, c.u->b_in, c.u->stats, n.g, n.b, c.N, x.H, x.W, x.C, silu, out->p, c.s);
     return gn_apply(x.p, c.u->stats, n.g, n.b, film, film_stride, c.N, x.H, x.W, x.C, silu, resample, out->p, 0, c.s, x.p2, x.p2 ? x.Ca : 0,
                     raw_pool, nullptr, c.t.gn_iters);
 }
@@ -403,6 +406,7 @@
             float* part = reinterpret_cast<float*>(arena_take(c.u, (size_t)c.N * ((o.H * o.W + 127) / 128) * (o.C / 8) * 2 * 2));
             if (c.table) { Act in{nullptr, 32, o.H, o.W}; table_row(c, "input_blocks.0.0", p, ConvIn{&in}, &o); }
             if (!c.dry) adopt_parts(&o, part, p.gn_chunks);
+            o.col = col;
             if (c.go()) {
                 PD_REQUIRE(c.u->have_win && c.u->have_bin, "unet: input conv not loaded");
                 PD_TRY(conv_in_3x3(p, x_nchw, c.u->w_in, c.u->b_in, o.p, c.N, o.H, o.W, o.C, cpad, col, c.u->zero_page, c.s, part));
@@ -418,7 +422,8 @@
 }
 
 int forward_impl(const Tuning& tun, pdhip_unet* u, const float* x, const float* t, int N, float* out, hipStream_t s, bool dry,
-                 const float* shared_emb = nullptr, int head_ch = 0, Table* table = nullptr) {
+                 const float* shared_emb = nullptr, int head_ch = 0, Table* table = nullptr,
+                 const HeadUpdate* upd = nullptr) {
     Ctx c{u, N, s, dry, shared_emb ? shared_emb : u->emb_all, shared_emb ? 0 : u->emb_rows, table, tun};
     u->arena_off = 0;
     u->arena_overflow = false;
@@ -461,7 +466,7 @@
         PD_TRY(run_gn_stats(c, h));
         const bool eps_only = head_ch == 3 && u->out_ch == 6;
         PD_TRY(head_gn_silu_conv3x3(h.p, u->stats, u->out_norm.g, u->out_norm.b, eps_only ? u->head_wz3 : u->head_wz, u->out_b, out, N,
-                                    h.H, h.W, h.C, eps_only ? 3 : u->out_ch, s));
+                                    h.H, h.W, h.C, eps_only ? 3 : u->out_ch, s, tun.ends, upd));
     }
     return PDHIP_OK;
 }
@@ -896,10 +901,12 @@
         u->steps_cached = n_steps;
     }
     const Tuning tun = tuning();
+    const bool fused = (tun.ends & ENDS_HEAD_UPDATE) != 0 && u->image_size % 4 == 0;
     for (int k = 0; k < n_steps; ++k) {
-        PD_TRY(forward_impl(tun, u, u->sx, nullptr, N, u->set_, s, false, u->steps_emb + (size_t)k * u->emb_rows, 3));
-        PD_TRY(ddnm_update(u->sx, u->set_, 3, u->sy, masks, eps_tape ? eps_tape + (size_t)k * n3 : nullptr, seed,
-                           (unsigned long long)k + 1, sched.co[k], N, HW, s, quad0));
+        const float* eps_k = eps_tape ? eps_tape + (size_t)k * n3 : nullptr;
+        const HeadUpdate upd{u->sx, u->sy, masks, eps_k, seed, (unsigned long long)k + 1, quad0, sched.co[k]};
+        PD_TRY(forward_impl(tun, u, u->sx, nullptr, N, u->set_, s, false, u->steps_emb + (size_t)k * u->emb_rows, 3, nullptr, fused ? &upd : nullptr));
+        if (!fused) PD_TRY(ddnm_update(u->sx, u->set_, 3, u->sy, masks, eps_k, seed, (unsigned long long)k + 1, sched.co[k], N, HW, s, quad0));
     }
     return ddnm_finish(u->sx, out, n3, s);
 }
@@ -940,6 +947,7 @@
 }
 extern "C" int pdhip_debug_set_gn_iters(int iters) { return swap_hook(tuning().gn_iters, iters); }
 extern "C" int pdhip_debug_set_gn_skip_variant(int v) { return swap_hook(tuning().gs_variant, v); }
+extern "C" int pdhip_debug_set_ends(int bits) { return swap_hook(tuning().ends, bits); }
 
 extern "C" int pdhip_conv2d_nhwc_f16(const void* x, const void* w_packed, const float* bias, const void* residual, void* y,
                                      int N, int H, int W, int Cin, int Cout, int Cout_pad, int taps, const void* zero_page,
@@ -1071,7 +1079,27 @@
     k_pack_conv_f32<<<grid_for((long long)Cout * 9 * C), 256, 0, s>>>(w_oihw, 0, Cout, C, 9, wp);
     PD_LAUNCH_CHECK();
     PD_TRY(head_pack(wp, Cout, C, wz, s));
-    return head_gn_silu_conv3x3((const half_t*)x, stats, gamma, beta, wz, bias, y_nchw, N, H, W, C, Cout, s);
+    return head_gn_silu_conv3x3((const half_t*)x, stats, gamma, beta, wz, bias, y_nchw, N, H, W, C, Cout, s, tuning().ends);
+}
+extern "C" int pdhip_unet_head_ddnm_f32(const void* x, const float* gamma, const float* beta, const float* w_oihw, const float* bias, int N, int H, int W,
+                                        int C, float* ws, long long ws_floats, float* xs, const float* y, const float* mask, const float* eps,
+                                        uint64_t seed, int step, void* stream) {
+    PD_REQUIRE(x && gamma && beta && w_oihw && bias && ws && xs && y && mask, "pdhip_unet_head_ddnm_f32: null argument");
+    PD_REQUIRE(N >= 1 && H >= 1 && W >= 4 && W % 4 == 0 && step >= 0 && step < 100, "pdhip_unet_head_ddnm_f32: need W %% 4 == 0 and a step in [0, 100) (W=%d step=%d)", W, step);
+    PD_REQUIRE((size_t)ws_floats >= pdhip_unet_head_ws_floats(N, H, W, C, 3), "pdhip_unet_head_ddnm_f32: workspace too small");
+    static const Sched sched = make_schedule();
+    hipStream_t s = as_stream(stream);
+    float* stats = ws;
+    float* gws = stats + (size_t)N * 64;
+    const size_t gws_floats = (size_t)N * 64 * ((H * W + 255) / 256);
+    float* wp = gws + gws_floats;
+    half_t* wz = reinterpret_cast<half_t*>(wp + (size_t)3 * 9 * C);
+    PD_TRY(gn_stats((const half_t*)x, N, H * W, C, 1e-5f, stats, gws, gws_floats, s));
+    k_pack_conv_f32<<<grid_for((long long)3 * 9 * C), 256, 0, s>>>(w_oihw, 0, 3, C, 9, wp);
+    PD_LAUNCH_CHECK();
+    PD_TRY(head_pack(wp, 3, C, wz, s));
+    const HeadUpdate upd{xs, y, mask, eps, seed, (unsigned long long)step + 1, 0, sched.co[step]};
+    return head_gn_silu_conv3x3((const half_t*)x, stats, gamma, beta, wz, bias, nullptr, N, H, W, C, 3, s, tuning().ends, &upd);
 }
 extern "C" int pdhip_attention_f16(const void* qkv, void* out, int N, int T, int C, int head_dim, void* vt_ws, void* stream) {
     PD_REQUIRE(qkv && out, "pdhip_attention_f16: null argument");
@@ -1109,6 +1137,12 @@
     PD_REQUIRE(film == nullptr || film_stride >= 2LL * C, "pdhip_gn_table_f32: film rows hold scale[C] | shift[C]");
     return gn_table(stats, gamma, beta, film, film_stride, N, C, table, as_stream(stream));
 }
+extern "C" int pdhip_gn_apply_conv_in_f16(const void* col, const void* Wt, const float* bias, const float* stats, const float* gamma, const float* beta,
+                                          int N, int H, int W, int C, int silu, void* y, void* stream) {
+    PD_REQUIRE(col && Wt && bias && stats && gamma && beta && y, "pdhip_gn_apply_conv_in_f16: null argument");
+    PD_REQUIRE(N > 0 && H > 0 && W > 0, "pdhip_gn_apply_conv_in_f16: empty tensor");
+    return gn_apply_conv_in((const half_t*)col, (const half_t*)Wt, bias, stats, gamma, beta, N, H, W, C, silu, (half_t*)y, as_stream(stream));
+}
 extern "C" int pdhip_resample2x_nhwc_f16(const void* x, int N, int H, int W, int C, int mode, void* y, void* stream) {
     PD_REQUIRE(x && y && N > 0 && H > 0 && W > 0 && C > 0, "pdhip_resample2x_nhwc_f16: bad arguments");
     PD_REQUIRE(mode != 1 || (H % 2 == 0 && W % 2 == 0), "pdhip_resample2x_nhwc_f16: avgpool needs even H, W");
diff --git a/pointdreamer_amd/ddnm_inpainting.py b/pointdreamer_amd/ddnm_inpainting.py
--- a/pointdreamer_amd/ddnm_inpainting.py
+++ b/pointdreamer_amd/ddnm_inpainting.py
@@ -80,6 +80,9 @@
 _reg('pdhip_resample2x_nhwc_f16', C.c_int, [vp, i32, i32, i32, i32, i32, vp, vp])
 _reg('pdhip_concat_channels_f16', C.c_int, [vp, i32, vp, i32, C.c_longlong, vp, vp])
 _reg('pdhip_bench_copy16', C.c_int, [vp, vp, C.c_longlong, i32, i32, vp])
+_reg('pdhip_debug_set_ends', C.c_int, [i32])
+_reg('pdhip_gn_apply_conv_in_f16', C.c_int, [vp, vp, vp, vp, vp, vp, i32, i32, i32, i32, i32, vp, vp])
+_reg('pdhip_unet_head_ddnm_f32', C.c_int, [vp, vp, vp, vp, vp, i32, i32, i32, i32, vp, C.c_longlong, vp, vp, vp, vp, u64, i32, vp])
 
 IMAGENET_256 = dict(image_size=256, num_channels=256, num_res_blocks=2, attention_resolutions="32,16,8",
                     num_head_channels=64, learn_sigma=True, use_scale_shift_norm=True, resblock_updown=True,
```
